# Orange-OpenSource/pyDcop

Measured on AMD Instinct MI355X. Metric: MaxSum iterations/sec on 100k-var random graph-coloring DCOP, higher is better.
Workload: dtype f64; 1 GPU; coloring_100k; n_vars=100000, n_factors=200000, n_edges=400000, domain=3, params=damping 0.5/both, stability 0.1, start leafs, parallelism=one GPU, 1 launch(es) per cycle, parity_checked=True, parity_test=tests/test_gpu_parity.py::test_north_star_100k_coloring

## Files before the change

include/maxsum_gpu.h:

```cpp
#ifndef MAXSUM_GPU_H
#define MAXSUM_GPU_H

#include <stdint.h>

#ifdef __cplusplus
extern "C" {
#endif

#define MXS_OK            0
#define MXS_E_INVALID    -1
#define MXS_E_NODEVICE   -2
#define MXS_E_HIP        -3
#define MXS_E_NOMEM      -4
#define MXS_E_STATE      -5
#define MXS_E_COMM       -6

#define MXS_MODE_MIN 0
#define MXS_MODE_MAX 1
#define MXS_DAMP_NONE    0
#define MXS_DAMP_VARS    1
#define MXS_DAMP_FACTORS 2
#define MXS_DAMP_BOTH    3
#define MXS_START_LEAFS      0
#define MXS_START_LEAFS_VARS 1
#define MXS_START_ALL        2
#define MXS_DTYPE_F64 0
#define MXS_DTYPE_F32 1

typedef struct mxs_graph {
    int32_t        n_vars;
    int32_t        n_factors;
    int32_t        n_edges;
    const int32_t *dom_size;
    const double  *var_cost;
    const int32_t *init_idx;
    const int32_t *factor_rowptr;
    const int32_t *edge_var;
    const int64_t *table_off;
    const double  *tables;
    const int32_t *var_rowptr;
    const int32_t *var_edges;
    const uint8_t *var_owned;
    const uint8_t *factor_owned;
    const double  *eval_var_cost;
} mxs_graph;

typedef struct mxs_params {
    int32_t mode;
    int32_t damping_nodes;
    int32_t start_messages;
    int32_t dtype;
    double  damping;
    double  stability;
    int32_t graph_chunk;
    int32_t layout_flags;
} mxs_params;

typedef struct mxs_engine mxs_engine;

int mxs_device_count(int32_t *count);

int mxs_create(const mxs_graph *g, const mxs_params *p, int32_t device,
               mxs_engine **out);

int mxs_reset(mxs_engine *e);

int mxs_run(mxs_engine *e, int32_t n_cycles);

int mxs_run_timed(mxs_engine *e, int32_t n_cycles, float *elapsed_ms);

int mxs_run_reps(mxs_engine *e, int32_t n_cycles, int32_t reps, float *elapsed_ms);

int mxs_run_async(mxs_engine *e, int32_t n_cycles);
int mxs_sync(mxs_engine *e);

int mxs_cycle_count(const mxs_engine *e, int64_t *cycles);

int mxs_get_assignment(mxs_engine *e, int32_t *idx, double *belief);

int mxs_get_messages(mxs_engine *e, double *v2f, double *f2v,
                     uint8_t *count_v2f, uint8_t *count_f2v);

int mxs_set_state(mxs_engine *e, const double *v2f, const double *f2v,
                  const uint8_t *count_v2f, const uint8_t *count_f2v,
                  const int32_t *idx, const double *belief, int64_t cycles);

int mxs_eval_cost(mxs_engine *e, const int32_t *idx, double infinity,
                  double *cost, int64_t *violations);

int mxs_cycle_bytes(const mxs_engine *e, int64_t *algorithmic_bytes,
                    int32_t *launches_per_cycle);

int mxs_table_storage(const mxs_engine *e, int64_t factors[4], int64_t *table_bytes_per_cycle);

int mxs_factor_order(const mxs_engine *e, int32_t *tiled);

int mxs_factor_kernels(const mxs_engine *e, int64_t counts[7]);

int mxs_variable_kernels(const mxs_engine *e, int64_t counts[6]);

int mxs_update_factor_table(mxs_engine *e, int32_t factor, const double *table, int64_t n_entries);

int mxs_set_parent_table(mxs_engine *e, int32_t factor, const double *parent, int32_t n_dims,
                         const int32_t *dims, const uint8_t *is_external);
int mxs_slice_factor(mxs_engine *e, int32_t factor, const int32_t *external_idx);

int mxs_debug_timeline(mxs_engine *e, int64_t *out, int32_t cap, int32_t *n_blocks);

int mxs_halo_setup(mxs_engine *e, const int32_t *send_edges, int64_t n_send,
                   const int32_t *recv_edges, int64_t n_recv);
int mxs_halo_buffers(mxs_engine *e, void **send_dev, int64_t *send_bytes,
                     void **recv_dev, int64_t *recv_bytes);
int mxs_halo_bind(mxs_engine *e, void *send_dev, void *recv_dev);
int mxs_step_compute(mxs_engine *e);
int mxs_step_pack(mxs_engine *e);
int mxs_step_unpack(mxs_engine *e);
int mxs_stream(mxs_engine *e, void **stream);

#define MXS_UNIQUE_ID_BYTES 128
int mxs_comm_unique_id(const char *rccl_path, uint8_t *id );
int mxs_comm_init(mxs_engine *e, const char *rccl_path, int32_t rank, int32_t world,
                  const uint8_t *id, const int64_t *send_counts, const int64_t *recv_counts);
int mxs_comm_exchange(mxs_engine *e);
int mxs_run_sharded(mxs_engine *e, int32_t n_cycles);
#define MXS_MAX_PEERS 8
#define MXS_MAX_ARITY 30
#define MXS_IPC_HANDLE_BYTES 64
typedef struct mxs_peer_info {
    int32_t qualifies;
    int32_t rank;
    int64_t ghost_len;
    int64_t recv_at[MXS_MAX_PEERS];
    int64_t recv_len[MXS_MAX_PEERS];
    uint8_t ghost_handle[MXS_IPC_HANDLE_BYTES];
    uint8_t flag_handle[MXS_IPC_HANDLE_BYTES];
    int64_t pid;
    uint64_t ghost_ptr, flag_ptr;
} mxs_peer_info;
int mxs_peer_export(mxs_engine *e, int32_t rank, int32_t world, const int64_t *send_counts,
                    const int64_t *recv_counts, mxs_peer_info *out);
int mxs_peer_connect(mxs_engine *e, const mxs_peer_info *all );

int mxs_shard_mode(const mxs_engine *e, int32_t *fused_launch, int32_t *direct_exchange);

int mxs_destroy(mxs_engine *e);

const char *mxs_last_error(void);

typedef struct mxs_amaxsum mxs_amaxsum;
int mxs_amaxsum_create(const mxs_graph *g, const mxs_params *p, int32_t device, mxs_amaxsum **out);
int mxs_amaxsum_reset(mxs_amaxsum *e);
int mxs_amaxsum_run(mxs_amaxsum *e, int32_t max_generations, int64_t *delivered);
int mxs_amaxsum_status(const mxs_amaxsum *e, int32_t *next_generation, int64_t *pending, int64_t *delivered);
int mxs_amaxsum_generation_sizes(const mxs_amaxsum *e, int64_t *out, int32_t cap, int32_t *n);
int mxs_amaxsum_get_assignment(mxs_amaxsum *e, int32_t *idx, double *belief);
int mxs_amaxsum_get_messages(mxs_amaxsum *e, double *f_cost, double *v_cost, double *f_prev, double *v_prev,
                             uint8_t *f_has, uint8_t *v_has, uint8_t *f_cnt, uint8_t *v_cnt);
int mxs_amaxsum_eval_cost(mxs_amaxsum *e, const int32_t *idx, double infinity, double *cost, int64_t *violations);
int mxs_amaxsum_update_factor_table(mxs_amaxsum *e, int32_t factor, const double *table, int64_t n_entries);
int mxs_amaxsum_destroy(mxs_amaxsum *e);

typedef struct mxs_mgm mxs_mgm;
int mxs_mgm_create(const mxs_graph *g, const mxs_params *p, const int32_t *name_rank, int32_t device,
                   mxs_mgm **out);
int mxs_mgm_reset(mxs_mgm *e);
int mxs_mgm_set_value_rank(mxs_mgm *e, const int32_t *value_rank);
int mxs_mgm_run(mxs_mgm *e, int32_t n_rounds);
int mxs_mgm_rounds(const mxs_mgm *e, int64_t *rounds);
int mxs_mgm_get_state(mxs_mgm *e, int32_t *idx, double *cost, uint8_t *has_cost, double *gain, int32_t *new_value);
int mxs_mgm_eval_cost(mxs_mgm *e, const int32_t *idx, double infinity, double *cost, int64_t *violations);
int mxs_mgm_destroy(mxs_mgm *e);

typedef struct mxs_dsa mxs_dsa;
int mxs_dsa_create(const mxs_graph *g, const mxs_params *p, int32_t variant, double probability,
                   int32_t arity_mode, uint64_t seed, int32_t device, mxs_dsa **out);
int mxs_dsa_reset(mxs_dsa *e);
int mxs_dsa_set_value_rank(mxs_dsa *e, const int32_t *value_rank);
int mxs_dsa_run(mxs_dsa *e, int32_t n_cycles);
int mxs_dsa_cycles(const mxs_dsa *e, int64_t *cycles);
int mxs_dsa_get_state(mxs_dsa *e, int32_t *idx, double *cost);
int mxs_dsa_eval_cost(mxs_dsa *e, const int32_t *idx, double infinity, double *cost, int64_t *violations);
int mxs_dsa_destroy(mxs_dsa *e);
// ... 68 lines not shown
```

pydcop_amd/csrc/engine.hip:

```cpp
#include <hip/hip_runtime.h>
#include <dlfcn.h>
#include <unistd.h>

#include <algorithm>
#include <climits>
#include <cstdio>
#include <cstdlib>
#include <cstring>
#include <map>
#include <memory>
#include <mutex>
#include <string>
#include <vector>

#include "../../include/maxsum_gpu.h"
#include "kernels.h"
#include "nary_box.h"
#include "bin_box.h"
#include "small_box.h"
#include "layout.h"

namespace mxs {

static thread_local std::string g_err;
// ... 70 lines not shown
    r->GroupEnd = (int (*)())sym("ncclGroupEnd");
    r->GetErrorString = (const char* (*)(int))sym("ncclGetErrorString");
    if (!ok) return nullptr;
    const Rccl* out = r.get();
    libs[key] = std::move(r);
    return out;
}

#define NCCL_TRY(expr)                                                                      \
    do {                                                                                    \
        int _r = (expr);                                                                    \
        if (_r != 0)                                                                        \
            return fail(MXS_E_COMM, std::string(#expr) + ": " + rccl->GetErrorString(_r));  \
    } while (0)

template <typename U>
struct DevBuf {
    U* p = nullptr;
    size_t n = 0;
    hipError_t alloc(size_t count) {
        if (p) (void)hipFree(p);
        p = nullptr;
        n = count;
        return hipMalloc((void**)&p, std::max<size_t>(count, 1) * sizeof(U));
    }
    hipError_t upload(const std::vector<U>& h, hipStream_t st) {
        hipError_t e = alloc(h.size());
        if (e != hipSuccess || h.empty()) return e;
        e = hipMemcpyAsync(p, h.data(), h.size() * sizeof(U), hipMemcpyHostToDevice, st);
        if (e != hipSuccess) return e;
        return hipStreamSynchronize(st);
    }
    ~DevBuf() {
        if (p) (void)hipFree(p);
    }
};

struct EngineBase {
    virtual ~EngineBase() {}
    virtual int init(const mxs_graph& g, const mxs_params& p, int device) = 0;
    virtual int reset() = 0;
    virtual int run_async(int n) = 0;
    virtual int sync() = 0;
    virtual int run_timed(int n, float* ms) = 0;
    virtual int run_reps(int n, int reps, float* ms) = 0;
    virtual int get_assignment(int32_t* idx, double* belief) = 0;
    virtual int get_messages(double* v2f, double* f2v, uint8_t* cv, uint8_t* cf) = 0;
    virtual int set_state(const double* v2f, const double* f2v, const uint8_t* cv, const uint8_t* cf,
                          const int32_t* idx, const double* belief, int64_t cyc) = 0;
    virtual int eval_cost(const int32_t* idx, double infinity, double* cost, int64_t* viol) = 0;
    virtual int halo_setup(const int32_t* se, int64_t ns, const int32_t* re, int64_t nr) = 0;
    virtual int halo_buffers(void** s, int64_t* sb, void** r, int64_t* rb) = 0;
    virtual int halo_bind(void* s, void* r) = 0;
    virtual int step_compute() = 0;
    virtual int step_pack() = 0;
    virtual int step_unpack() = 0;
    virtual int comm_init(const char* path, int rank, int world, const uint8_t* id,
                          const int64_t* sc, const int64_t* rc) = 0;
    virtual int comm_exchange() = 0;
    virtual int run_sharded(int n) = 0;
    virtual void shard_mode(int32_t* f, int32_t* d) const = 0;
    virtual int peer_export(int rank, int world, const int64_t* sc, const int64_t* rc, mxs_peer_info* out) = 0;
    virtual int peer_connect(const mxs_peer_info* all) = 0;
    virtual bool peer_mode() const = 0;
    virtual int debug_timeline(int64_t* out, int32_t cap, int32_t* n_blocks) = 0;
    virtual int update_table(int32_t factor, const double* table, int64_t n) = 0;
    virtual int set_parent(int32_t factor, const double* parent, int32_t nd, const int32_t* dims, const uint8_t* ext) = 0;
    virtual int slice_factor(int32_t factor, const int32_t* ext_idx) = 0;
    Layout L;
    mxs_params params{};
    int64_t cycles = 0;
    hipStream_t stream = nullptr;
    hipStream_t comm = nullptr;
    int launches_per_cycle = 1;
};

template <typename T>
struct Engine : EngineBase {
    int device = 0;
    int cur = 0;
    DevBuf<T> v2f[2], f2v[2], tables, var_cost, belief, halo_send, halo_recv;
    DevBuf<uint8_t> cF, cV, owned, fowned;
    DevBuf<int32_t> vrowptr, vdom, init_idx, edge_gen_factor, edge_dom, sel, vell;
    DevBuf<WaveMeta> vwave;
    DevBuf<int32_t> edge_v2f, f2v_off, vslot_f2v, vslot_v2f;
    DevBuf<int32_t> frowptr, edge_var_int, eval_idx;
    DevBuf<int64_t> vcost_off, eval_tab_off, halo_send_off, halo_recv_off, timeline;
    bool timeline_on = false;
    DevBuf<FactorGen> fgen;
    DevBuf<uint32_t> sched;
    DevBuf<uint8_t> ctables;
    size_t ctables_used = 0;
    DevBuf<ClassInfo> classes;
    DevBuf<ClassInfo> classes2;
    DevBuf<ClassInfo> classes_f;
    DevBuf<ClassInfo> classes8;
    DevBuf<uint32_t> halo_flags;
    bool fused = false;
    uint32_t unpacks = 0;
    DevBuf<NaryDesc> ndesc;
    DevBuf<WideBlock> wide_blocks;
    DevBuf<HubBlock> hub_blocks;
    bool has_hub = false;
#ifdef MXS_WIDE_PROFILE
    DevBuf<int64_t> wide_prof;
#endif
    DevBuf<double> eval_tables, eval_var_cost, part_cost;
    DevBuf<unsigned long long> part_viol;
    hipEvent_t ev0 = nullptr, ev1 = nullptr;
    hipStream_t side = nullptr;
    hipEvent_t ev_fork = nullptr, ev_join = nullptr;
    bool overlap = false, capturing = false;
    bool streaming = false;
    hipEvent_t ev_p1 = nullptr;
    hipEvent_t ev_halo = nullptr;
    bool halo_pending = false;
    hipGraphExec_t graph_exec = nullptr;
    int graph_cycles = 0;
    bool graph_tried = false;
    int64_t n_halo_send = 0, n_halo_recv = 0;
    T* send_buf = nullptr;
    T* recv_buf = nullptr;
    bool halo_ready = false;
    static constexpr int EVAL_BLOCKS = 1024;
    static constexpr int FUSED_MAX_CUT_BLOCKS = 1024;

    ~Engine() override {
        for (int q = 0; q < MXS_MAX_PEERS; ++q) {
            if (peer_local[q]) continue;
            if (peer_ghost[q]) (void)hipIpcCloseMemHandle(peer_ghost[q]);
            if (peer_flag[q]) (void)hipIpcCloseMemHandle(peer_flag[q]);
        }
        if (nccl_comm) {
            if (comm) (void)hipStreamSynchronize(comm);
            (void)rccl->CommDestroy(nccl_comm);
        }
#ifdef MXS_WIDE_PROFILE
        wide_profile_dump();
#endif
        if (graph_exec) (void)hipGraphExecDestroy(graph_exec);
        if (ev_fork) (void)hipEventDestroy(ev_fork);
        if (ev_join) (void)hipEventDestroy(ev_join);
        if (side) (void)hipStreamDestroy(side);
        if (ev0) (void)hipEventDestroy(ev0);
        if (ev1) (void)hipEventDestroy(ev1);
        if (ev_p1) (void)hipEventDestroy(ev_p1);
        if (ev_halo) (void)hipEventDestroy(ev_halo);
        if (comm) (void)hipStreamDestroy(comm);
        if (stream) (void)hipStreamDestroy(stream);
    }

    SweepArgs<T> make_args(int from, bool start, int phase = 1) const {
        SweepArgs<T> a{};
        a.v2f_old = v2f[from].p;
        a.v2f_new = v2f[from ^ 1].p;
        a.f2v_old = f2v[from].p;
        a.f2v_new = f2v[from ^ 1].p;
        a.tables = tables.p;
        a.ctables = ctables.p;
        a.tab_neg = L.is_max ? 1 : 0;
        a.var_cost = var_cost.p;
        a.cF = cF.p;
        a.cV = cV.p;
        a.edge_v2f = edge_v2f.p;
        a.f2v_off = f2v_off.p;
        a.vrowptr = vrowptr.p;
        a.vslot_f2v = vslot_f2v.p;
        a.vslot_v2f = vslot_v2f.p;
        a.vell = vell.p;
        a.vwave = vwave.p;
        a.hub_blocks = hub_blocks.p;
        a.vdom = vdom.p;
        a.vcost_off = vcost_off.p;
        a.init_idx = init_idx.p;
        a.fgen = fgen.p;
        a.edge_gen_factor = edge_gen_factor.p;
        a.edge_dom = edge_dom.p;
        a.sel = sel.p;
        a.belief = belief.p;
        a.damping = (T)params.damping;
        a.stability = (T)params.stability;
        a.damp_f = (params.damping_nodes & MXS_DAMP_FACTORS) ? 1 : 0;
        a.damp_v = (params.damping_nodes & MXS_DAMP_VARS) ? 1 : 0;
        a.start = start ? 1 : 0;
        a.start_mode = params.start_messages;
        a.null_f2v = (int32_t)L.null_f2v;
        a.timeline = timeline_on ? timeline.p : nullptr;
#ifdef MXS_WIDE_PROFILE
        if (!timeline_on) a.timeline = wide_prof.p;
#endif
        a.halo_flags = nullptr;
        a.need_epoch = 0;
        a.send_out = direct ? send2[from ^ 1].p : nullptr;
        a.send_slot = direct ? send_slot.p : nullptr;
        a.n_peers = 0;
        a.me = comm_rank;
        a.ghost_lo = INT32_MAX;
        a.ghost_old = nullptr;
        for (int q = 0; q < MXS_MAX_PEERS; ++q) {
            a.peer_first[q] = INT32_MAX;
            a.peer_dst[q] = nullptr;
        }
        if (p2p) {
            a.n_peers = comm_world;
            a.ghost_lo = (int32_t)L.v2f_elems;
            a.ghost_old = start ? ghost3.p + 3 * ghost_len : ghost3.p + (int64_t)(gen % 3) * ghost_len;
            a.send_slot = send_slot.p;
            a.send_out = nullptr;
            for (int q = 0; q < comm_world; ++q) {
                a.peer_first[q] = peer_first[q];
                a.peer_dst[q] = peer_ghost[q] ? peer_ghost[q] + (int64_t)((gen + 1) % 3) * peer_len[q] + peer_at[q] : nullptr;
            }
        }
        if (phase == 3) {
            a.n_classes = (int32_t)L.fused_block_base.size();
            for (int i = 0; i < MAX_CLASSES; ++i)
                a.block_base[i] = i < a.n_classes ? L.fused_block_base[i] : INT32_MAX;
            a.classes = classes_f.p;
            a.halo_flags = halo_flags.p;
            a.need_epoch = p2p ? gen : unpacks;
            return a;
        }
        const std::vector<int32_t>& order = phase == 1 ? L.sweep_order : L.sweep_order2;
        a.n_classes = (int32_t)order.size();
        for (int i = 0; i < MAX_CLASSES; ++i)
            a.block_base[i] = i < a.n_classes ? L.classes[order[i]].block_base : INT32_MAX;
        a.classes = phase == 1 ? classes.p : classes2.p;
        a.sched = (phase == 1 && !L.sched.empty()) ? sched.p : nullptr;
        return a;
    }

    int launch_sweep(const SweepArgs<T>& a, int nb) {
        if (nb <= 0) return MXS_OK;
        const dim3 grid(nb), block(BLOCK);
        if (p2p) {
            switch (L.dsel) {
                case 2: hipLaunchKernelGGL((k_sweep_p2p<T, 2>), grid, block, 0, stream, a); break;
                case 3: hipLaunchKernelGGL((k_sweep_p2p<T, 3>), grid, block, 0, stream, a); break;
                case 4: hipLaunchKernelGGL((k_sweep_p2p<T, 4>), grid, block, 0, stream, a); break;
                default: hipLaunchKernelGGL((k_sweep_p2p<T, 0>), grid, block, 0, stream, a); break;
            }
        } else if (timeline_on && has_hub) {
            if (L.dsel == 3) hipLaunchKernelGGL((k_sweep_timeline_hub<T, 3>), grid, block, 0, stream, a);
            else hipLaunchKernelGGL((k_sweep_timeline_hub<T, 0>), grid, block, 0, stream, a);
        } else if (timeline_on) {
            switch (L.dsel) {
                case 2: hipLaunchKernelGGL((k_sweep_timeline<T, 2>), grid, block, 0, stream, a); break;
                case 3: hipLaunchKernelGGL((k_sweep_timeline<T, 3>), grid, block, 0, stream, a); break;
                case 4: hipLaunchKernelGGL((k_sweep_timeline<T, 4>), grid, block, 0, stream, a); break;
                default: hipLaunchKernelGGL((k_sweep_timeline<T, 0>), grid, block, 0, stream, a); break;
            }
        } else if (has_hub) {
#define MXS_SWEEP_HUB(DS)                                                                                          \
    do {                                                                                                           \
        if (streaming) {                                                                                           \
            if (a.sched) hipLaunchKernelGGL((k_sweep_hub<T, DS, NT_STREAMING, true>), grid, block, 0, stream, a);  \
            else hipLaunchKernelGGL((k_sweep_hub<T, DS, NT_STREAMING, false>), grid, block, 0, stream, a);         \
        } else {                                                                                                   \
            if (a.sched) hipLaunchKernelGGL((k_sweep_hub<T, DS, MXS_NT, true>), grid, block, 0, stream, a);        \
            else hipLaunchKernelGGL((k_sweep_hub<T, DS, MXS_NT, false>), grid, block, 0, stream, a);               \
        }                                                                                                          \
    } while (0)
            if (L.dsel == 3) MXS_SWEEP_HUB(3);
            else MXS_SWEEP_HUB(0);
#undef MXS_SWEEP_HUB
        } else {
#define MXS_SWEEP(DS)                                                                                          \
    do {                                                                                                       \
        if (streaming) {                                                                                       \
            if (a.sched) hipLaunchKernelGGL((k_sweep<T, DS, NT_STREAMING, true>), grid, block, 0, stream, a);  \
            else hipLaunchKernelGGL((k_sweep<T, DS, NT_STREAMING, false>), grid, block, 0, stream, a);         \
        } else {                                                                                               \
            if (a.sched) hipLaunchKernelGGL((k_sweep<T, DS, MXS_NT, true>), grid, block, 0, stream, a);        \
            else hipLaunchKernelGGL((k_sweep<T, DS, MXS_NT, false>), grid, block, 0, stream, a);               \
        }                                                                                                      \
    } while (0)
            switch (L.dsel) {
                case 2:
                    if (streaming) {
                        if (a.sched) hipLaunchKernelGGL((k_sweep_d2<T, NT_STREAMING, true>), grid, block, 0, stream, a);
                        else hipLaunchKernelGGL((k_sweep_d2<T, NT_STREAMING, false>), grid, block, 0, stream, a);
                    } else {
                        if (a.sched) hipLaunchKernelGGL((k_sweep_d2<T, MXS_NT, true>), grid, block, 0, stream, a);
                        else hipLaunchKernelGGL((k_sweep_d2<T, MXS_NT, false>), grid, block, 0, stream, a);
                    }
                    break;
                case 3: MXS_SWEEP(3); break;
                case 4: MXS_SWEEP(4); break;
                default: MXS_SWEEP(0); break;
            }
#undef MXS_SWEEP
        }
        HIP_TRY(hipGetLastError());
        return MXS_OK;
    }

    std::vector<int8_t> nary_ls_cache;
    bool nary_last_same(const NaryLaunch& nl) {
        const size_t idx = (size_t)(&nl - L.nary_launches.data());
        if (nary_ls_cache.size() != L.nary_launches.size()) nary_ls_cache.assign(L.nary_launches.size(), -1);
        if (nary_ls_cache[idx] < 0) {
            int8_t ok = 1;
            for (int j = 0; j < nl.count && ok; ++j) {
                const NaryDesc& d = L.ndesc[nl.first + j];
                if (nl.threads % d.dom[(d.arity & 255) - 1] != 0) ok = 0;
            }
            nary_ls_cache[idx] = ok;
        }
        return nary_ls_cache[idx] == 1;
    }

    std::vector<int32_t> nary_cap_cache;
    int nary_group_cap(const NaryLaunch& nl) {
        const size_t idx = (size_t)(&nl - L.nary_launches.data());
        if (nary_cap_cache.size() != L.nary_launches.size()) nary_cap_cache.assign(L.nary_launches.size(), -1);
        if (nary_cap_cache[idx] < 0) {
            int cap = 2;
            for (int j = 0; j < nl.count; ++j) {
                const NaryDesc& d = L.ndesc[nl.first + j];
                int sumd = 0;
                for (int i = 0; i < (d.arity & 255); ++i) sumd += d.dom[i];
                cap = std::max(cap, sumd);
            }
            nary_cap_cache[idx] = (cap + 1) & ~1;
        }
        return nary_cap_cache[idx];
    }

    const NaryLaunch* launch_of(int fi) const {
        for (const NaryLaunch& x : L.nary_launches)
            if (L.f_ndesc[fi] >= x.first && L.f_ndesc[fi] < x.first + x.count) return &x;
        return nullptr;
    }

    int pack8_host_group() const {
        if (L.pack8_classes.empty() || !L.opt.pack8_fused) return -1;
        if (params.layout_flags & (32 | 64)) return -1;
        int best = -1;
        for (size_t i = 0; i < L.nary_launches.size(); ++i) {
            const NaryLaunch& nl = L.nary_launches[i];
            if (!is_bin2(nl.box) || nl.cut) continue;
            if (best < 0 || nl.count > L.nary_launches[best].count) best = (int)i;
        }
        return best;
    }

    int launch_nary(const SweepArgs<T>& a, int cut) {
        const int host8 = cut == 0 ? pack8_host_group() : -1;
// ... 53 lines not shown
        }                                                                                                                                      \
        break;
                switch (nl.arity) {
                    MXS_NARY_MULTI(3) MXS_NARY_MULTI(4) MXS_NARY_MULTI(5) MXS_NARY_MULTI(6)
                    default: return fail(MXS_E_STATE, "no multi-pass n-ary kernel for this arity");
                }
#undef MXS_NARY_MULTI
                HIP_TRY(hipGetLastError());
                continue;
            }
            switch (nl.arity * 16 + nl.nj) {
                MXS_NARY_CASE(2, 1) MXS_NARY_CASE(2, 2) MXS_NARY_CASE(2, 3) MXS_NARY_CASE(2, 4)
                MXS_NARY_CASE(3, 1) MXS_NARY_CASE(3, 2) MXS_NARY_CASE(3, 3) MXS_NARY_CASE(3, 4)
                MXS_NARY_CASE(4, 1) MXS_NARY_CASE(4, 2) MXS_NARY_CASE(4, 3) MXS_NARY_CASE(4, 4)
                MXS_NARY_CASE(5, 1) MXS_NARY_CASE(5, 2) MXS_NARY_CASE(5, 3) MXS_NARY_CASE(5, 4)
                default: return fail(MXS_E_STATE, "no n-ary kernel for this (arity, size) group");
            }
#undef MXS_NARY_CASE
#undef MXS_NARY_PACKED
            HIP_TRY(hipGetLastError());
        }
        return MXS_OK;
    }

    int launch_wide(const SweepArgs<T>& a, hipStream_t ws) {
        if (!L.pack8_classes.empty() && pack8_host_group() < 0) {
            const ClassInfo& ci = L.classes[L.pack8_classes[0]];
            hipLaunchKernelGGL((k_variable_pack8<T>), dim3((unsigned)((ci.count + BLOCK - 1) / BLOCK)), dim3(BLOCK), 0, ws, a,
                               (const ClassInfo*)classes8.p);
            HIP_TRY(hipGetLastError());
        }
        if (!L.wide_blocks.empty()) {
            hipLaunchKernelGGL((k_variable_wide<T>), dim3((unsigned)L.wide_blocks.size()), dim3(WIDE_TPB), 0, ws, a,
                               (const WideBlock*)wide_blocks.p);
            HIP_TRY(hipGetLastError());
        }
        return MXS_OK;
    }
    int n_wide_launches() const { return (L.wide_blocks.empty() ? 0 : 1) + ((L.pack8_classes.empty() || pack8_host_group() >= 0) ? 0 : 1); }

    int launch_phase(int from, bool start, int phase) {
        const SweepArgs<T> a = make_args(from, start, phase);
        if (phase == 3) {
            int rc = launch_sweep(a, L.n_blocks_fused);
            if (rc) return rc;
            { int rc2 = launch_wide(a, stream); if (rc2) return rc2; }
            return launch_nary(a, 0);
        }
        if (phase == 1) {
            int rc = launch_sweep(a, (start || L.sweep_regular) ? L.n_blocks_sweep : 0);
            if (rc) return rc;
            const bool vars_only = (params.layout_flags & 32) != 0, factors_only = (params.layout_flags & 64) != 0;
            if (vars_only || factors_only) {
                if (!factors_only) { rc = launch_wide(a, stream); if (rc) return rc; }
                return vars_only ? MXS_OK : launch_nary(a, 0);
            }
            const bool fork = overlap && !capturing && n_wide_launches() > 0 && !L.nary_launches.empty();
            hipStream_t ws = stream;
            if (fork) {
                HIP_TRY(hipEventRecord(ev_fork, stream));
                HIP_TRY(hipStreamWaitEvent(side, ev_fork, 0));
                ws = side;
            }
            rc = launch_wide(a, ws);
            if (rc) return rc;
            if (fork) HIP_TRY(hipEventRecord(ev_join, side));
            rc = launch_nary(a, 0);
            if (rc) return rc;
            if (fork) HIP_TRY(hipStreamWaitEvent(stream, ev_join, 0));
            return MXS_OK;
        }
        int rc = launch_sweep(a, L.n_blocks_sweep2);
        if (rc) return rc;
        return launch_nary(a, 1);
    }

    int launch_cycle(int from, bool start) {
        int rc = launch_phase(from, start, 1);
        if (rc) return rc;
        return launch_phase(from, start, 2);
    }

    int upload_class_arrays() {
        std::vector<ClassInfo> order;
        for (int c : L.sweep_order) order.push_back(L.classes[c]);
        HIP_TRY(classes.upload(order, stream));
        order.clear();
        for (int c : L.sweep_order2) order.push_back(L.classes[c]);
        HIP_TRY(classes2.upload(order, stream));
        order.clear();
        if (L.n_blocks_fused > 0) {
            for (int c : L.sweep_order) order.push_back(L.classes[c]);
            for (int c : L.sweep_order2) order.push_back(L.classes[c]);
            for (size_t i = 0; i < order.size(); ++i) order[i].block_base = L.fused_block_base[i];
        }
        HIP_TRY(classes_f.upload(order, stream));
        order.clear();
        for (int c : L.pack8_classes) order.push_back(L.classes[c]);
        HIP_TRY(classes8.upload(order, stream));
        return MXS_OK;
    }

    int promote_class(int cls) {
        if (L.classes[cls].tab_type == TAB_FULL) return MXS_OK;
        { int rc = sync(); if (rc) return rc; }
        L.classes[cls].tab_type = TAB_FULL;
        for (int fi = 0; fi < L.n_factors; ++fi)
            if (L.f_class[fi] == cls) L.f_tab_type[fi] = (uint8_t)TAB_FULL;
        if (graph_exec) {
            (void)hipGraphExecDestroy(graph_exec);
            graph_exec = nullptr;
            graph_tried = false;
        }
        return upload_class_arrays();
    }

    int widen_factor(int fi, const double* values = nullptr) {
        if (L.f_tab_type[fi] == TAB_FULL) return MXS_OK;
        if (L.f_class[fi] >= 0) return promote_class(L.f_class[fi]);
        { int rc = sync(); if (rc) return rc; }
        int64_t bin2_at = -1;
        if (const NaryLaunch* nl = launch_of(fi); nl && is_bin2(nl->box)) {
            int rc = append_bin2_full_image(fi, *nl, values, &bin2_at);
            if (rc) return rc;
        }
        struct Item { int cut, code, type, fi; NaryDesc d; };
        std::vector<int> fi_of(L.ndesc.size(), -1);
        for (int f2 = 0; f2 < L.n_factors; ++f2)
            if (L.f_ndesc[f2] >= 0) fi_of[L.f_ndesc[f2]] = f2;
        std::vector<Item> items;
        for (const NaryLaunch& nl : L.nary_launches)
            for (int j = 0; j < nl.count; ++j) {
                Item it{nl.cut, nary_group_code(nl.box, nl.arity, nl.nj, nl.threads / 64), nl.tab_type, fi_of[nl.first + j],
                        L.ndesc[nl.first + j]};
                if (it.fi == fi && bin2_at >= 0) {
                    it.type = TAB_FULL;
                    it.d.tab_off = bin2_at;
                } else if (it.fi == fi) {
                    it.type = TAB_FULL;
                    it.d.tab_off = L.f_tab_base[fi];
                    int64_t R = 1;
                    for (int i = 1; i < nl.arity; ++i) R *= it.d.dom[i];
                    if (!(nl.box == 0 && nl.nj == NARY_NJ_MULTI)) it.code = nary_group_code(0, nl.arity, nary_classic_nj(R), nary_classic_waves(R));
                }
                items.push_back(it);
            }
        std::stable_sort(items.begin(), items.end(), [](const Item& x, const Item& y) {
            return x.cut != y.cut ? x.cut < y.cut : x.code != y.code ? x.code < y.code : x.type < y.type;
        });
        L.ndesc.clear();
        L.nary_launches.clear();
        nary_ls_cache.clear();
        nary_cap_cache.clear();
        for (size_t i = 0; i < items.size(); ++i) {
            const Item& it = items[i];
            if (i == 0 || it.cut != items[i - 1].cut || it.code != items[i - 1].code || it.type != items[i - 1].type)
                L.nary_launches.push_back(NaryLaunch{(it.code / 256) % 16, (it.code / 16) % 16, (it.code % 16) * 64,
                                                     (int32_t)i, 0, it.cut, it.type, it.code / 4096});
            L.nary_launches.back().count += 1;
            L.f_ndesc[it.fi] = (int32_t)i;
            L.ndesc.push_back(it.d);
        }
        L.f_tab_type[fi] = (uint8_t)TAB_FULL;
        if (bin2_at >= 0) L.f_ctab_off[fi] = bin2_at;
        if (graph_exec) {
            (void)hipGraphExecDestroy(graph_exec);
            graph_exec = nullptr;
            graph_tried = false;
        }
        HIP_TRY(ndesc.upload(L.ndesc, stream));
        launches_per_cycle = ((L.n_blocks_sweep > 0 && L.sweep_regular) ? 1 : 0) + (L.n_blocks_sweep2 > 0 ? 1 : 0) +
                             (int)L.nary_launches.size() + n_wide_launches();
        return MXS_OK;
    }

    int init(const mxs_graph& g, const mxs_params& p, int dev) override {
        params = p;
        device = dev;
        std::string e = build_layout(g, p, L);
        if (!e.empty()) return fail(MXS_E_INVALID, e);
        if (params.graph_chunk < 0) params.graph_chunk = L.algorithmic_bytes < (4 << 20) ? 32 : 0;
        {
            streaming = L.algorithmic_bytes > ((int64_t)256 << 20);
            const char* env = getenv("MAXSUM_STREAMING");
            if (env && (env[0] == '0' || env[0] == '1')) streaming = env[0] == '1';
        }
        int count = 0;
        if (hipGetDeviceCount(&count) != hipSuccess || count <= 0)
            return fail(MXS_E_NODEVICE, "no HIP device visible: the Max-Sum engine has no CPU fallback");
        if (dev < 0 || dev >= count) return fail(MXS_E_INVALID, "device index out of range");
        hipDeviceProp_t prop;
        HIP_TRY(hipGetDeviceProperties(&prop, dev));
        if (std::string(prop.gcnArchName).find("gfx950") == std::string::npos)
            return fail(MXS_E_NODEVICE, std::string("device is ") + prop.gcnArchName +
                                            ", this library is built for gfx950 (MI355X) only");
        HIP_TRY(hipSetDevice(dev));
        HIP_TRY(hipStreamCreateWithFlags(&stream, hipStreamNonBlocking));
        HIP_TRY(hipEventCreate(&ev0));
        HIP_TRY(hipEventCreate(&ev1));
        HIP_TRY(hipStreamCreateWithFlags(&side, hipStreamNonBlocking));
        HIP_TRY(hipEventCreateWithFlags(&ev_fork, hipEventDisableTiming));
        HIP_TRY(hipEventCreateWithFlags(&ev_join, hipEventDisableTiming));
        {
            const char* env = getenv("MAXSUM_NARY_OVERLAP");
            overlap = L.algorithmic_bytes >= ((int64_t)400 << 20);
            if (env && (env[0] == '0' || env[0] == '1')) overlap = env[0] == '1';
        }
        {
            int lo = 0, hi = 0;
            HIP_TRY(hipDeviceGetStreamPriorityRange(&lo, &hi));
            HIP_TRY(hipStreamCreateWithPriority(&comm, hipStreamNonBlocking, hi));
        }
        HIP_TRY(hipEventCreateWithFlags(&ev_p1, hipEventDisableTiming));
        HIP_TRY(hipEventCreateWithFlags(&ev_halo, hipEventDisableTiming));

        auto conv = [](const std::vector<double>& src) {
            std::vector<T> out(src.size());
            for (size_t i = 0; i < src.size(); ++i) out[i] = (T)src[i];
            return out;
        };
        for (int b = 0; b < 2; ++b) {
            HIP_TRY(v2f[b].alloc((size_t)L.v2f_elems));
            HIP_TRY(f2v[b].alloc((size_t)L.f2v_elems));
        }
        HIP_TRY(edge_v2f.upload(L.v2f_off, stream));
        HIP_TRY(f2v_off.upload(L.f2v_off, stream));
        HIP_TRY(vslot_f2v.upload(L.vslot_f2v, stream));
        HIP_TRY(vslot_v2f.upload(L.vslot_v2f, stream));
        HIP_TRY(tables.upload(conv(L.tables), stream));
        HIP_TRY(ctables.upload(L.ctables, stream));
        HIP_TRY(var_cost.upload(conv(L.var_cost), stream));
        HIP_TRY(cF.alloc((size_t)L.n_edges));
        HIP_TRY(cV.alloc((size_t)L.n_cv));
        HIP_TRY(vell.upload(L.vell, stream));
        HIP_TRY(vwave.upload(L.vwave, stream));
        HIP_TRY(owned.upload(L.owned, stream));
        HIP_TRY(fowned.upload(L.fowned, stream));
        HIP_TRY(vrowptr.upload(L.vrowptr, stream));
        HIP_TRY(vdom.upload(L.vdom, stream));
        HIP_TRY(init_idx.upload(L.init_idx, stream));
        HIP_TRY(edge_gen_factor.upload(L.edge_gen_factor, stream));
        HIP_TRY(edge_dom.upload(L.edge_dom, stream));
        HIP_TRY(sel.alloc((size_t)L.n_vars));
        HIP_TRY(belief.alloc((size_t)L.n_vars));
        HIP_TRY(vcost_off.upload(L.vcost_off, stream));
        HIP_TRY(fgen.upload(L.fgen, stream));
        { int rc = upload_class_arrays(); if (rc) return rc; }
        HIP_TRY(sched.upload(L.sched, stream));
        HIP_TRY(halo_flags.alloc(64));
        HIP_TRY(ndesc.upload(L.ndesc, stream));
        HIP_TRY(wide_blocks.upload(L.wide_blocks, stream));
        HIP_TRY(hub_blocks.upload(L.hub_blocks, stream));
        has_hub = !L.hub_blocks.empty();
#ifdef MXS_WIDE_PROFILE
        if (!L.wide_blocks.empty()) {
            HIP_TRY(wide_prof.alloc(8 * L.wide_blocks.size()));
            HIP_TRY(hipMemset(wide_prof.p, 0, sizeof(int64_t) * 8 * L.wide_blocks.size()));
        }
#endif
        HIP_TRY(frowptr.upload(L.frowptr, stream));
        HIP_TRY(edge_var_int.upload(L.edge_var_int, stream));
        HIP_TRY(eval_tab_off.upload(L.eval_tab_off, stream));
        HIP_TRY(eval_tables.upload(L.eval_tables, stream));
        HIP_TRY(eval_var_cost.upload(L.eval_var_cost, stream));
        HIP_TRY(eval_idx.alloc((size_t)L.n_vars));
        HIP_TRY(part_cost.alloc(EVAL_BLOCKS));
        HIP_TRY(part_viol.alloc(EVAL_BLOCKS));
        launches_per_cycle = ((L.n_blocks_sweep > 0 && L.sweep_regular) ? 1 : 0) + (L.n_blocks_sweep2 > 0 ? 1 : 0) +
                             (int)L.nary_launches.size() + n_wide_launches();
        return reset();
    }

    int reset() override {
        HIP_TRY(hipSetDevice(device));
        if (comm) HIP_TRY(hipStreamSynchronize(comm));
        HIP_TRY(hipStreamSynchronize(stream));
        for (int b = 0; b < 2; ++b) {
            HIP_TRY(hipMemsetAsync(v2f[b].p, 0, std::max<size_t>(v2f[b].n, 1) * sizeof(T), stream));
            HIP_TRY(hipMemsetAsync(f2v[b].p, 0, std::max<size_t>(f2v[b].n, 1) * sizeof(T), stream));
        }
        HIP_TRY(hipMemsetAsync(cF.p, 0, std::max<size_t>(cF.n, 1), stream));
        HIP_TRY(hipMemsetAsync(cV.p, 0, std::max<size_t>(cV.n, 1), stream));
        HIP_TRY(hipMemsetAsync(sel.p, 0, std::max<size_t>(sel.n, 1) * sizeof(int32_t), stream));
        HIP_TRY(hipMemsetAsync(belief.p, 0, std::max<size_t>(belief.n, 1) * sizeof(T), stream));
        if (!p2p) HIP_TRY(hipMemsetAsync(halo_flags.p, 0, 64 * sizeof(uint32_t), stream));
        unpacks = 0;
        cur = 0;
        cycles = 0;
        int rc = p2p ? launch_phase(cur, true, 3) : launch_cycle(cur, true);
        if (rc) return rc;
        cur ^= 1;
        halo_pending = false;
        if (p2p) {
            rc = p2p_publish();
            if (rc) return rc;
            return sync();
        }
        HIP_TRY(hipEventRecord(ev_p1, stream));
        if (halo_ready) {
            rc = pack();
            if (rc) return rc;
        }
        return sync();
    }

    void try_build_graph() {
        graph_tried = true;
        int chunk = params.graph_chunk;
        if (chunk < 0) chunk = 32;
        if (chunk < 2) return;
        chunk &= ~1;
        if (cur != 0) return;
        hipGraph_t graph = nullptr;
        if (hipStreamBeginCapture(stream, hipStreamCaptureModeThreadLocal) != hipSuccess) {
            (void)hipGetLastError();
            return;
        }
// ... 63 lines not shown
#endif
    int sync() override {
        HIP_TRY(hipStreamSynchronize(stream));
        if (comm) HIP_TRY(hipStreamSynchronize(comm));
        if (fused || p2p) {
            uint32_t h[1] = {0};
            HIP_TRY(hipMemcpyAsync(h, halo_flags.p + HALO_ERR_WORD, sizeof(h), hipMemcpyDeviceToHost, stream));
            HIP_TRY(hipStreamSynchronize(stream));
            if (h[0] != 0)
                return fail(MXS_E_STATE, "sharded cycle: cut factors waited > 5 s for a halo exchange that "
                                         "never arrived (an exchange / mxs_step_unpack per mxs_step_compute?)");
        }
        return MXS_OK;
    }

    int run_timed(int n, float* ms) override {
        HIP_TRY(hipSetDevice(device));
        if (!graph_tried && cur == 0 && n >= 2 * std::max(2, params.graph_chunk < 0 ? 32 : params.graph_chunk))
            try_build_graph();
        HIP_TRY(hipEventRecord(ev0, stream));
        int rc = run_async(n);
        if (rc) return rc;
        HIP_TRY(hipEventRecord(ev1, stream));
        HIP_TRY(hipEventSynchronize(ev1));
        float t = 0.f;
        HIP_TRY(hipEventElapsedTime(&t, ev0, ev1));
        if (ms) *ms = t;
        return MXS_OK;
    }

    int run_reps(int n, int reps, float* ms) override {
        HIP_TRY(hipSetDevice(device));
        if (n < 1 || reps < 1 || reps > 100000) return fail(MXS_E_INVALID, "mxs_run_reps: n >= 1, 1 <= reps <= 100000");
        if (halo_ready || p2p) return fail(MXS_E_STATE, "mxs_run_reps: not on a sharded engine");
        if (!graph_tried && cur == 0 && n >= 2 * std::max(2, params.graph_chunk < 0 ? 32 : params.graph_chunk))
            try_build_graph();
        std::vector<hipEvent_t> evs((size_t)reps + 1, nullptr);
        int rc = MXS_OK;
        hipError_t he = hipSuccess;
        for (hipEvent_t& e : evs)
            if (he == hipSuccess) he = hipEventCreate(&e);
        for (int r = 0; r < reps && he == hipSuccess && rc == MXS_OK; ++r) {
            if (r == 0) he = hipEventRecord(evs[0], stream);
            if (he == hipSuccess) rc = run_async(n);
            if (rc == MXS_OK && he == hipSuccess) he = hipEventRecord(evs[r + 1], stream);
        }
        if (he == hipSuccess && rc == MXS_OK) he = hipEventSynchronize(evs[reps]);
        for (int r = 0; r < reps && he == hipSuccess && rc == MXS_OK; ++r) {
            float t = 0.f;
            he = hipEventElapsedTime(&t, evs[r], evs[r + 1]);
            if (ms) ms[r] = t;
        }
        for (hipEvent_t e : evs)
            if (e) (void)hipEventDestroy(e);
        if (rc) return rc;
        HIP_TRY(he);
        return sync();
    }

    int get_assignment(int32_t* idx, double* bel) override {
        HIP_TRY(hipSetDevice(device));
        { int rc = sync(); if (rc) return rc; }
        const int nV = L.n_vars;
        std::vector<int32_t> hs(nV);
        std::vector<T> hb(nV);
        if (nV) {
            HIP_TRY(copy_sync(hs.data(), sel.p, sizeof(int32_t) * nV, hipMemcpyDeviceToHost, stream));
            HIP_TRY(copy_sync(hb.data(), belief.p, sizeof(T) * nV, hipMemcpyDeviceToHost, stream));
        }
        const double sign = L.is_max ? -1.0 : 1.0;
        for (int vi = 0; vi < nV; ++vi) {
            const int v = L.var_i2e[vi];
            if (idx) idx[v] = hs[vi];
            if (bel) bel[v] = sign * (double)hb[vi];
        }
        return MXS_OK;
    }

    int get_messages(double* v2f_out, double* f2v_out, uint8_t* cv, uint8_t* cf) override {
        HIP_TRY(hipSetDevice(device));
        { int rc = sync(); if (rc) return rc; }
        const int nE = L.n_edges;
        std::vector<T> hv((size_t)(L.v2f_elems + (p2p ? ghost_len : 0))), hf((size_t)L.f2v_elems);
        std::vector<uint8_t> hcF(nE), hcV((size_t)L.n_cv);
        if (L.v2f_elems)
            HIP_TRY(copy_sync(hv.data(), v2f[cur].p, sizeof(T) * (size_t)L.v2f_elems, hipMemcpyDeviceToHost, stream));
        if (p2p && ghost_len)
            HIP_TRY(copy_sync(hv.data() + L.v2f_elems, ghost3.p + (int64_t)(gen % 3) * ghost_len,
                              sizeof(T) * (size_t)ghost_len, hipMemcpyDeviceToHost, stream));
        if (L.f2v_elems)
            HIP_TRY(copy_sync(hf.data(), f2v[cur].p, sizeof(T) * hf.size(), hipMemcpyDeviceToHost, stream));
        if (nE) {
            HIP_TRY(copy_sync(hcF.data(), cF.p, nE, hipMemcpyDeviceToHost, stream));
            HIP_TRY(copy_sync(hcV.data(), cV.p, (size_t)L.n_cv, hipMemcpyDeviceToHost, stream));
        }
        std::vector<int64_t> ext_off(nE + 1, 0);
        for (int e = 0; e < nE; ++e) ext_off[e + 1] = ext_off[e] + L.edge_dom[L.edge_e2i[e]];
        const double sign = L.is_max ? -1.0 : 1.0;
        for (int ei = 0; ei < nE; ++ei) {
            const int e = L.edge_i2e[ei];
            const int D = L.edge_dom[ei];
            for (int d = 0; d < D; ++d) {
                if (v2f_out) v2f_out[ext_off[e] + d] = sign * (double)hv[L.v2f_off[ei] + d];
                if (f2v_out) f2v_out[ext_off[e] + d] = sign * (double)hf[L.f2v_off[ei] + d];
            }
            if (cf) cf[e] = L.edge_fcim[ei] ? (uint8_t)(int)hf[L.f2v_off[ei] + D] : hcF[ei];
        }
        if (cv)
            for (int k = 0; k < nE; ++k) {
                const int ei = L.vslot_edge[k];
                cv[L.edge_i2e[ei]] = L.edge_vcim[ei] ? (uint8_t)(int)hv[L.v2f_off[ei] + L.edge_dom[ei]]
                                                     : hcV[L.vslot_cv[k]];
            }
        return MXS_OK;
    }

    int set_state(const double* v2f_in, const double* f2v_in, const uint8_t* cv, const uint8_t* cf,
                  const int32_t* idx, const double* bel, int64_t cyc) override {
        HIP_TRY(hipSetDevice(device));
        { int rc = sync(); if (rc) return rc; }
        if (halo_ready || p2p) return fail(MXS_E_STATE, "mxs_set_state on a shard with an exchange set up");
        if (cyc < 0) return fail(MXS_E_INVALID, "negative cycle count");
        const int nE = L.n_edges, nV = L.n_vars;
        std::vector<T> hv((size_t)L.v2f_elems), hf((size_t)L.f2v_elems);
        std::vector<uint8_t> hcF(nE), hcV((size_t)L.n_cv);
        if (L.v2f_elems) HIP_TRY(copy_sync(hv.data(), v2f[cur].p, sizeof(T) * hv.size(), hipMemcpyDeviceToHost, stream));
        if (L.f2v_elems) HIP_TRY(copy_sync(hf.data(), f2v[cur].p, sizeof(T) * hf.size(), hipMemcpyDeviceToHost, stream));
        if (nE) {
            HIP_TRY(copy_sync(hcF.data(), cF.p, nE, hipMemcpyDeviceToHost, stream));
            HIP_TRY(copy_sync(hcV.data(), cV.p, (size_t)L.n_cv, hipMemcpyDeviceToHost, stream));
        }
        std::vector<int64_t> ext_off(nE + 1, 0);
        for (int e = 0; e < nE; ++e) ext_off[e + 1] = ext_off[e] + L.edge_dom[L.edge_e2i[e]];
        const double sign = L.is_max ? -1.0 : 1.0;
        for (int ei = 0; ei < nE; ++ei) {
            const int e = L.edge_i2e[ei];
            const int D = L.edge_dom[ei];
            for (int d = 0; d < D; ++d) {
                if (v2f_in) hv[L.v2f_off[ei] + d] = (T)(sign * v2f_in[ext_off[e] + d]);
                if (f2v_in) hf[L.f2v_off[ei] + d] = (T)(sign * f2v_in[ext_off[e] + d]);
            }
            if (cf) {
                if (cf[e] > SAME_COUNT) return fail(MXS_E_INVALID, "send counter above SAME_COUNT");
                if (L.edge_fcim[ei]) hf[L.f2v_off[ei] + D] = (T)(int)cf[e];
                else hcF[ei] = cf[e];
            }
        }
        if (cv)
            for (int k = 0; k < nE; ++k) {
                const int ei = L.vslot_edge[k];
                const uint8_t c = cv[L.edge_i2e[ei]];
                if (c > SAME_COUNT) return fail(MXS_E_INVALID, "send counter above SAME_COUNT");
                if (L.edge_vcim[ei]) hv[L.v2f_off[ei] + L.edge_dom[ei]] = (T)(int)c;
                else hcV[L.vslot_cv[k]] = c;
            }
        if (L.v2f_elems) HIP_TRY(copy_sync(v2f[cur].p, hv.data(), sizeof(T) * hv.size(), hipMemcpyHostToDevice, stream));
        if (L.f2v_elems) HIP_TRY(copy_sync(f2v[cur].p, hf.data(), sizeof(T) * hf.size(), hipMemcpyHostToDevice, stream));
        if (nE) {
            HIP_TRY(copy_sync(cF.p, hcF.data(), nE, hipMemcpyHostToDevice, stream));
            HIP_TRY(copy_sync(cV.p, hcV.data(), (size_t)L.n_cv, hipMemcpyHostToDevice, stream));
        }
        if ((idx || bel) && nV) {
            std::vector<int32_t> hs(nV);
            std::vector<T> hb(nV);
            HIP_TRY(copy_sync(hs.data(), sel.p, sizeof(int32_t) * nV, hipMemcpyDeviceToHost, stream));
            HIP_TRY(copy_sync(hb.data(), belief.p, sizeof(T) * nV, hipMemcpyDeviceToHost, stream));
            for (int vi = 0; vi < nV; ++vi) {
                const int v = L.var_i2e[vi];
                if (idx) {
                    if (idx[v] < 0 || idx[v] >= L.vdom[vi]) return fail(MXS_E_INVALID, "selection index out of the domain");
                    hs[vi] = idx[v];
                }
                if (bel) hb[vi] = (T)(sign * bel[v]);
            }
            HIP_TRY(copy_sync(sel.p, hs.data(), sizeof(int32_t) * nV, hipMemcpyHostToDevice, stream));
            HIP_TRY(copy_sync(belief.p, hb.data(), sizeof(T) * nV, hipMemcpyHostToDevice, stream));
        }
        cycles = cyc;
        return MXS_OK;
    }

    int eval_cost(const int32_t* idx, double infinity, double* cost, int64_t* viol) override {
        HIP_TRY(hipSetDevice(device));
        { int rc = sync(); if (rc) return rc; }
        const int nV = L.n_vars;
        const int32_t* didx = sel.p;
        if (idx) {
            std::vector<int32_t> h(nV);
            for (int vi = 0; vi < nV; ++vi) {
                const int32_t x = idx[L.var_i2e[vi]];
                if (x < 0 || x >= L.vdom[vi]) return fail(MXS_E_INVALID, "assignment index out of the domain");
                h[vi] = x;
            }
            HIP_TRY(copy_sync(eval_idx.p, h.data(), sizeof(int32_t) * nV, hipMemcpyHostToDevice, stream));
            didx = eval_idx.p;
        }
        EvalArgs a{};
        a.frowptr = frowptr.p;
        a.edge_var_int = edge_var_int.p;
        a.edge_dom = edge_dom.p;
        a.tab_off = eval_tab_off.p;
        a.tables = eval_tables.p;
        a.vdom = vdom.p;
        a.vcost_off = vcost_off.p;
        a.var_cost = eval_var_cost.p;
        a.owned = owned.p;
        a.fowned = fowned.p;
        a.idx = didx;
        a.part_cost = part_cost.p;
        a.part_viol = part_viol.p;
        a.n_factors = L.n_factors;
        a.n_vars = nV;
        a.infinity = infinity;
        const int total = L.n_factors + nV;
        const int nb = std::max(1, std::min(EVAL_BLOCKS, (total + BLOCK - 1) / BLOCK));
        hipLaunchKernelGGL(k_eval, dim3(nb), dim3(BLOCK), 0, stream, a);
        HIP_TRY(hipGetLastError());
        std::vector<double> pc(nb);
        std::vector<unsigned long long> pv(nb);
        HIP_TRY(hipStreamSynchronize(stream));
        HIP_TRY(copy_sync(pc.data(), part_cost.p, sizeof(double) * nb, hipMemcpyDeviceToHost, stream));
        HIP_TRY(copy_sync(pv.data(), part_viol.p, sizeof(unsigned long long) * nb, hipMemcpyDeviceToHost, stream));
        double c = 0;
        int64_t v = 0;
        for (int i = 0; i < nb; ++i) {
            c += pc[i];
            v += (int64_t)pv[i];
        }
        if (cost) *cost = c;
        if (viol) *viol = v;
        return MXS_OK;
    }

    int debug_timeline(int64_t* out, int32_t cap, int32_t* n_blocks) override {
        HIP_TRY(hipSetDevice(device));
        if (halo_ready) return fail(MXS_E_STATE, "mxs_debug_timeline: not on a sharded engine");
        const int nb = L.n_blocks_sweep;
        if (n_blocks) *n_blocks = nb;
        if (!out) return MXS_OK;
        if (cap < nb) return fail(MXS_E_INVALID, "timeline buffer too small");
        if (timeline.n < (size_t)3 * nb) {
            if (timeline.p) (void)hipFree(timeline.p);
// ... 758 lines not shown
    return e->impl->get_messages(v2f, f2v, cv, cf);
}

int mxs_set_state(mxs_engine* e, const double* v2f, const double* f2v, const uint8_t* cv, const uint8_t* cf,
                  const int32_t* idx, const double* belief, int64_t cycles) {
    CHECK_HANDLE(e);
    return e->impl->set_state(v2f, f2v, cv, cf, idx, belief, cycles);
}

int mxs_table_storage(const mxs_engine* e, int64_t factors[4], int64_t* table_bytes) {
    CHECK_HANDLE(e);
    const mxs::Layout& L = e->impl->L;
    const int64_t w = L.opt.word;
    int64_t n[4] = {0, 0, 0, 0}, bytes = 0;
    for (int fi = 0; fi < L.n_factors; ++fi) {
        const int t = L.f_tab_type[fi];
        const int64_t entries = L.eval_tab_off[fi + 1] - L.eval_tab_off[fi];
        n[t] += 1;
        if (L.f_class[fi] >= 0) bytes += t == mxs::TAB_FULL ? entries * w : L.classes[L.f_class[fi]].ctab_rec;
        else if (L.f_ndesc[fi] < 0) bytes += entries * w;
        else {
            for (const mxs::NaryLaunch& x : L.nary_launches)
                if (L.f_ndesc[fi] >= x.first && L.f_ndesc[fi] < x.first + x.count) {
                    const mxs::NaryDesc& d = L.ndesc[L.f_ndesc[fi]];
                    if (t == mxs::TAB_FULL && !mxs::is_bin2(x.box)) bytes += entries * w;
                    else bytes += mxs::nary_place_bytes(mxs::nary_place(x, d, (int)w), d.dom[0]);
                }
        }
    }
    if (factors) std::memcpy(factors, n, sizeof(n));
    if (table_bytes) *table_bytes = bytes;
    return MXS_OK;
}

int mxs_set_parent_table(mxs_engine* e, int32_t factor, const double* parent, int32_t n_dims,
                         const int32_t* dims, const uint8_t* is_external) {
    CHECK_HANDLE(e);
    return e->impl->set_parent(factor, parent, n_dims, dims, is_external);
}

int mxs_slice_factor(mxs_engine* e, int32_t factor, const int32_t* external_idx) {
    CHECK_HANDLE(e);
    return e->impl->slice_factor(factor, external_idx);
}

int mxs_eval_cost(mxs_engine* e, const int32_t* idx, double infinity, double* cost, int64_t* viol) {
    CHECK_HANDLE(e);
    return e->impl->eval_cost(idx, infinity, cost, viol);
}

int mxs_cycle_bytes(const mxs_engine* e, int64_t* bytes, int32_t* launches) {
    CHECK_HANDLE(e);
    if (bytes) *bytes = e->impl->L.algorithmic_bytes;
    if (launches) *launches = e->impl->launches_per_cycle;
    return MXS_OK;
}

int mxs_factor_order(const mxs_engine* e, int32_t* tiled) {
    CHECK_HANDLE(e);
    if (tiled) *tiled = e->impl->L.tiled ? 1 : 0;
    return MXS_OK;
}

int mxs_factor_kernels(const mxs_engine* e, int64_t counts[7]) {
    CHECK_HANDLE(e);
    if (!counts) return MXS_OK;
    const mxs::Layout& L = e->impl->L;
    for (int i = 0; i < 7; ++i) counts[i] = 0;
    for (int fi = 0; fi < L.n_factors; ++fi) {
        if (L.f_class[fi] >= 0) {
            const int k = L.classes[L.f_class[fi]].kind;
            counts[k == mxs::K_F_UNARY ? 0 : k == mxs::K_F_BIN ? 1 : 2] += 1;
        } else if (L.f_ndesc[fi] >= 0) {
            for (const mxs::NaryLaunch& x : L.nary_launches)
                if (L.f_ndesc[fi] >= x.first && L.f_ndesc[fi] < x.first + x.count)
                    counts[mxs::is_small(x.box) ? 6 : mxs::is_bin2(x.box) ? 5 : x.box ? 4 : 3] += 1;
        } else {
            counts[2] += 1;
        }
    }
    return MXS_OK;
}

int mxs_variable_kernels(const mxs_engine* e, int64_t counts[6]) {
    CHECK_HANDLE(e);
    if (!counts) return MXS_OK;
    const mxs::Layout& L = e->impl->L;
    for (int i = 0; i < 6; ++i) counts[i] = 0;
    int64_t swept = 0;
    for (const mxs::ClassInfo& ci : L.classes) {
        int64_t n = 0;
        if (ci.kind == mxs::K_V_PACK || ci.kind == mxs::K_V_PACK8) {
            for (int64_t w = ci.ell_base >> 6; w < (ci.ell_base + ci.count) >> 6; ++w) n += ((uint32_t)L.vwave[w].deg_nv >> 8) & 255u;
            counts[ci.kind == mxs::K_V_PACK ? 0 : 1] += n;
        } else if (ci.kind == mxs::K_V_WIDE) {
            counts[2] += (n = ci.count);
        } else if (ci.kind == mxs::K_V_GEN && !ci.start_only) {
            counts[3] += (n = ci.count);
        } else if (ci.kind == mxs::K_V_HUB) {
            for (int32_t w = ci.first; w < ci.first + ci.count; ++w) n += L.hub_blocks[w].ko0 == 0;
            counts[5] += n;
        }
        swept += n;
    }
    counts[4] = L.n_vars - swept;
    return MXS_OK;
}

int mxs_halo_setup(mxs_engine* e, const int32_t* se, int64_t ns, const int32_t* re, int64_t nr) {
    CHECK_HANDLE(e);
    if ((ns && !se) || (nr && !re) || ns < 0 || nr < 0) return fail(MXS_E_INVALID, "bad halo lists");
    return e->impl->halo_setup(se, ns, re, nr);
}

int mxs_halo_buffers(mxs_engine* e, void** s, int64_t* sb, void** r, int64_t* rb) {
    CHECK_HANDLE(e);
    return e->impl->halo_buffers(s, sb, r, rb);
}

int mxs_halo_bind(mxs_engine* e, void* s, void* r) { CHECK_HANDLE(e); return e->impl->halo_bind(s, r); }

int mxs_step_compute(mxs_engine* e) { CHECK_HANDLE(e); return e->impl->step_compute(); }
int mxs_step_pack(mxs_engine* e) { CHECK_HANDLE(e); return e->impl->step_pack(); }
int mxs_step_unpack(mxs_engine* e) { CHECK_HANDLE(e); return e->impl->step_unpack(); }

int mxs_comm_unique_id(const char* rccl_path, uint8_t* id) {
    if (!id) return fail(MXS_E_INVALID, "null argument");
    std::string err;
    const mxs::Rccl* rccl = mxs::load_rccl(rccl_path, err);
    if (!rccl) return fail(MXS_E_COMM, err);
    mxs::NcclUniqueId uid;
    int r = rccl->GetUniqueId(&uid);
    if (r != 0) return fail(MXS_E_COMM, std::string("ncclGetUniqueId: ") + rccl->GetErrorString(r));
    std::memcpy(id, uid.internal, MXS_UNIQUE_ID_BYTES);
    return MXS_OK;
}

int mxs_comm_init(mxs_engine* e, const char* rccl_path, int32_t rank, int32_t world, const uint8_t* id,
                  const int64_t* send_counts, const int64_t* recv_counts) {
    CHECK_HANDLE(e);
    return e->impl->comm_init(rccl_path, rank, world, id, send_counts, recv_counts);
}

int mxs_comm_exchange(mxs_engine* e) { CHECK_HANDLE(e); return e->impl->comm_exchange(); }
int mxs_run_sharded(mxs_engine* e, int32_t n) { CHECK_HANDLE(e); return e->impl->run_sharded(n); }

int mxs_peer_export(mxs_engine* e, int32_t rank, int32_t world, const int64_t* send_counts,
                    const int64_t* recv_counts, mxs_peer_info* out) {
    CHECK_HANDLE(e);
    return e->impl->peer_export(rank, world, send_counts, recv_counts, out);
}

int mxs_peer_connect(mxs_engine* e, const mxs_peer_info* all) {
    CHECK_HANDLE(e);
    return e->impl->peer_connect(all);
}

int mxs_shard_mode(const mxs_engine* e, int32_t* fused_launch, int32_t* direct_exchange) {
    CHECK_HANDLE(e);
    e->impl->shard_mode(fused_launch, direct_exchange);
    return MXS_OK;
}

int mxs_stream(mxs_engine* e, void** stream) {
    CHECK_HANDLE(e);
    if (stream) *stream = (void*)e->impl->comm;
// ... 33 lines not shown
```

pydcop_amd/csrc/kernels.h:

```cpp
#pragma once
#include <hip/hip_runtime.h>

#include <cmath>
#include <cstdint>
#include <cstring>
#include <type_traits>
#include <utility>

#include "layout.h"

namespace mxs {

constexpr int SAME_COUNT = 4;
#ifndef MXS_ASM_MIN
#define MXS_ASM_MIN 1
#endif
#ifndef SWEEP_MIN_WAVES
#define SWEEP_MIN_WAVES 4
#endif

#ifndef MXS_NT
#define MXS_NT 0
#endif
constexpr int NT_STREAMING = 9;
// ... 34 lines not shown
#define MXS_NT_TIGHT 1
#endif

template <typename T, int ELEMS, int NT = MXS_NT>
__device__ __forceinline__ void wave_store_linear(T* arr, int64_t wave_base, const T (&vals)[ELEMS]) {
    constexpr bool NT_STORE = (NT & 8) != 0;
    static_assert(64 * ELEMS * sizeof(T) % 16 == 0 && 64 * ELEMS * sizeof(T) <= STAGE_BYTES_PER_WAVE, "");
    if constexpr (ELEMS * sizeof(T) % 16 != 0) {
        const int w = (int)threadIdx.x >> 6, l = (int)threadIdx.x & 63;
        char* so = (char*)g_stage[w];
        __builtin_amdgcn_wave_barrier();
#pragma unroll
        for (int d = 0; d < ELEMS; ++d) ((T*)so)[l * ELEMS + d] = vals[d];
        __builtin_amdgcn_wave_barrier();
        char* out = (char*)(arr + wave_base);
        constexpr int BYTES = 64 * ELEMS * (int)sizeof(T), FULL = BYTES / 1024, REST = (BYTES % 1024) / 16;
#pragma unroll
        for (int k = 0; k < FULL; ++k) store_piece16<NT_STORE && MXS_NT_TIGHT>(out + k * 1024 + l * 16, so + k * 1024 + l * 16);
        if (REST > 0 && l < REST) store_piece16<NT_STORE && MXS_NT_TIGHT>(out + FULL * 1024 + l * 16, so + FULL * 1024 + l * 16);
        return;
    }
    const int w = (int)threadIdx.x >> 6, l = (int)threadIdx.x & 63;
    char* so = (char*)g_stage[w];
    __builtin_amdgcn_wave_barrier();
#pragma unroll
    for (int d = 0; d < ELEMS; ++d) ((T*)so)[l * ELEMS + d] = vals[d];
    __builtin_amdgcn_wave_barrier();
    char* out = (char*)(arr + wave_base);
    constexpr int PIECES = ELEMS * (int)sizeof(T) / 16;
#pragma unroll
    for (int k = 0; k < PIECES; ++k) store_piece16<NT_STORE>(out + k * 1024 + l * 16, so + k * 1024 + l * 16);
}

template <typename T>
struct SweepArgs {
    const T* v2f_old;
    T* v2f_new;
    const T* f2v_old;
    T* f2v_new;
    const T* tables;
    const uint8_t* ctables;
    int32_t tab_neg;
    const T* var_cost;
    uint8_t* cF;
    uint8_t* cV;
    const int32_t* edge_v2f;
    const int32_t* f2v_off;
    const int32_t* vrowptr;
    const int32_t* vslot_f2v;
    const int32_t* vslot_v2f;
    const int32_t* vell;
    const WaveMeta* vwave;
    const HubBlock* hub_blocks;
    const int32_t* vdom;
    const int64_t* vcost_off;
    const int32_t* init_idx;
    const FactorGen* fgen;
    const int32_t* edge_gen_factor;
    const int32_t* edge_dom;
    int32_t* sel;
    T* belief;
    T damping;
    T stability;
    int32_t damp_f;
    int32_t damp_v;
    int32_t start;
    int32_t start_mode;
    int32_t null_f2v;
    int64_t* timeline;
    uint32_t* halo_flags;
    uint32_t need_epoch;
    T* send_out;
    const int32_t* send_slot;
    int32_t n_peers;
    int32_t me;
    int32_t ghost_lo;
    const T* ghost_old;
    int32_t peer_first[MXS_MAX_PEERS];
    T* peer_dst[MXS_MAX_PEERS];
    int32_t n_classes;
    int32_t block_base[MAX_CLASSES];
    const ClassInfo* classes;
    const uint32_t* sched;
};

template <typename T>
__device__ __forceinline__ T pos_inf() {
    return (T)INFINITY;
}
__device__ __forceinline__ double absT(double x) { return fabs(x); }
__device__ __forceinline__ float absT(float x) { return fabsf(x); }

template <typename T>
__device__ __forceinline__ bool comp_match(T c, T prev_c, T stability) {
    if (prev_c != c) {
        const T delta = absT(prev_c - c);
        if (prev_c + c != (T)0) {
            if (!(((T)2 * delta / absT(prev_c + c)) < stability)) return false;
        } else {
            return false;
        }
    }
    return true;
}

template <typename T, int D>
__device__ __forceinline__ uint8_t damp_and_filter(T (&m)[D], const T (&prev)[D], uint8_t cnt,
                                                   bool damp_on, T damping, T stability) {
    if (cnt > 0 && damp_on) {
#pragma unroll
        for (int d = 0; d < D; ++d) m[d] = damping * prev[d] + ((T)1 - damping) * m[d];
    }
    bool match = cnt > 0;
#pragma unroll
    for (int d = 0; d < D; ++d) match = match && comp_match(m[d], prev[d], stability);
    if (!match) return 1;
    if (cnt < SAME_COUNT) return (uint8_t)(cnt + 1);
#pragma unroll
    for (int d = 0; d < D; ++d) m[d] = prev[d];
    return cnt;
}

template <typename T, int D>
struct Msg {
    static constexpr int H = half_stride(D, (int)sizeof(T));
    static constexpr int ALIGN = (H * (int)sizeof(T)) % 16 == 0 ? 16 : ((H * (int)sizeof(T)) % 8 == 0 ? 8 : 4);
    template <bool NT = false>
    static __device__ __forceinline__ void load(const T* p, T (&m)[D]) {
        const T* q = (const T*)__builtin_assume_aligned(p, ALIGN);
#pragma unroll
        for (int d = 0; d < D; ++d) m[d] = ldp<NT>(q + d);
    }
    static __device__ __forceinline__ void store(T* p, const T (&m)[D]) {
        T* q = (T*)__builtin_assume_aligned(p, ALIGN);
#pragma unroll
        for (int d = 0; d < H; ++d) q[d] = d < D ? m[d < D ? d : 0] : (T)0;
    }
    static __device__ __forceinline__ void load_sys(const T* p, T (&m)[D]) {
#pragma unroll
        for (int d = 0; d < D; ++d) m[d] = __hip_atomic_load(p + d, __ATOMIC_RELAXED, __HIP_MEMORY_SCOPE_SYSTEM);
    }
    static constexpr bool CNT_IN_MSG = H > D;
    template <bool NT = false>
    static __device__ __forceinline__ uint8_t load_c(const T* p, T (&m)[D]) {
        const T* q = (const T*)__builtin_assume_aligned(p, ALIGN);
#pragma unroll
        for (int d = 0; d < D; ++d) m[d] = ldp<NT>(q + d);
        return (uint8_t)(int)ldp<NT>(q + (D < H ? D : 0));
    }
    static __device__ __forceinline__ T padded(const T (&m)[D], uint8_t cnt, int d) {
        return d < D ? m[d < D ? d : 0] : (d == D ? (T)(int)cnt : (T)0);
    }
    static __device__ __forceinline__ void store_c(T* p, const T (&m)[D], uint8_t cnt) {
        T* q = (T*)__builtin_assume_aligned(p, ALIGN);
#pragma unroll
        for (int d = 0; d < H; ++d) q[d] = padded(m, cnt, d);
    }
};

template <typename T, int N, int NT = MXS_NT>
__device__ __forceinline__ void load_table(const SweepArgs<T>& a, const ClassInfo& ci, int j, T (&tab)[N]) {
    MXS_NT_FLAGS(NT);
    if (ci.tab_type == TAB_FULL) {
#pragma unroll
        for (int k = 0; k < N; ++k) tab[k] = ldp<NT_IDX>(a.tables + ci.tab_base + (int64_t)k * ci.count + j);
        return;
    }
    if (ci.tab_type == TAB_I8) {
        constexpr int REC = tab_record_bytes(N, 1);
        uint32_t w[REC / 4];
        const uint32_t* p = (const uint32_t*)__builtin_assume_aligned(
            a.ctables + ci.ctab_base + (int64_t)j * REC, REC >= 16 ? 16 : REC);
#pragma unroll
        for (int i = 0; i < REC / 4; ++i) w[i] = ldp<NT_IDX>(p + i);
#pragma unroll
        for (int k = 0; k < N; ++k) tab[k] = (T)(int)(int8_t)(uint8_t)(w[k >> 2] >> (8 * (k & 3)));
    } else if (ci.tab_type == TAB_I16) {
        constexpr int REC = tab_record_bytes(N, 2);
        uint32_t w[REC / 4];
        const uint32_t* p = (const uint32_t*)__builtin_assume_aligned(
            a.ctables + ci.ctab_base + (int64_t)j * REC, REC >= 16 ? 16 : REC);
#pragma unroll
        for (int i = 0; i < REC / 4; ++i) w[i] = ldp<NT_IDX>(p + i);
#pragma unroll
        for (int k = 0; k < N; ++k) tab[k] = (T)(int)(int16_t)(uint16_t)(w[k >> 1] >> (16 * (k & 1)));
    } else {
        constexpr int REC = tab_record_bytes(N, 4);
        uint32_t w[REC / 4];
        const uint32_t* p = (const uint32_t*)__builtin_assume_aligned(
            a.ctables + ci.ctab_base + (int64_t)j * REC, REC >= 16 ? 16 : REC);
#pragma unroll
        for (int i = 0; i < REC / 4; ++i) w[i] = ldp<NT_IDX>(p + i);
#pragma unroll
        for (int k = 0; k < N; ++k) {
            float f;
            __builtin_memcpy(&f, &w[k], 4);
            tab[k] = (T)f;
        }
    }
    if (a.tab_neg) {
#pragma unroll
        for (int k = 0; k < N; ++k) tab[k] = -tab[k];
    }
}

template <typename T, int D, int NT = MXS_NT>
__device__ __forceinline__ void factor_unary(const SweepArgs<T>& a, const ClassInfo& ci, int j) {
    MXS_NT_FLAGS(NT);
    constexpr int H = Msg<T, D>::H;
    const int64_t fo = ci.f2v_base + (int64_t)j * H;
    const int e = ci.edge_base + j;
    constexpr bool CIM = Msg<T, D>::CNT_IN_MSG;
    T out[D], prev[D], tab[D];
    uint8_t cn;
    if constexpr (CIM) cn = Msg<T, D>::template load_c<NT_PREV>(a.f2v_old + fo, prev);
    else {
        Msg<T, D>::template load<NT_PREV>(a.f2v_old + fo, prev);
        cn = a.cF[e];
    }
    load_table<T, D, NT>(a, ci, j, tab);
#pragma unroll
    for (int d = 0; d < D; ++d)
        out[d] = tab[d] + (T)0;
    uint8_t c = 0;
    if (!a.start)
        c = damp_and_filter<T, D>(out, prev, cn, a.damp_f != 0, a.damping, a.stability);
    if constexpr (CIM) {
        Msg<T, D>::store_c(a.f2v_new + fo, out, c);
    } else {
        Msg<T, D>::store(a.f2v_new + fo, out);
        a.cF[e] = c;
    }
}

template <typename T, int D, bool P2P = false, int NT = MXS_NT, bool CUT_HALF = true>
__device__ __forceinline__ void factor_binary(const SweepArgs<T>& a, const ClassInfo& ci, int j) {
    MXS_NT_FLAGS(NT);
    constexpr int H = Msg<T, D>::H;
    const int e = ci.edge_base + 2 * j;
    const int64_t fo0 = ci.f2v_base + (int64_t)j * H, fo1 = ci.f2v_base1 + (int64_t)j * H;
    constexpr bool CIM = Msg<T, D>::CNT_IN_MSG;
    const bool do0 = !CUT_HALF || ci.own_pos != 2, do1 = !CUT_HALF || ci.own_pos != 1;
    const int v0 = do1 ? ldp<NT_IDX>(a.edge_v2f + e) : 0, v1 = do0 ? ldp<NT_IDX>(a.edge_v2f + e + 1) : 0;
    uint8_t cn0 = 0, cn1 = 0;
    T m0[D], p0[D], m1[D], p1[D], tab[D * D];
#pragma unroll
    for (int d = 0; d < D; ++d) m0[d] = p0[d] = m1[d] = p1[d] = (T)0;
    if constexpr (CIM) {
        if (do0) cn0 = Msg<T, D>::template load_c<NT_PREV>(a.f2v_old + fo0, p0);
        if (do1) cn1 = Msg<T, D>::template load_c<NT_PREV>(a.f2v_old + fo1, p1);
    } else {
        if (do0) {
            cn0 = a.cF[e];
            Msg<T, D>::template load<NT_PREV>(a.f2v_old + fo0, p0);
        }
        if (do1) {
            cn1 = a.cF[e + 1];
            Msg<T, D>::template load<NT_PREV>(a.f2v_old + fo1, p1);
        }
    }
    load_table<T, D * D, NT>(a, ci, j, tab);
    if constexpr (P2P) {
        if (do1) {
            if (v0 >= a.ghost_lo) Msg<T, D>::load_sys(a.ghost_old + (v0 - a.ghost_lo), m0);
            else Msg<T, D>::load(a.v2f_old + v0, m0);
        }
        if (do0) {
            if (v1 >= a.ghost_lo) Msg<T, D>::load_sys(a.ghost_old + (v1 - a.ghost_lo), m1);
            else Msg<T, D>::load(a.v2f_old + v1, m1);
        }
    } else {
        if (do1) Msg<T, D>::template load<NT_GATHER>(a.v2f_old + v0, m0);
        if (do0) Msg<T, D>::template load<NT_GATHER>(a.v2f_old + v1, m1);
    }
    T o0[D], o1[D];
#pragma unroll
    for (int x = 0; x < D; ++x) {
        T best0 = pos_inf<T>(), best1 = pos_inf<T>();
#pragma unroll
        for (int y = 0; y < D; ++y) {
            const T c0 = tab[x * D + y] + ((T)0 + m1[y]);
            if (best0 > c0) best0 = c0;
            const T c1 = tab[y * D + x] + ((T)0 + m0[y]);
            if (best1 > c1) best1 = c1;
        }
        o0[x] = best0;
        o1[x] = best1;
    }
    uint8_t c0 = 0, c1 = 0;
    if (a.start) {
        const bool sends = a.start_mode == MXS_START_ALL;
#pragma unroll
        for (int d = 0; d < D; ++d) {
            o0[d] = sends ? o0[d] : (T)0;
            o1[d] = sends ? o1[d] : (T)0;
        }
    } else {
        c0 = damp_and_filter<T, D>(o0, p0, cn0, a.damp_f != 0, a.damping, a.stability);
        c1 = damp_and_filter<T, D>(o1, p1, cn1, a.damp_f != 0, a.damping, a.stability);
    }
    const int lw = (int)threadIdx.x & 63;
    if constexpr ((64 * H * sizeof(T)) % 16 == 0) {
        if ((j - lw + 63) < ci.count) {
            T full[H];
            if (do0) {
#pragma unroll
                for (int d = 0; d < H; ++d) full[d] = Msg<T, D>::padded(o0, CIM ? c0 : 0, d);
                wave_store_linear<T, H, NT>(a.f2v_new, fo0 - (int64_t)lw * H, full);
            }
            if (do1) {
#pragma unroll
                for (int d = 0; d < H; ++d) full[d] = Msg<T, D>::padded(o1, CIM ? c1 : 0, d);
                wave_store_linear<T, H, NT>(a.f2v_new, fo1 - (int64_t)lw * H, full);
            }
        } else {
            if (do0) Msg<T, D>::store_c(a.f2v_new + fo0, o0, CIM ? c0 : 0);
            if (do1) Msg<T, D>::store_c(a.f2v_new + fo1, o1, CIM ? c1 : 0);
        }
    } else {
        if (do0) Msg<T, D>::store_c(a.f2v_new + fo0, o0, CIM ? c0 : 0);
        if (do1) Msg<T, D>::store_c(a.f2v_new + fo1, o1, CIM ? c1 : 0);
    }
    if constexpr (!CIM) {
        if (do0) a.cF[e] = c0;
        if (do1) a.cF[e + 1] = c1;
    }
}

template <typename T>
__device__ __forceinline__ T factor_gen_value(const SweepArgs<T>& a, const FactorGen& fg, int pos,
                                              int d, int64_t others) {
    T best = pos_inf<T>();
    for (int64_t lin = 0; lin < others; ++lin) {
        int64_t rem = others, l = lin, t = 0;
        T sum_cost = (T)0;
        for (int i = 0; i < fg.arity; ++i) {
            const int e = fg.edge_base + i;
            const int Di = a.edge_dom[e];
            int digit;
            if (i == pos) {
                digit = d;
            } else {
                rem /= Di;
                digit = (int)(l / rem);
                l -= (int64_t)digit * rem;
                sum_cost += a.v2f_old[a.edge_v2f[e] + digit];
            }
            t = t * Di + digit;
        }
        const T cur = a.tables[fg.tab_off + t] + sum_cost;
        if (best > cur) best = cur;
    }
    return best;
}

template <typename T>
__device__ __forceinline__ void factor_generic(const SweepArgs<T>& a, const ClassInfo& ci, int j) {
    const int e = ci.edge_base + j;
    const FactorGen fg = a.fgen[a.edge_gen_factor[e]];
    const int pos = e - fg.edge_base;
    const int D = a.edge_dom[e];
    const T* prev = a.f2v_old + a.f2v_off[e];
    T* w = a.f2v_new + a.f2v_off[e];
    int64_t others = 1;
    for (int i = 0; i < fg.arity; ++i)
        if (i != pos) others *= a.edge_dom[fg.edge_base + i];
    if (a.start) {
        const bool sends = (fg.arity == 1 && a.start_mode != MXS_START_ALL) ||
                           a.start_mode == MXS_START_ALL;
        for (int d = 0; d < D; ++d) w[d] = sends ? factor_gen_value(a, fg, pos, d, others) : (T)0;
        a.cF[e] = 0;
        return;
    }
    const uint8_t cnt = a.cF[e];
    const bool damp = cnt > 0 && a.damp_f;
    bool match = cnt > 0;
    for (int d = 0; d < D; ++d) {
        T m = factor_gen_value(a, fg, pos, d, others);
        const T p = prev[d];
        if (damp) m = a.damping * p + ((T)1 - a.damping) * m;
        if (match) match = comp_match(m, p, a.stability);
        w[d] = m;
    }
    uint8_t out = 1;
    if (match) {
        if (cnt < SAME_COUNT) {
            out = (uint8_t)(cnt + 1);
        } else {
            out = cnt;
            for (int d = 0; d < D; ++d) w[d] = prev[d];
        }
    }
    a.cF[e] = out;
}

template <typename T, int D, bool P2P = false, int NT = MXS_NT>
__device__ __forceinline__ void variable_pack(const SweepArgs<T>& a, const ClassInfo& ci, int item) {
    MXS_NT_FLAGS(NT);
    constexpr int H = Msg<T, D>::H;
    const int lane_id = item + (int)threadIdx.x;
    if (lane_id >= ci.count) return;
    const int64_t pos = ci.ell_base + lane_id;
    const WaveMeta wm = a.vwave[__builtin_amdgcn_readfirstlane((int)(pos >> 6))];
    const uint32_t dn = (uint32_t)wm.deg_nv;
    const int deg = (int)(dn & 255u), nv = (int)((dn >> 8) & 255u);
    const int l = (int)threadIdx.x & 63;
    const int var = (int)(((uint32_t)l * (dn >> 16)) >> 15);
    const int k = l - var * deg;
    const bool has = var < nv;
    const int v = wm.first_var + (has ? var : 0);
    const int32_t slot = ldp<NT_IDX>(a.vell + pos);
    const int32_t send_at = a.send_slot != nullptr ? a.send_slot[pos] : -1;
    constexpr bool CIM = Msg<T, D>::CNT_IN_MSG;
    T pv[D], in[D], c[D], b[D], m[D];
    const int64_t vo = ci.v2f_base + (int64_t)lane_id * H;
    uint8_t cnt;
    if constexpr (CIM) cnt = Msg<T, D>::template load_c<NT_PREV>(a.v2f_old + vo, pv);
    else {
        cnt = a.cV[ci.cv_base + lane_id];
        Msg<T, D>::template load<NT_PREV>(a.v2f_old + vo, pv);
    }
    Msg<T, D>::template load<NT_GATHER>(a.f2v_old + (has ? slot : a.null_f2v), in);
#pragma unroll
    for (int d = 0; d < D; ++d) c[d] = a.var_cost[ci.cost_base + (int64_t)(v - ci.first) * D + d];
    int init = -1;
    if (a.start) init = a.init_idx[v];
    const int seg = l - (has ? k : 0);
    T sum_cost = (T)0;
#pragma unroll
    for (int d = 0; d < D; ++d) {
        T bd = c[d], md = c[d];
        for (int kk = 0; kk < deg; ++kk) {
            const T x = __shfl(in[d], seg + kk, 64);
            bd += x;
            if (kk != k) {
                sum_cost += x;
                md += x;
            }
        }
        b[d] = bd;
        m[d] = md;
    }
    int best = 0;
    T best_c = b[0];
#pragma unroll
    for (int d = 1; d < D; ++d)
        if (b[d] < best_c) {
            best = d;
            best_c = b[d];
        }
    if (init >= 0) {
        best = init;
        best_c = (T)0;
    }
    if (has && k == 0) {
        a.sel[v] = best;
        a.belief[v] = best_c;
    }
    const T avg = sum_cost / (T)D;
#pragma unroll
    for (int d = 0; d < D; ++d) m[d] = m[d] - avg;
    uint8_t co = 0;
    if (a.start) {
        const bool sends = (deg == 1 && a.start_mode == MXS_START_LEAFS) ||
                           a.start_mode != MXS_START_LEAFS;
#pragma unroll
        for (int d = 0; d < D; ++d) m[d] = sends ? m[d] : (T)0;
    } else {
        co = damp_and_filter<T, D>(m, pv, cnt, a.damp_v != 0, a.damping, a.stability);
    }
    if (!has) {
        co = 0;
#pragma unroll
        for (int d = 0; d < D; ++d) m[d] = (T)0;
    }
    if (send_at >= 0) {
        T* dst = a.send_out + (int64_t)send_at * H;
        if constexpr (P2P) {
            T* base = a.peer_dst[0];
            int first = a.peer_first[0];
#pragma unroll
            for (int q = 1; q < MXS_MAX_PEERS; ++q) {
                const bool ge = send_at >= a.peer_first[q];
                base = ge ? a.peer_dst[q] : base;
                first = ge ? a.peer_first[q] : first;
            }
            dst = base + (int64_t)(send_at - first) * H;
        }
        Msg<T, D>::store_c(dst, m, CIM ? co : 0);
    }
    if constexpr ((64 * H * sizeof(T)) % 16 == 0) {
        T full[H];
#pragma unroll
        for (int d = 0; d < H; ++d) full[d] = Msg<T, D>::padded(m, CIM ? co : 0, d);
        wave_store_linear<T, H, NT>(a.v2f_new, vo - (int64_t)l * H, full);
    } else {
        Msg<T, D>::store(a.v2f_new + vo, m);
    }
    if constexpr (!CIM) a.cV[ci.cv_base + lane_id] = co;
}

constexpr int PACK8_D = 8;
template <typename T>
__device__ __forceinline__ void variable_pack8_block(const SweepArgs<T>& a, const ClassInfo& ci, int block) {
    constexpr int H = PACK8_D;
    static_assert(half_stride(5, (int)sizeof(T)) == H && half_stride(8, (int)sizeof(T)) == H, "records of 5..8 values are 8 elements long");
    const int lane_id = block * BLOCK + (int)threadIdx.x;
    if (lane_id >= ci.count) return;
    const int64_t pos = ci.ell_base + lane_id;
// ... 253 lines not shown
                    for (; kk + 24 <= k_hi; kk += 24) {
                        fetch(xc, kk + 16);
                        consume(xa, kk, sel);
                        fetch(xa, kk + 24);
                        consume(xb, kk + 8, sel);
                        fetch(xb, kk + 32);
                        consume(xc, kk + 16, sel);
                    }
                    if (kk < k_hi) consume(xa, kk, sel);
                    if (kk + 8 < k_hi) consume(xb, kk + 8, sel);
                };
                const int n8 = (n + 7) & ~7;
                const int w_lo = ko_w - kt < 0 ? 0 : (ko_w - kt > n8 ? n8 : ((ko_w - kt) & ~7));
                const int w_hi = ko_w + 64 - kt < 0 ? 0 : (ko_w + 64 - kt > n8 ? n8 : ((ko_w + 64 - kt + 7) & ~7));
                run(0, w_lo, std::false_type{});
                run(w_lo, w_hi, std::true_type{});
                run(w_hi, n8, std::false_type{});
                if (MSG && last_k) {
                    const int d = d0 + dd;
                    if (park) {
                        if (real) a.v2f_new[vo + d] = acc;
                    } else {
#pragma unroll
                        for (int q = 0; q < 4; ++q) mreg[q] = d == q ? acc : mreg[q];
                    }
                    if (d == 0 || acc < best_c) {
                        best = d;
                        best_c = acc;
                    }
                }
            }
        };
        if (wave_on) {
            if (msg_role) walk(std::true_type{});
            else walk(std::false_type{});
        }
        d0 = d0n;
        kt = ktn;
    }
    if (!msg_role && wave_on) s_sum[(grp << 6) + lane] = acc;
    lds_barrier();
    if (bel) {
        const int v = hb.var;
        if (a.start && a.init_idx[v] >= 0) {
            best = a.init_idx[v];
            best_c = (T)0;
        }
        a.sel[v] = best;
        a.belief[v] = best_c;
    }
    if (!real) return;
    const T avg = s_sum[(grp << 6) + lane] / (T)D;
    const T* prev = a.v2f_old + vo;
    T* w = a.v2f_new + vo;
    const bool start_sends = (deg == 1 && a.start_mode == MXS_START_LEAFS) || a.start_mode != MXS_START_LEAFS;
    const bool damp = cnt > 0 && a.damp_v;
    bool match = cnt > 0;
    for (int dd = 0; dd < D; ++dd) {
        T mm = park ? w[dd] : (dd == 0 ? mreg[0] : dd == 1 ? mreg[1] : dd == 2 ? mreg[2] : mreg[3]);
        mm = mm - avg;
        if (a.start) {
            w[dd] = start_sends ? mm : (T)0;
            continue;
        }
        const T p = prev[dd];
        if (damp) mm = a.damping * p + ((T)1 - a.damping) * mm;
        if (match) match = comp_match(mm, p, a.stability);
        w[dd] = mm;
    }
    uint8_t out = 1;
    if (a.start) {
        out = 0;
    } else if (match) {
        if (cnt < SAME_COUNT) {
            out = (uint8_t)(cnt + 1);
        } else {
            out = cnt;
            for (int dd = 0; dd < D; ++dd) w[dd] = prev[dd];
        }
    }
    a.cV[k0 + ko] = out;
}

template <typename T, int D, bool P2P = false, int NT = MXS_NT, bool CUT_HALF = true>
__device__ __forceinline__ void sweep_d(const SweepArgs<T>& a, const ClassInfo& ci, int item) {
    if (ci.kind == K_V_PACK) {
        variable_pack<T, D, P2P, NT>(a, ci, item);
        return;
    }
    const int j = item + (int)threadIdx.x;
    if (j >= ci.count) return;
    if (ci.kind == K_F_BIN) factor_binary<T, D, P2P, NT, CUT_HALF>(a, ci, j);
    else if (ci.kind == K_F_UNARY) factor_unary<T, D, NT>(a, ci, j);
}

constexpr unsigned long long HALO_WAIT_TICKS = 500000000ull;
constexpr int HALO_ERR_WORD = 32;
__device__ __forceinline__ void wait_for_halo(uint32_t* flags, uint32_t need, int n_peers, int me) {
    if (threadIdx.x == 0) {
        const unsigned long long t0 = wall_clock64();
        const int n = n_peers > 0 ? n_peers : 1;
        for (int q = 0; q < n; ++q) {
            if (n_peers > 0 && q == me) continue;
            while (__hip_atomic_load(flags + q, __ATOMIC_RELAXED, __HIP_MEMORY_SCOPE_SYSTEM) < need &&
                   __hip_atomic_load(flags + HALO_ERR_WORD, __ATOMIC_RELAXED, __HIP_MEMORY_SCOPE_AGENT) == 0) {
                __builtin_amdgcn_s_sleep(64);
                if (wall_clock64() - t0 > HALO_WAIT_TICKS) {
                    atomicOr(flags + HALO_ERR_WORD, 1u);
                    break;
                }
            }
        }
        if (n_peers > 0) __builtin_amdgcn_fence(__ATOMIC_ACQUIRE, "");
    }
    __syncthreads();
    if (n_peers > 0) {
        __builtin_amdgcn_fence(__ATOMIC_ACQUIRE, "workgroup");
    } else {
        __builtin_amdgcn_fence(__ATOMIC_ACQUIRE, "agent");
    }
}

template <typename T, int DSEL, bool P2P = false, int NT = MXS_NT, bool SCHED = false, bool HUB = false>
__device__ __forceinline__ int sweep_block(const SweepArgs<T>& a) {
    int c = 0, blk = -1;
    if (SCHED || a.sched != nullptr) {
        const uint32_t s = a.sched[blockIdx.x];
        c = (int)(s >> 24);
        blk = (int)(s & 0xffffffu);
    } else {
#pragma unroll
        for (int i = 1; i < MAX_CLASSES; ++i) c += ((int)blockIdx.x >= a.block_base[i]) ? 1 : 0;
    }
    const ClassInfo ci = a.classes[c];
    const int item = (blk >= 0 ? blk : (int)blockIdx.x - ci.block_base) * ci.per_block;
    if (!SCHED && ci.wait_halo && a.halo_flags != nullptr) wait_for_halo(a.halo_flags, a.need_epoch, a.n_peers, a.me);
    if (HUB && ci.kind == K_V_HUB) {
        variable_hub<T>(a, ci, item);
        return ci.kind;
    }
    if (ci.kind == K_F_GEN || ci.kind == K_V_GEN) {
        const int j = item + (int)threadIdx.x;
        if (j >= ci.count) return ci.kind;
        if (ci.kind == K_F_GEN) factor_generic<T>(a, ci, j);
        else variable_generic<T>(a, ci, j);
        return ci.kind;
    }
    if (DSEL != 0) {
        sweep_d<T, (DSEL != 0 ? DSEL : 2), P2P, NT, !SCHED>(a, ci, item);
    } else {
        switch (ci.D) {
            case 2: sweep_d<T, 2, P2P, NT, !SCHED>(a, ci, item); break;
            case 3: sweep_d<T, 3, P2P, NT, !SCHED>(a, ci, item); break;
            case 4: sweep_d<T, 4, P2P, NT, !SCHED>(a, ci, item); break;
            default: break;
        }
    }
    return ci.kind;
}

#ifndef SWEEP_SGPRS
#define SWEEP_SGPRS 104
#endif
template <typename T, int DSEL, int NT = MXS_NT, bool SCHED = false>
__global__ void __launch_bounds__(BLOCK, SWEEP_MIN_WAVES) __attribute__((amdgpu_num_sgpr(SWEEP_SGPRS)))
k_sweep(SweepArgs<T> a) {
    sweep_block<T, DSEL, false, NT, SCHED>(a);
}
template <typename T, int NT = MXS_NT, bool SCHED = false>
__global__ void __launch_bounds__(BLOCK, SWEEP_MIN_WAVES) __attribute__((amdgpu_num_sgpr(80)))
k_sweep_d2(SweepArgs<T> a) {
    sweep_block<T, 2, false, NT, SCHED>(a);
}

template <typename T, int DSEL, int NT = MXS_NT, bool SCHED = false>
__global__ void __launch_bounds__(BLOCK, SWEEP_MIN_WAVES) k_sweep_hub(SweepArgs<T> a) {
    sweep_block<T, DSEL, false, NT, SCHED, true>(a);
}

template <typename T, int DSEL>
__global__ void __launch_bounds__(BLOCK, SWEEP_MIN_WAVES) k_sweep_p2p(SweepArgs<T> a) {
    sweep_block<T, DSEL, true, MXS_NT, false, true>(a);
}

template <typename T, int DSEL, bool HUB>
__device__ __forceinline__ void sweep_timeline(const SweepArgs<T>& a) {
    const int64_t t0 = (int64_t)wall_clock64();
    const int kind = sweep_block<T, DSEL, false, MXS_NT, false, HUB>(a);
    __builtin_amdgcn_s_waitcnt(0);
    const int64_t t1 = (int64_t)wall_clock64();
    if (threadIdx.x == 0) {
        a.timeline[3 * (int64_t)blockIdx.x + 0] = t0;
        a.timeline[3 * (int64_t)blockIdx.x + 1] = t1;
        a.timeline[3 * (int64_t)blockIdx.x + 2] = kind;
    }
}
template <typename T, int DSEL>
__global__ void __launch_bounds__(BLOCK, SWEEP_MIN_WAVES) k_sweep_timeline(SweepArgs<T> a) {
    sweep_timeline<T, DSEL, false>(a);
}
template <typename T, int DSEL>
__global__ void __launch_bounds__(BLOCK) k_sweep_timeline_hub(SweepArgs<T> a) {
    sweep_timeline<T, DSEL, true>(a);
}

constexpr int NARY_MAX_SUMD = 1024;
constexpr int NARY_MAX_R = 1024;
constexpr int NARY_MAX_NJ = NARY_MAX_R / BLOCK;
constexpr int NARY_MAX_ARITY = 6;

template <typename T>
struct OrdKey;
template <>
struct OrdKey<double> {
    typedef unsigned long long U;
    static __device__ __forceinline__ U enc(double x) {
        U b;
        memcpy(&b, &x, 8);
        return (b >> 63) ? ~b : (b | 0x8000000000000000ull);
    }
    static __device__ __forceinline__ double dec(U k) {
        const U b = (k >> 63) ? (k & 0x7fffffffffffffffull) : ~k;
        double x;
        memcpy(&x, &b, 8);
        return x;
    }
};
template <>
struct OrdKey<float> {
    typedef unsigned int U;
    static __device__ __forceinline__ U enc(float x) {
        U b;
        memcpy(&b, &x, 4);
        return (b >> 31) ? ~b : (b | 0x80000000u);
    }
    static __device__ __forceinline__ float dec(U k) {
        const U b = (k >> 31) ? (k & 0x7fffffffu) : ~k;
        float x;
        memcpy(&x, &b, 4);
        return x;
    }
};

template <typename T>
__device__ __forceinline__ T wave_min(T x) {
#pragma unroll
    for (int s = 32; s > 0; s >>= 1) {
        const T y = __shfl(x, (int)((threadIdx.x & 63) ^ s), 64);
        x = y < x ? y : x;
    }
    return x;
}

__device__ __forceinline__ double min2(double x, double y) {
#if defined(__HIP_DEVICE_COMPILE__) && MXS_ASM_MIN
    double r;
    asm("v_min_f64 %0, %1, %2" : "=v"(r) : "v"(x), "v"(y));
    return r;
#else
    return __builtin_fmin(x, y);
#endif
}
__device__ __forceinline__ float min2(float x, float y) { return __builtin_fminf(x, y); }

template <int CTRL, int ROW_MASK>
__device__ __forceinline__ double dpp_mov(double x) {
    int lo = __double2loint(x), hi = __double2hiint(x);
    lo = __builtin_amdgcn_update_dpp(lo, lo, CTRL, ROW_MASK, 0xf, false);
    hi = __builtin_amdgcn_update_dpp(hi, hi, CTRL, ROW_MASK, 0xf, false);
    return __hiloint2double(hi, lo);
}
template <int CTRL, int ROW_MASK>
__device__ __forceinline__ float dpp_mov(float x) {
    int b = __float_as_int(x);
    b = __builtin_amdgcn_update_dpp(b, b, CTRL, ROW_MASK, 0xf, false);
    return __int_as_float(b);
}
typedef unsigned int swap2u __attribute__((ext_vector_type(2)));
template <bool W32, bool SECOND>
__device__ __forceinline__ unsigned int swap_word(unsigned int w) {
    const swap2u r = W32 ? __builtin_amdgcn_permlane32_swap(w, w, false, false)
                         : __builtin_amdgcn_permlane16_swap(w, w, false, false);
// ... 946 lines not shown
```

pydcop_amd/csrc/layout.cpp:

```cpp
#include "layout.h"

#include <algorithm>
#include <cstdlib>
#include <cmath>
#include <cstring>
#include <numeric>
#include <map>
#include <sstream>
#include <tuple>

namespace mxs {

LayoutOptions options_from_params(const mxs_params& p) {
    LayoutOptions o;
    o.word = (p.dtype == MXS_DTYPE_F32) ? 4 : 8;
    const int f = p.layout_flags;
    o.no_specialise = (f & 4) != 0;
    o.sort_by_degree = !(f & 8);
    o.nary = !(f & 16);
    o.sort_factors = MXS_SORT_FACTORS_DEFAULT != 0;
    if (f & 128) o.sort_factors = true;
    if (f & 256) o.sort_factors = false;
    o.factors_second = MXS_FACTORS_SECOND_DEFAULT != 0;
    if (f & 512) o.factors_second = true;
    if (f & 1024) o.factors_second = false;
    o.schedule = MXS_SCHEDULE_DEFAULT != 0;
    if (f & 4096) o.schedule = true;
    if (f & 2048) o.schedule = false;
    o.compact_tables = MXS_COMPACT_TABLES_DEFAULT != 0;
    if (f & 16384) o.compact_tables = true;
    if (f & 8192) o.compact_tables = false;
    o.box = !(f & 32768);
    o.half_cut = !(f & 65536);
    o.pack8_fused = !(f & 2097152);
    o.pack8 = !(f & 1048576);
    o.bin2 = !(f & 524288);
    o.merge_types = !(f & 16777216);
    o.nary_multi = !(f & 33554432);
    o.small = !(f & 8388608);
    o.hub = !(f & 4194304);
    o.tile_bytes = -1;
    if (f & 131072) o.tile_bytes = MXS_TILE_BYTES;
    if (f & 262144) o.tile_bytes = 0;
    if (!(f & (131072 | 262144)))
        if (const char* tb = std::getenv("MAXSUM_TILE_KB")) {
            char* end = nullptr;
            const long long kb = std::strtoll(tb, &end, 10);
            if (end != tb && *end == '\0' && kb >= 0) o.tile_bytes = (int64_t)kb * 1024;
        }
    return o;
}

namespace {

struct FKey {
    int kind, D;
    int cut = 0;
    int own = 0;
    bool operator<(const FKey& o) const {
        return cut != o.cut ? cut < o.cut : kind != o.kind ? kind < o.kind : D != o.D ? D < o.D : own < o.own;
    }
    bool operator==(const FKey& o) const { return kind == o.kind && D == o.D && cut == o.cut && own == o.own; }
};

std::string validate(const mxs_graph& g) {
    std::ostringstream err;
    if (g.n_vars < 0 || g.n_factors < 0 || g.n_edges < 0) return "negative size";
    if (g.n_vars && (!g.dom_size || !g.var_cost || !g.var_rowptr)) return "null variable arrays";
    if (g.n_factors && (!g.factor_rowptr || !g.table_off || !g.tables)) return "null factor arrays";
    if (g.n_edges && (!g.edge_var || !g.var_edges)) return "null edge arrays";
    for (int32_t v = 0; v < g.n_vars; ++v)
        if (g.dom_size[v] < 1 || g.dom_size[v] > 4096) {
            err << "variable " << v << ": domain size " << g.dom_size[v] << " not in 1..4096";
            return err.str();
        }
    if (g.n_factors) {
        if (g.factor_rowptr[0] != 0 || g.factor_rowptr[g.n_factors] != g.n_edges)
            return "factor_rowptr does not span the edges";
        if (g.table_off[0] != 0) return "table_off[0] must be 0";
    } else if (g.n_edges) {
        return "edges without factors";
    }
    for (int32_t f = 0; f < g.n_factors; ++f) {
        const int32_t e0 = g.factor_rowptr[f], e1 = g.factor_rowptr[f + 1];
        if (e1 <= e0) { err << "factor " << f << " has no variable"; return err.str(); }
        if (e1 - e0 > MAX_ARITY) { err << "factor " << f << ": arity > " << MAX_ARITY << " not supported"; return err.str(); }
        int64_t size = 1;
        for (int32_t e = e0; e < e1; ++e) {
            const int32_t v = g.edge_var[e];
            if (v < 0 || v >= g.n_vars) { err << "edge " << e << ": variable out of range"; return err.str(); }
            for (int32_t e2 = e0; e2 < e; ++e2)
                if (g.edge_var[e2] == v) { err << "factor " << f << " lists variable " << v << " twice"; return err.str(); }
            size *= g.dom_size[v];
            if (size > ((int64_t)1 << 40)) { err << "factor " << f << ": table too large"; return err.str(); }
        }
        if (g.table_off[f + 1] - g.table_off[f] != size) {
            err << "factor " << f << ": table_off inconsistent with scope (" << size << " entries expected)";
            return err.str();
        }
    }
    if (g.n_vars) {
        if (g.var_rowptr[0] != 0 || g.var_rowptr[g.n_vars] != g.n_edges)
            return "var_rowptr does not span the edges";
        std::vector<uint8_t> seen(g.n_edges, 0);
        for (int32_t v = 0; v < g.n_vars; ++v) {
            if (g.var_rowptr[v + 1] < g.var_rowptr[v]) return "var_rowptr not monotone";
            for (int32_t k = g.var_rowptr[v]; k < g.var_rowptr[v + 1]; ++k) {
                const int32_t e = g.var_edges[k];
                if (e < 0 || e >= g.n_edges || seen[e] || g.edge_var[e] != v) {
                    err << "var_edges[" << k << "] inconsistent";
                    return err.str();
                }
                seen[e] = 1;
            }
            if (g.init_idx && g.init_idx[v] >= g.dom_size[v]) return "init_idx out of the domain";
        }
    }
    return "";
}

}

int narrowest_tab_type(const double* v, int64_t n, int word) {
    bool i8 = true, i16 = true, f32 = true;
    for (int64_t k = 0; k < n; ++k) {
        const double x = v[k];
        const bool integral = std::isfinite(x) && x == std::floor(x) && !(x == 0.0 && std::signbit(x));
        if (!integral || std::fabs(x) > 127.0) i8 = false;
        if (!integral || std::fabs(x) > 32767.0) i16 = false;
        if (!((double)(float)x == x || (x != x))) f32 = false;
        if (x != x) i8 = i16 = false;
        if (!i16 && !f32) break;
    }
    if (i8) return TAB_I8;
    if (i16) return TAB_I16;
    if (f32 && word == 8) return TAB_F32;
    return TAB_FULL;
}

void encode_tab_record(const double* v, int entries, int t, uint8_t* dst) {
    for (int k = 0; k < entries; ++k) {
        if (t == TAB_I8) {
            const int8_t x = (int8_t)v[k];
            std::memcpy(dst + k, &x, 1);
        } else if (t == TAB_I16) {
            const int16_t x = (int16_t)v[k];
            std::memcpy(dst + 2 * k, &x, 2);
        } else {
            const float x = (float)v[k];
            std::memcpy(dst + 4 * k, &x, 4);
        }
    }
}

void encode_tab_entry(double v, int t, int word, uint8_t* dst) {
    if (t != TAB_FULL) {
        encode_tab_record(&v, 1, t, dst);
    } else if (word == 8) {
        std::memcpy(dst, &v, 8);
    } else {
        const float x = (float)v;
        std::memcpy(dst, &x, 4);
    }
}

std::string build_layout(const mxs_graph& g, const mxs_params& p, Layout& L) {
    {
        std::string e = validate(g);
        if (!e.empty()) return e;
    }
    if (p.mode != MXS_MODE_MIN && p.mode != MXS_MODE_MAX) return "invalid mode";
    if (p.damping_nodes < 0 || p.damping_nodes > 3) return "invalid damping_nodes";
    if (p.start_messages < 0 || p.start_messages > 2) return "invalid start_messages";
    if (p.dtype != MXS_DTYPE_F64 && p.dtype != MXS_DTYPE_F32) return "invalid dtype";

    L = Layout();
    L.opt = options_from_params(p);
    L.n_vars = g.n_vars;
    L.n_factors = g.n_factors;
    L.n_edges = g.n_edges;
    L.is_max = (p.mode == MXS_MODE_MAX);
    const double sign = L.is_max ? -1.0 : 1.0;
    const int nV = g.n_vars, nF = g.n_factors, nE = g.n_edges;

    std::vector<int> vsort(nV);
    for (int v = 0; v < nV; ++v) {
        const int deg = g.var_rowptr[v + 1] - g.var_rowptr[v];
        const int D = g.dom_size[v];
        const bool own = !g.var_owned || g.var_owned[v];
        int kind, sub;
        if (!own) { kind = 90; sub = 0; }
        else if (deg == 0) { kind = 80; sub = 0; }
        else if (!L.opt.no_specialise && D >= 2 && D <= MAX_REG_D && deg <= MAX_PACK_DEG) {
            kind = K_V_PACK; sub = D;
        } else if (!L.opt.no_specialise && L.opt.pack8 && D > MAX_REG_D && D <= MAX_PACK8_D && deg <= MAX_PACK_DEG) {
            kind = K_V_PACK8;
            sub = 0;
        } else if (!L.opt.no_specialise && D <= 256 && (int64_t)deg * D <= 1024 && deg <= 256 &&
                   !(L.opt.hub && D <= MAX_PACK8_D && deg > MAX_PACK_DEG)) {
            kind = K_V_WIDE;
            sub = 0;
        } else if (!L.opt.no_specialise && L.opt.hub) {
            kind = K_V_HUB;
// ... 88 lines not shown
            const bool o0 = g.var_owned[g.edge_var[e0]] != 0, o1 = g.var_owned[g.edge_var[e0 + 1]] != 0;
            k.own = (o0 && !o1) ? 1 : ((!o0 && o1) ? 2 : 0);
        }
        fkey[f] = k;
    }
    if (L.opt.bin2 && L.opt.compact_tables && L.opt.merge_types) {
        struct Stat { int64_t entries[4] = {0, 0, 0, 0}; int to[4] = {0, 1, 2, 3}; };
        std::map<std::tuple<int, int, int>, Stat> stat;
        auto bin2_key = [&](int f, std::tuple<int, int, int>& key, int& t) {
            const FKey& k = fkey[f];
            if (k.kind != K_F_NARY || !is_bin2(nary_code_box(k.D >> 2))) return false;
            key = std::make_tuple(k.D >> 2, k.cut, k.own);
            t = k.D & 3;
            return true;
        };
        std::tuple<int, int, int> key;
        int t = 0;
        for (int f = 0; f < nF; ++f)
            if (bin2_key(f, key, t)) stat[key].entries[t] += g.table_off[f + 1] - g.table_off[f];
        auto bytes_of = [&](int tt) { return tt == TAB_FULL ? (int64_t)L.opt.word : (int64_t)tab_elem_bytes(tt); };
        bool any = false;
        for (auto& kv : stat) {
            Stat& st = kv.second;
            for (int n = TAB_I8; n > TAB_FULL; --n) {
                if (!st.entries[n]) continue;
                int w = n - 1;
                while (w >= TAB_FULL && !st.entries[w]) --w;
                if (w < TAB_FULL) continue;
                if (st.entries[n] * (bytes_of(w) - bytes_of(n)) > BIN2_MERGE_BYTES) continue;
                st.entries[w] += st.entries[n];
                st.entries[n] = 0;
                for (int q = TAB_FULL; q <= TAB_I8; ++q)
                    if (st.to[q] == n) st.to[q] = w;
                any = true;
            }
        }
        if (any)
            for (int f = 0; f < nF; ++f)
                if (bin2_key(f, key, t)) fkey[f].D = (fkey[f].D & ~3) | stat[key].to[t];
    }
    L.factor_i2e.resize(nF);
    std::iota(L.factor_i2e.begin(), L.factor_i2e.end(), 0);
    std::vector<int64_t> floc(nF, 0);
    if (L.opt.sort_factors)
        for (int f = 0; f < nF; ++f)
            if (g.factor_rowptr[f + 1] > g.factor_rowptr[f]) floc[f] = L.var_e2i[g.edge_var[g.factor_rowptr[f]]];
    if (L.opt.sort_factors && L.opt.tile_bytes != 0 && nV > 0) {
        const int64_t tile = L.opt.tile_bytes > 0 ? L.opt.tile_bytes : MXS_TILE_BYTES;
        const int64_t per_var = std::max<int64_t>(1, (int64_t)nE * 3 * L.opt.word / std::max(1, nV));
        const int64_t W = std::max<int64_t>(256, tile / per_var);
        const int64_t NB = (nV + W - 1) / W;
        bool on = NB > 1;
        if (on && L.opt.tile_bytes < 0) {
            int64_t n_bin = 0, n_near = 0, bytes = 0;
            for (int f = 0; f < nF; ++f) {
                const int e0 = g.factor_rowptr[f];
                int64_t cells = 1;
                for (int e = e0; e < g.factor_rowptr[f + 1]; ++e) cells *= g.dom_size[g.edge_var[e]];
                bytes += cells * L.opt.word;
                if (fkey[f].kind != K_F_BIN) continue;
                const int64_t b0 = L.var_e2i[g.edge_var[e0]] / W, b1 = L.var_e2i[g.edge_var[e0 + 1]] / W;
                ++n_bin;
                n_near += b0 == b1;
            }
            for (int e = 0; e < nE; ++e) bytes += 6 * (int64_t)g.dom_size[g.edge_var[e]] * L.opt.word + 8;
            for (int v = 0; v < nV; ++v) bytes += (int64_t)g.dom_size[v] * L.opt.word + 8 + L.opt.word;
            on = n_bin > 0 && 2 * n_near < n_bin && (L.opt.word == 4 || bytes <= MXS_TILE_RESIDENT_BYTES);
        }
        if (on)
            for (int f = 0; f < nF; ++f) {
                const int e0 = g.factor_rowptr[f];
                if (fkey[f].kind != K_F_BIN) continue;
                const int64_t v0 = L.var_e2i[g.edge_var[e0]], v1 = L.var_e2i[g.edge_var[e0 + 1]];
                floc[f] = ((v0 / W) * NB + v1 / W) * (int64_t)nV + v0;
            }
        L.tiled = on;
    }
    std::stable_sort(L.factor_i2e.begin(), L.factor_i2e.end(), [&](int a, int b) {
        return fkey[a] < fkey[b] || (fkey[a] == fkey[b] && floc[a] < floc[b]);
    });

    L.factor_e2i.resize(nF);
    for (int fi = 0; fi < nF; ++fi) L.factor_e2i[L.factor_i2e[fi]] = fi;
    L.f_tab_base.assign(nF, 0);
    L.f_tab_stride.assign(nF, 1);
    L.f_ctab_off.assign(nF, -1);
    L.f_class.assign(nF, -1);
    L.f_ndesc.assign(nF, -1);
    L.f_tab_type.assign(nF, (uint8_t)TAB_FULL);

    L.edge_i2e.resize(nE);
    L.edge_e2i.resize(nE);
    L.frowptr.assign(nF + 1, 0);
    L.f2v_off.resize(nE);
    L.v2f_off.assign(nE, 0);
    L.edge_dom.resize(nE);
    L.edge_half.resize(nE);
    L.edge_gen_factor.assign(nE, -1);
    L.edge_fcim.assign(nE, 0);
    L.edge_vcim.assign(nE, 0);
    {
        int ei = 0;
        int64_t off = 0;
        const int align = 32 / L.opt.word;
        for (int fi = 0; fi < nF;) {
            const FKey key = fkey[L.factor_i2e[fi]];
            int fj = fi;
            while (fj < nF && fkey[L.factor_i2e[fj]] == key) ++fj;
            off = (off + align - 1) / align * align;
            const bool split = key.kind == K_F_BIN;
            const int Hc = split ? L.half(key.D) : 0;
            const int64_t half_len = split ? ((int64_t)(fj - fi) * Hc + align - 1) / align * align : 0;
            for (int f2 = fi; f2 < fj; ++f2) {
                const int f = L.factor_i2e[f2];
                L.frowptr[f2] = ei;
                for (int e = g.factor_rowptr[f]; e < g.factor_rowptr[f + 1]; ++e, ++ei) {
                    L.edge_i2e[ei] = e;
                    L.edge_e2i[e] = ei;
                    const int D = g.dom_size[g.edge_var[e]];
                    const int H = L.half(D);
                    L.edge_dom[ei] = D;
                    L.edge_half[ei] = H;
                    int64_t at = off;
                    if (split) {
                        at = off + (int64_t)(e - g.factor_rowptr[f]) * half_len + (int64_t)(f2 - fi) * Hc;
                    } else {
                        const int bytes = H * L.opt.word;
                        const int al = (bytes % 16 == 0 ? 16 : bytes % 8 == 0 ? 8 : L.opt.word) / L.opt.word;
                        off = (off + al - 1) / al * al;
                        at = off;
                        off += H;
                    }
                    if (at > ((int64_t)1 << 31) - 8192) return "message buffer exceeds 2^31 elements";
                    L.f2v_off[ei] = (int32_t)at;
                }
            }
            if (split) off += 2 * half_len;
            if (off > ((int64_t)1 << 31) - 8192) return "message buffer exceeds 2^31 elements";
            fi = fj;
        }
        L.frowptr[nF] = ei;
        off = (off + align - 1) / align * align;
        L.null_f2v = off;
        off += std::max(L.half(MAX_REG_D), L.half(MAX_PACK8_D));
        L.f2v_elems = off;
    }

    L.vrowptr.assign(nV + 1, 0);
    L.vslot_edge.resize(nE);
    L.vslot_f2v.resize(nE);
    L.vslot_v2f.assign(nE, 0);
    L.vslot_cv.resize(nE);
    L.vdom.resize(nV);
    L.vhalf.resize(nV);
    L.vcost_off.resize(nV);
    L.init_idx.assign(nV, -1);
    L.owned.assign(nV, 1);
    L.edge_var_int.resize(nE);
    {
        std::vector<int64_t> ext_cost_off(nV + 1, 0);
        for (int v = 0; v < nV; ++v) ext_cost_off[v + 1] = ext_cost_off[v] + g.dom_size[v];
        L.var_cost.resize(ext_cost_off[nV]);
        L.eval_var_cost.resize(ext_cost_off[nV]);
        int k = 0;
        int64_t coff = 0;
        for (int vi = 0; vi < nV; ++vi) {
            const int v = L.var_i2e[vi];
            L.vrowptr[vi] = k;
            for (int kk = g.var_rowptr[v]; kk < g.var_rowptr[v + 1]; ++kk, ++k) {
                const int ei = L.edge_e2i[g.var_edges[kk]];
                L.vslot_edge[k] = ei;
                L.vslot_f2v[k] = L.f2v_off[ei];
                L.edge_var_int[ei] = vi;
            }
            L.vdom[vi] = g.dom_size[v];
            L.vhalf[vi] = L.half(g.dom_size[v]);
            L.vcost_off[vi] = coff;
            for (int d = 0; d < g.dom_size[v]; ++d) {
                L.var_cost[coff + d] = sign * g.var_cost[ext_cost_off[v] + d];
                L.eval_var_cost[coff + d] = (g.eval_var_cost ? g.eval_var_cost : g.var_cost)[ext_cost_off[v] + d];
            }
            coff += g.dom_size[v];
            if (g.init_idx) L.init_idx[vi] = g.init_idx[v];
            if (g.var_owned) L.owned[vi] = g.var_owned[v] ? 1 : 0;
        }
        L.vrowptr[nV] = k;
    }

    L.eval_tab_off.assign(nF + 1, 0);
    for (int fi = 0; fi < nF; ++fi) {
        const int f = L.factor_i2e[fi];
        L.eval_tab_off[fi + 1] = L.eval_tab_off[fi] + (g.table_off[f + 1] - g.table_off[f]);
    }
    L.fowned.assign(nF, 1);
    if (g.factor_owned)
        for (int fi = 0; fi < nF; ++fi) L.fowned[fi] = g.factor_owned[L.factor_i2e[fi]] ? 1 : 0;
    L.eval_tables.resize(L.eval_tab_off[nF]);
    L.tables.resize(L.eval_tab_off[nF]);
    for (int fi = 0; fi < nF; ++fi) {
        const int f = L.factor_i2e[fi];
        std::copy(g.tables + g.table_off[f], g.tables + g.table_off[f + 1],
                  L.eval_tables.begin() + L.eval_tab_off[fi]);
    }
    const bool second = g.var_owned != nullptr && L.opt.factors_second;
    auto sweep_class = [&](int cls, int per_block, int cut = 0) {
        L.classes[cls].per_block = per_block;
        (cut ? L.sweep_order2 : L.sweep_order).push_back(cls);
    };
    for (int fi = 0; fi < nF;) {
        const FKey key = fkey[L.factor_i2e[fi]];
        int fj = fi;
        while (fj < nF && fkey[L.factor_i2e[fj]] == key) ++fj;
        const int n = fj - fi;
        ClassInfo ci{};
        ci.kind = key.kind;
        ci.D = key.kind == K_F_NARY ? 0 : key.D;
        ci.H = ci.D ? L.half(ci.D) : 0;
        ci.first = fi;
        ci.count = n;
        ci.edge_base = L.frowptr[fi];
        ci.f2v_base = nE ? L.f2v_off[L.frowptr[fi]] : 0;
        ci.f2v_base1 = key.kind == K_F_BIN ? L.f2v_off[L.frowptr[fi] + 1] : 0;
        ci.own_pos = key.own;
        ci.tab_base = L.eval_tab_off[fi];
        const int cls = (int)L.classes.size();
        if (key.kind == K_F_UNARY || key.kind == K_F_BIN) {
            const int entries = (key.kind == K_F_UNARY) ? key.D : key.D * key.D;
            for (int j = 0; j < n; ++j) {
                const double* src = L.eval_tables.data() + L.eval_tab_off[fi + j];
                for (int k = 0; k < entries; ++k)
                    L.tables[ci.tab_base + (int64_t)k * n + j] = sign * src[k];
                L.f_tab_base[fi + j] = ci.tab_base + j;
                L.f_tab_stride[fi + j] = n;
            }
            if (ci.H > ci.D)
                for (int e = L.frowptr[fi]; e < L.frowptr[fj]; ++e) L.edge_fcim[e] = 1;
            if (L.opt.compact_tables) {
                const int64_t lo = L.eval_tab_off[fi], hi = L.eval_tab_off[fj];
                const int t = narrowest_tab_type(L.eval_tables.data() + lo, hi - lo, L.opt.word);
                if (t != TAB_FULL) {
                    ci.tab_type = t;
                    ci.ctab_rec = tab_record_bytes(entries, tab_elem_bytes(t));
                    ci.ctab_base = (int64_t)((L.ctables.size() + 255) / 256 * 256);
                    L.ctables.resize((size_t)(ci.ctab_base + (int64_t)n * ci.ctab_rec), 0);
                    for (int j = 0; j < n; ++j) {
                        L.f_tab_type[fi + j] = (uint8_t)t;
                        L.f_ctab_off[fi + j] = ci.ctab_base + (int64_t)j * ci.ctab_rec;
                        encode_tab_record(L.eval_tables.data() + L.eval_tab_off[fi + j], entries, t,
                                          L.ctables.data() + L.f_ctab_off[fi + j]);
                    }
                }
            }
            for (int j = 0; j < n; ++j) L.f_class[fi + j] = cls;
            L.classes.push_back(ci);
            sweep_class(cls, BLOCK, key.cut || second);
        } else {
            const int gen_base = (int)L.fgen.size();
            for (int j = 0; j < n; ++j) {
                const int f2 = fi + j;
                FactorGen fg{L.frowptr[f2], L.frowptr[f2 + 1] - L.frowptr[f2], L.eval_tab_off[f2]};
                for (int e = L.frowptr[f2]; e < L.frowptr[f2 + 1]; ++e)
                    L.edge_gen_factor[e] = gen_base + j;
                L.fgen.push_back(fg);
                L.f_tab_base[f2] = L.eval_tab_off[f2];
                L.f_tab_stride[f2] = 1;
                for (int64_t k = L.eval_tab_off[f2]; k < L.eval_tab_off[f2 + 1]; ++k)
                    L.tables[k] = sign * L.eval_tables[k];
            }
            if (key.kind == K_F_GEN) {
                ci.count = L.frowptr[fj] - L.frowptr[fi];
                L.classes.push_back(ci);
                sweep_class(cls, BLOCK, key.cut || second);
            } else {
                const int code = key.D / 4, t = key.D % 4;
                NaryLaunch nl{(code / 256) % 16, (code / 16) % 16, (code % 16) * 64, (int32_t)L.ndesc.size(), n, key.cut, t,
                              code / 4096};
                for (int j = 0; j < n; ++j) {
                    const int f2 = fi + j;
                    NaryDesc d{};
                    d.tab_off = L.eval_tab_off[f2];
                    d.edge_base = L.frowptr[f2];
                    d.arity = L.frowptr[f2 + 1] - L.frowptr[f2];
                    for (int i = 0; i < NARY_DESC_ARITY; ++i) {
                        const bool in = i < d.arity;
                        d.dom[i] = in ? L.edge_dom[d.edge_base + i] : 1;
                        d.f2v_off[i] = in ? L.f2v_off[d.edge_base + i] : 0;
                        d.v2f_off[i] = 0;
                        d.magic[i] = d.dom[i] > 1 ? (uint32_t)((((uint64_t)1 << 32) + d.dom[i] - 1) / d.dom[i]) : 0u;
                    }
                    if (t != TAB_FULL || is_bin2(nl.box) || is_small(nl.box)) {
                        const NaryPlace pl = nary_place(nl, d, L.opt.word);
                        const int64_t ne = L.eval_tab_off[f2 + 1] - L.eval_tab_off[f2];
                        const int64_t al = is_bin2(nl.box) ? 16 : 256;
                        const int64_t at = (int64_t)((L.ctables.size() + al - 1) / al * al);
                        L.ctables.resize((size_t)(at + nary_place_bytes(pl, d.dom[0])), 0);
                        const double* src = L.eval_tables.data() + L.eval_tab_off[f2];
                        for (int64_t k = 0; k < ne; ++k)
                            encode_tab_entry(src[k], t, L.opt.word, L.ctables.data() + at + nary_place_pos(pl, k));
                        L.f_tab_type[f2] = (uint8_t)t;
                        L.f_ctab_off[f2] = at;
                        d.tab_off = at;
                    }
                    L.f_ndesc[f2] = (int32_t)L.ndesc.size();
                    L.ndesc.push_back(d);
                }
                L.nary_launches.push_back(nl);
            }
        }
        fi = fj;
    }

    L.n_cv = nE;
    for (int k = 0; k < nE; ++k) L.vslot_cv[k] = k;
    int64_t voff = 0;
    for (int vi = 0; vi < nV;) {
        const int v0 = L.var_i2e[vi];
        const int key = vsort[v0] / 4096;
        int vj = vi;
        while (vj < nV && vsort[L.var_i2e[vj]] / 4096 == key) ++vj;
        const int kind = key / 1024, sub = key % 1024;
        ClassInfo ci{};
        ci.first = vi;
        ci.count = vj - vi;
        ci.cost_base = L.vcost_off[vi];
        bool swept = true;
        {
            const int64_t align = 32 / L.opt.word;
            voff = (voff + align - 1) / align * align;
        }
        if (kind == K_V_PACK) {
            ci.kind = K_V_PACK;
            ci.D = sub;
            ci.H = L.half(ci.D);
        } else if (kind == K_V_PACK8) {
            ci.kind = K_V_PACK8;
            ci.D = MAX_PACK8_D;
            ci.H = L.half(ci.D);
            ci.uni_D = L.vdom[vi];
            for (int w = vi; w < vj; ++w)
                if (L.vdom[w] != ci.uni_D) ci.uni_D = 0;
        } else if (kind == K_V_GEN) {
            ci.kind = K_V_GEN;
        } else if (kind == K_V_HUB) {
            ci.kind = K_V_HUB;
            std::vector<int> order(vj - vi);
            std::iota(order.begin(), order.end(), vi);
            std::stable_sort(order.begin(), order.end(), [&](int x, int y) {
                return (int64_t)(L.vrowptr[x + 1] - L.vrowptr[x]) * L.vdom[x] > (int64_t)(L.vrowptr[y + 1] - L.vrowptr[y]) * L.vdom[y];
            });
            ci.first = (int32_t)L.hub_blocks.size();
            for (int w : order) {
                const int deg = L.vrowptr[w + 1] - L.vrowptr[w];
                const uint32_t row = 8u + (uint32_t)(deg < HUB_TILE ? ((deg + 7) & ~7) : HUB_TILE);
                for (int ko0 = 0; ko0 <= deg; ko0 += HUB_EDGES)
                    L.hub_blocks.push_back(HubBlock{w, ko0, L.vdom[w], deg, L.vrowptr[w],
                                                    (uint32_t)((((uint64_t)1 << 32) + row - 1) / row), L.vcost_off[w]});
            }
            ci.count = (int32_t)L.hub_blocks.size() - ci.first;
        } else if (kind == K_V_WIDE) {
            ci.kind = K_V_WIDE;
            for (int w = vi; w < vj;) {
                const int D = L.vdom[w];
                WideBlock wb{w, 0, D, L.vrowptr[w], 0, (uint32_t)((((uint64_t)1 << 32) + D - 1) / D), L.vcost_off[w]};
                while (w < vj && L.vdom[w] == D) {
                    const int deg = L.vrowptr[w + 1] - L.vrowptr[w];
                    if (wb.n_vars > 0 && ((int64_t)(wb.n_slots + deg) * D > WIDE_CAPB || wb.n_slots + deg > WIDE_MAX_SLOTS ||
                                          wb.n_vars + 1 > WIDE_MAX_VARS || (int64_t)(wb.n_vars + 1) * D > WIDE_MAX_COSTS))
                        break;
                    wb.n_vars += 1;
                    wb.n_slots += deg;
                    ++w;
                }
                L.wide_blocks.push_back(wb);
            }
        } else if (kind == 80) {
            ci.kind = K_V_GEN;
            ci.start_only = 1;
        } else {
            swept = false;
        }
        if (ci.kind == K_V_PACK || ci.kind == K_V_PACK8) {
            ci.ell_base = (int64_t)L.vell.size();
            ci.cv_base = L.n_cv;
            ci.v2f_base = voff;
            int64_t lanes = 0;
            for (int w = vi; w < vj;) {
                const int deg = L.vrowptr[w + 1] - L.vrowptr[w];
                int w2 = w;
                while (w2 < vj && L.vrowptr[w2 + 1] - L.vrowptr[w2] == deg) ++w2;
                const int per_wave = 64 / deg;
                for (int x = w; x < w2; x += per_wave) {
                    const int nv = std::min(per_wave, w2 - x);
                    L.vwave.push_back(WaveMeta{x, (int32_t)((uint32_t)deg | ((uint32_t)nv << 8) |
                                                          ((uint32_t)((32768 + deg - 1) / deg) << 16))});
                    for (int lane = 0; lane < 64; ++lane) {
                        const int var = lane / deg, k = lane % deg;
                        if (var < nv) {
                            const int ks = L.vrowptr[x + var] + k;
                            L.vell.push_back(L.vslot_f2v[ks]);
                            L.vslot_cv[ks] = ci.cv_base + lanes;
                            L.vslot_v2f[ks] = (int32_t)(ci.v2f_base + lanes * ci.H);
                            if (ci.H > ci.D) L.edge_vcim[L.vslot_edge[ks]] = 1;
                        } else {
                            L.vell.push_back(-1);
                        }
                        ++lanes;
                    }
                }
                w = w2;
            }
            ci.count = (int32_t)lanes;
            L.n_cv += lanes;
            voff += lanes * ci.H;
        } else {
            for (int w = vi; w < vj; ++w)
                for (int k = L.vrowptr[w]; k < L.vrowptr[w + 1]; ++k) {
                    L.vslot_v2f[k] = (int32_t)voff;
                    voff += L.vhalf[w];
                }
        }
        if (voff > ((int64_t)1 << 31) - 8192) return "message buffer exceeds 2^31 elements";
        if (swept) {
            const int cls = (int)L.classes.size();
            L.classes.push_back(ci);
            if (ci.kind == K_V_WIDE) {
                L.classes[cls].per_block = 1;
                L.wide_classes.push_back(cls);
            } else if (ci.kind == K_V_PACK8) {
                L.classes[cls].per_block = BLOCK;
                L.pack8_classes.push_back(cls);
            } else {
                sweep_class(cls, ci.kind == K_V_HUB ? 1 : BLOCK);
            }
        }
        vi = vj;
    }
    L.v2f_elems = voff;
    for (int k = 0; k < nE; ++k) L.v2f_off[L.vslot_edge[k]] = L.vslot_v2f[k];
    for (NaryDesc& d : L.ndesc)
        for (int i = 0; i < (d.arity & 255); ++i) d.v2f_off[i] = L.v2f_off[d.edge_base + i];

    {
        auto prio = [&](int c) {
            switch (L.classes[c].kind) {
                case K_V_HUB: return -1;
                case K_V_GEN: return 0;
                case K_F_GEN: return 1;
                case K_V_PACK: return 2;
                default: return 4;
            }
        };
        std::stable_sort(L.sweep_order.begin(), L.sweep_order.end(),
                         [&](int x, int y) { return prio(x) < prio(y); });
        if (p.layout_flags & (32 | 64)) {
            std::vector<int32_t> keep;
            for (int c : L.sweep_order) {
                const int k = L.classes[c].kind;
                const bool is_var = k == K_V_GEN || k == K_V_PACK || k == K_V_HUB;
                if (((p.layout_flags & 32) && !is_var) || ((p.layout_flags & 64) && is_var)) keep.push_back(c);
            }
            L.sweep_order = keep;
            if (p.layout_flags & 64) L.sweep_order2.clear();
        }
        if ((int)L.sweep_order.size() > MAX_CLASSES || (int)L.sweep_order2.size() > MAX_CLASSES)
            return "too many kernel classes";
        int nb = 0;
        for (int c : L.sweep_order) {
            ClassInfo& ci = L.classes[c];
            ci.block_base = nb;
            nb += (ci.count + ci.per_block - 1) / ci.per_block;
        }
        L.n_blocks_sweep = nb;
        nb = 0;
        for (int c : L.sweep_order2) {
            ClassInfo& ci = L.classes[c];
            ci.block_base = nb;
            nb += (ci.count + ci.per_block - 1) / ci.per_block;
        }
        L.n_blocks_sweep2 = nb;
        for (int c : L.sweep_order2) L.classes[c].wait_halo = 1;
        if (!L.sweep_order2.empty() && L.sweep_order.size() + L.sweep_order2.size() <= (size_t)MAX_CLASSES) {
            for (int c : L.sweep_order) L.fused_block_base.push_back(L.classes[c].block_base);
            for (int c : L.sweep_order2) L.fused_block_base.push_back(L.n_blocks_sweep + L.classes[c].block_base);
            L.n_blocks_fused = L.n_blocks_sweep + L.n_blocks_sweep2;
        }
        for (int c : L.sweep_order)
            if (!L.classes[c].start_only) L.sweep_regular = true;
        if (L.opt.schedule && L.n_blocks_sweep >= 2 && !(p.layout_flags & (32 | 64))) {
            struct Blk { double key; int prio; uint32_t code; };
            std::vector<Blk> blks;
            std::vector<uint32_t> hub_blks;
            std::vector<Blk> long_blks;
            constexpr int LONG_PACK_DEG = 24;
            blks.reserve(L.n_blocks_sweep);
            auto first_var_of_factor = [&](int fi) { return (double)L.edge_var_int[L.frowptr[fi]]; };
            for (size_t slot = 0; slot < L.sweep_order.size(); ++slot) {
                const ClassInfo& ci = L.classes[L.sweep_order[slot]];
                const int nbc = (ci.count + ci.per_block - 1) / ci.per_block;
                if (nbc >= (1 << 24)) { blks.clear(); break; }
                for (int j = 0; j < nbc; ++j) {
                    const int64_t i0 = (int64_t)j * ci.per_block;
                    const int64_t i1 = std::min<int64_t>(ci.count, i0 + ci.per_block) - 1;
                    double k0 = 0, k1 = 0;
                    int prio = 1;
                    if (ci.kind == K_V_HUB) {
                        hub_blks.push_back((uint32_t)(slot << 24) | (uint32_t)j);
                        continue;
                    }
                    switch (ci.kind) {
                        case K_V_PACK: {
                            const WaveMeta& w0 = L.vwave[(ci.ell_base + i0) >> 6];
                            const WaveMeta& w1 = L.vwave[(ci.ell_base + i1) >> 6];
                            if ((int)((uint32_t)w1.deg_nv & 255u) >= LONG_PACK_DEG) {
                                long_blks.push_back(Blk{-(double)((uint32_t)w1.deg_nv & 255u), 0, (uint32_t)(slot << 24) | (uint32_t)j});
                                continue;
                            }
                            k0 = w0.first_var;
                            k1 = w1.first_var + (int)(((uint32_t)w1.deg_nv >> 8) & 255u) - 1;
                            prio = 0;
                            break;
                        }
// ... 58 lines not shown
```

pydcop_amd/csrc/layout.h:

```cpp
#pragma once
#include <cstdint>
#include <string>
#include <vector>

#include "../../include/maxsum_gpu.h"

namespace mxs {

enum Kind : int32_t {
    K_F_UNARY = 1,
    K_F_BIN = 2,
    K_F_GEN = 3,
    K_F_NARY = 4,
    K_V_PACK = 5,
    K_V_GEN = 6,
    K_V_WIDE = 7,
    K_V_PACK8 = 8,
    K_V_HUB = 9,
};

#ifndef MXS_BLOCK
#define MXS_BLOCK 256
#endif
constexpr int BLOCK = MXS_BLOCK;

#ifndef MXS_FACTORS_SECOND_DEFAULT
#define MXS_FACTORS_SECOND_DEFAULT 0
#endif
#ifndef MXS_SORT_FACTORS_DEFAULT
#define MXS_SORT_FACTORS_DEFAULT 1
#endif
#ifndef MXS_SCHEDULE_DEFAULT
#define MXS_SCHEDULE_DEFAULT 1
#endif
#ifndef MXS_TILE_BYTES
#define MXS_TILE_BYTES (512 << 10)
#endif
#ifndef MXS_TILE_RESIDENT_BYTES
#define MXS_TILE_RESIDENT_BYTES (256ll << 20)
#endif
#ifndef MXS_COMPACT_TABLES_DEFAULT
#define MXS_COMPACT_TABLES_DEFAULT 1
#endif
enum TabType : int32_t { TAB_FULL = 0, TAB_F32 = 1, TAB_I16 = 2, TAB_I8 = 3 };
constexpr int tab_elem_bytes(int t) { return t == TAB_I8 ? 1 : t == TAB_I16 ? 2 : t == TAB_F32 ? 4 : 0; }
constexpr int tab_record_bytes(int entries, int elem) {
    const int b = entries * elem;
    return b <= 4 ? 4 : b <= 8 ? 8 : (b + 15) / 16 * 16;
}
constexpr int nary_slot_bytes(int nj, int elem) {
    const int b = nj * elem;
    return b <= 4 ? 4 : b <= 8 ? 8 : 16;
}
constexpr int64_t nary_packed_pos(int64_t d0, int64_t q, int nt, int slot, int elem) {
    return (d0 * nt + q % nt) * slot + (q / nt) * elem;
}
constexpr int BOX_SHAPES[][3] = {{2, 2, 2}, {3, 3, 3}, {4, 4, 4}, {6, 6, 6}};
constexpr int BOX_N_SHAPES = 4;
constexpr int BOX_WAVES = 4;
constexpr int BOX_MAX_SUMD = 128;
constexpr int BOX_MAX_WORDS = 64;
constexpr bool box_record_fits(int b0, int b1, int b2, int elem) {
    const int words = (b0 * b1 * b2 * elem + 3) / 4;
    return words <= BOX_MAX_WORDS || (words <= 2 * BOX_MAX_WORDS - 8 && words % 4 == 0 && b0 % 2 == 0);
}
constexpr int box_rec_words(int entries, int elem) { return (entries * elem + 3) / 4; }
constexpr bool box_pow2(int x) { return x > 0 && (x & (x - 1)) == 0; }
constexpr int box_lanes(int d, int b) {
    int l = 1;
    while (l * b < d) l *= 2;
    return l;
}
#ifndef MXS_BOX_MAX_PAD_PCT
#define MXS_BOX_MAX_PAD_PCT 240
#endif
constexpr int nary_box_shape(int d0, int d1, int d2, int elem) {
    int best = 0;
    long best_cells = 0;
    for (int s = 0; s < BOX_N_SHAPES; ++s) {
        const int b0 = BOX_SHAPES[s][0], b1 = BOX_SHAPES[s][1], b2 = BOX_SHAPES[s][2];
        const int l0 = box_lanes(d0, b0), l1 = box_lanes(d1, b1), l2 = box_lanes(d2, b2);
        if (l0 * l1 * l2 != 64) continue;
        if (l0 > 16 || l1 > 16 || l2 > 16) continue;
        if (l0 * b0 + l1 * b1 + l2 * b2 > BOX_MAX_SUMD) continue;
        if (!box_record_fits(b0, b1, b2, elem)) continue;
        const long cells = 64L * b0 * b1 * b2;
        if (cells * 100 > (long)MXS_BOX_MAX_PAD_PCT * d0 * d1 * d2) continue;
        if (!best || cells < best_cells) {
            best = s + 1;
            best_cells = cells;
        }
    }
    return best;
}
struct Bin2Shape {
    int L0, L1, B0, B1;
};
constexpr Bin2Shape BIN2_SHAPES[] = {
    {2, 2, 2, 2},  {2, 2, 3, 3},  {2, 2, 4, 4},
    {4, 4, 3, 3},  {4, 4, 4, 4},  {4, 4, 5, 5},  {4, 4, 6, 6},  {4, 4, 8, 8},
    {8, 8, 5, 5},  {8, 8, 6, 6},  {8, 8, 8, 8},
    {16, 1, 1, 1}, {16, 1, 2, 1}, {16, 1, 4, 1},
};
constexpr int BIN2_N_SHAPES = (int)(sizeof(BIN2_SHAPES) / sizeof(BIN2_SHAPES[0]));
constexpr int BIN2_BASE = 32;
constexpr int BIN2_WAVES = 4;
constexpr int BIN2_MAX_D = 64;
constexpr int SMALL_BASE = 64;
constexpr int SMALL_P = 5;
constexpr int SMALL_WAVES = 4;
constexpr bool is_small(int box) { return box >= SMALL_BASE; }
constexpr int small_lead(int arity) { return arity == 3 ? 1 : 2; }
constexpr int small_group(int arity) { return arity == 3 ? 8 : 32; }
constexpr int small_pow(int e) {
    int r = 1;
    for (int i = 0; i < e; ++i) r *= SMALL_P;
// ... 30 lines not shown
    int32_t dom[6];
    int32_t multi;
};
constexpr int64_t nary_place_pos(const NaryPlace& p, int64_t k) {
    if (p.box == 0) return p.multi ? k * p.elem : nary_packed_pos(k / p.R, k % p.R, p.nt, p.slot, p.elem);
    if (is_small(p.box)) {
        int x[6] = {0, 0, 0, 0, 0, 0};
        int64_t rem = k;
        for (int i = p.arity - 1; i >= 0; --i) {
            x[i] = (int)(rem % p.dom[i]);
            rem /= p.dom[i];
        }
        const int L = small_lead(p.arity);
        int64_t lane = 0, e = 0;
        for (int i = 0; i < L; ++i) lane = lane * SMALL_P + x[i];
        for (int i = L; i < p.arity; ++i) e = e * SMALL_P + x[i];
        return lane * small_rec_bytes(p.arity, p.elem) + e * p.elem;
    }
    if (is_bin2(p.box)) {
        const Bin2Shape sh = BIN2_SHAPES[p.box - BIN2_BASE];
        const int64_t piece = bin2_piece_bytes(sh.B1, p.elem), x1 = k % p.d1, x0 = k / p.d1;
        return x0 * (sh.L1 * piece) + (x1 / sh.B1) * piece + (x1 % sh.B1) * p.elem;
    }
    const int b0 = BOX_SHAPES[p.box - 1][0], b1 = BOX_SHAPES[p.box - 1][1], b2 = BOX_SHAPES[p.box - 1][2];
    const int64_t x2 = k % p.d2, x1 = (k / p.d2) % p.d1, x0 = k / ((int64_t)p.d1 * p.d2);
    const int l1n = box_lanes(p.d1, b1), l2n = box_lanes(p.d2, b2);
    const int64_t lane = ((x0 / b0) * l1n + x1 / b1) * l2n + x2 / b2;
    const int64_t byte = (((x0 % b0) * b1 + x1 % b1) * b2 + x2 % b2) * p.elem;
    const int words = box_rec_words(b0 * b1 * b2, p.elem), full = words / 4, rest = words % 4;
    const int64_t piece = byte / 16;
    return piece < full ? (piece * 64 + lane) * 16 + byte % 16
                        : (int64_t)full * 1024 + lane * rest * 4 + byte % 16;
}
constexpr int64_t nary_place_bytes(const NaryPlace& p, int D0) {
    if (p.box == 0) return p.multi ? ((int64_t)D0 * p.R * p.elem + 15) / 16 * 16 + 16 : (int64_t)D0 * p.nt * p.slot;
    if (is_small(p.box)) return ((int64_t)small_pow(small_lead(p.arity)) * small_rec_bytes(p.arity, p.elem) + 15) / 16 * 16;
    if (is_bin2(p.box)) {
        const Bin2Shape sh = BIN2_SHAPES[p.box - BIN2_BASE];
        return ((int64_t)D0 * sh.L1 * bin2_piece_bytes(sh.B1, p.elem) + 15) / 16 * 16;
    }
    const int* b = BOX_SHAPES[p.box - 1];
    return (int64_t)64 * 4 * box_rec_words(b[0] * b[1] * b[2], p.elem);
}
constexpr int NUM_XCD = 8;
constexpr int MAX_REG_D = 4;
constexpr int MAX_ARITY = MXS_MAX_ARITY;
constexpr int MAX_PACK_DEG = 64;
constexpr int MAX_PACK8_D = 8;
constexpr int MAX_CLASSES = 24;

#ifndef MXS_TIGHT
#define MXS_TIGHT 1
#endif
constexpr int half_stride(int D, int word) {
    const int bytes = D * word;
    if (MXS_TIGHT && bytes <= 32 && D <= 4) return D;
    const int padded = bytes <= 8 ? 8 : bytes <= 16 ? 16 : (bytes + 31) / 32 * 32;
    return padded / word;
}

struct ClassInfo {
    int32_t kind;
    int32_t D;
    int32_t H;
    int32_t wait_halo;
    int32_t first;
    int32_t count;
    int32_t edge_base;
    int32_t start_only;
    int64_t f2v_base;
    int64_t tab_base;
    int64_t cost_base;
    int32_t block_base;
    int32_t per_block;
    int64_t ell_base;
    int64_t cv_base;
    int64_t v2f_base;
    int64_t f2v_base1;
    int32_t tab_type;
    int32_t ctab_rec;
    int64_t ctab_base;
    int32_t own_pos;
    int32_t uni_D;
};

constexpr int NARY_DESC_ARITY = 6;
struct NaryDesc {
    int64_t tab_off;
    int32_t edge_base;
    int32_t arity;
    int32_t dom[NARY_DESC_ARITY];
    int32_t v2f_off[NARY_DESC_ARITY];
    int32_t f2v_off[NARY_DESC_ARITY];
    uint32_t magic[NARY_DESC_ARITY];
};

#ifndef MXS_WIDE_TPB
#define MXS_WIDE_TPB 256
#endif
constexpr int WIDE_TPB = MXS_WIDE_TPB;
constexpr int WIDE_CAPB = 4 * WIDE_TPB;
constexpr int WIDE_MAX_SLOTS = WIDE_TPB;
constexpr int WIDE_MAX_VARS = 128;
constexpr int WIDE_MAX_COSTS = WIDE_TPB * 3 / 2;
constexpr int WIDE_MAX_D = 256;
struct WideBlock {
    int32_t first_var;
    int32_t n_vars;
    int32_t D;
    int32_t slot0;
    int32_t n_slots;
    uint32_t magic;
    int64_t cost_off;
};

struct HubBlock {
    int32_t var;
    int32_t ko0;
    int32_t D, deg;
    int32_t slot0;
    uint32_t magic;
    int64_t cost_off;
};
constexpr int HUB_CW = MXS_BLOCK / 128;
constexpr int HUB_EDGES = 64 * HUB_CW;
constexpr int HUB_TILE = 2048;
constexpr int HUB_LDS = 2560;

struct NaryLaunch {
    int32_t arity, nj;
    int32_t threads;
    int32_t first;
    int32_t count;
    int32_t cut;
    int32_t tab_type;
    int32_t box;
};
inline NaryPlace nary_place(const NaryLaunch& nl, const NaryDesc& d, int word = 0) {
    NaryPlace p{};
    p.box = nl.box;
    p.elem = nl.tab_type == TAB_FULL ? word : tab_elem_bytes(nl.tab_type);
    p.nt = nl.threads;
    p.slot = nary_slot_bytes(nl.nj > 0 ? nl.nj : 1, p.elem);
    p.multi = nl.box == 0 && nl.nj == NARY_NJ_MULTI;
    int64_t R = 1;
    for (int i = 1; i < (d.arity & 255); ++i) R *= d.dom[i];
    p.R = (int32_t)R;
    p.d1 = d.dom[1];
    p.d2 = d.dom[2];
    p.arity = d.arity & 255;
    for (int i = 0; i < 6; ++i) p.dom[i] = d.dom[i];
    return p;
}
constexpr int nary_group_code(int box, int arity, int nj, int waves) { return ((box * 16 + arity) * 16 + nj) * 16 + waves; }
constexpr int nary_code_box(int code) { return code >> 12; }
constexpr int64_t BIN2_MERGE_BYTES = (int64_t)8 << 20;
constexpr int nary_classic_nj(int64_t R) { return (int)((R + BLOCK - 1) / BLOCK); }
constexpr int nary_classic_waves(int64_t R) { return (int)(((R + nary_classic_nj(R) - 1) / nary_classic_nj(R) + 63) / 64); }

struct WaveMeta {
    int32_t first_var;
    int32_t deg_nv;
};

struct FactorGen {
    int32_t edge_base;
    int32_t arity;
    int64_t tab_off;
};

struct LayoutOptions {
    int word = 8;
    bool no_specialise = false;
    bool sort_by_degree = true;
    bool nary = true;
    bool sort_factors = false;
    bool factors_second = false;
    bool schedule = false;
    bool compact_tables = false;
    bool box = true;
    bool pack8_fused = true;
    bool pack8 = true;
    bool small = true;
    bool nary_multi = true;
    bool merge_types = true;
    bool bin2 = true;
    bool hub = true;
    bool half_cut = true;
    int64_t tile_bytes = -1;
};

struct Layout {
    LayoutOptions opt;
    int32_t n_vars = 0, n_factors = 0, n_edges = 0;
    bool is_max = false;

    std::vector<int32_t> factor_i2e, var_i2e, edge_i2e;
    std::vector<int32_t> factor_e2i;
    std::vector<int64_t> f_tab_base;
    std::vector<int32_t> f_tab_stride;
    std::vector<int32_t> var_e2i, edge_e2i;

    std::vector<ClassInfo> classes;
    std::vector<int32_t> sweep_order;
    std::vector<int32_t> sweep_order2;
    std::vector<int32_t> fused_block_base;
    int32_t n_blocks_fused = 0;
    int32_t n_blocks_sweep2 = 0;
    int32_t n_blocks_sweep = 0;
    std::vector<uint32_t> sched;
    bool sweep_regular = false;
    std::vector<NaryDesc> ndesc;
    std::vector<NaryLaunch> nary_launches;
    std::vector<int32_t> pack8_classes;
    std::vector<int32_t> wide_classes;
    std::vector<WideBlock> wide_blocks;
    std::vector<HubBlock> hub_blocks;

    std::vector<int32_t> f2v_off;
    std::vector<int32_t> v2f_off;
    std::vector<int32_t> edge_dom;
    std::vector<int32_t> edge_half;
    std::vector<int32_t> edge_gen_factor;
    std::vector<int32_t> edge_var_int;
    std::vector<uint8_t> edge_fcim, edge_vcim;
    int64_t f2v_elems = 0, v2f_elems = 0;
    int64_t null_f2v = 0;

    std::vector<FactorGen> fgen;
    std::vector<double> tables;
    std::vector<uint8_t> ctables;
    std::vector<int64_t> f_ctab_off;
    std::vector<int32_t> f_class;
    std::vector<int32_t> f_ndesc;
    std::vector<uint8_t> f_tab_type;
    std::vector<int32_t> vrowptr;
    std::vector<int32_t> vslot_edge;
    std::vector<int32_t> vslot_f2v;
    std::vector<int32_t> vslot_v2f;
    std::vector<int64_t> vslot_cv;
    std::vector<int32_t> vell;
    std::vector<WaveMeta> vwave;
    int64_t n_cv = 0;
    int dsel = 0;
    std::vector<int32_t> vdom;
    std::vector<int32_t> vhalf;
    std::vector<int64_t> vcost_off;
    std::vector<double> var_cost;
    std::vector<int32_t> init_idx;
    std::vector<uint8_t> owned;
    std::vector<uint8_t> fowned;

    std::vector<int64_t> eval_tab_off;
    std::vector<double> eval_tables;
    std::vector<double> eval_var_cost;
    std::vector<int32_t> frowptr;

    int64_t algorithmic_bytes = 0;
    bool tiled = false;

    int half(int D) const { return half_stride(D, opt.word); }
};

std::string build_layout(const mxs_graph& g, const mxs_params& p, Layout& out);
int narrowest_tab_type(const double* v, int64_t n, int word);
void encode_tab_record(const double* v, int entries, int t, uint8_t* dst);
void encode_tab_entry(double v, int t, int word, uint8_t* dst);
LayoutOptions options_from_params(const mxs_params& p);

}
```

pydcop_amd/engine.py:

```python
import ctypes as C
import os
import sys
from typing import Optional, Tuple

import numpy as np

from .graph import CGraph, CParams, FlatGraph, Params

_HERE = os.path.dirname(os.path.abspath(__file__))
DEFAULT_LIB = os.environ.get("MAXSUM_HIP_LIB") or os.path.join(_HERE, "csrc", "libmaxsum_hip.so")
_TEST_ENGINES = set()


def register_test_engine(path: str, make_default: bool = False):
    global DEFAULT_LIB
    _TEST_ENGINES.add(os.path.realpath(path))
    if make_default:
        DEFAULT_LIB = os.path.realpath(path)

ABI_SYMBOLS = (
    "mxs_device_count", "mxs_create", "mxs_reset", "mxs_run", "mxs_run_timed", "mxs_run_reps",
    "mxs_run_async", "mxs_sync", "mxs_cycle_count", "mxs_get_assignment",
    "mxs_get_messages", "mxs_eval_cost", "mxs_cycle_bytes", "mxs_halo_setup",
    "mxs_halo_buffers", "mxs_halo_bind", "mxs_step_compute", "mxs_step_pack", "mxs_step_unpack", "mxs_stream",
    "mxs_comm_unique_id", "mxs_comm_init", "mxs_comm_exchange", "mxs_run_sharded", "mxs_shard_mode",
    "mxs_peer_export", "mxs_peer_connect",
    "mxs_debug_timeline", "mxs_update_factor_table", "mxs_destroy", "mxs_last_error", "mxs_version",
    "mxs_build_kind", "mxs_set_state", "mxs_set_parent_table", "mxs_slice_factor",
    "mxs_table_storage", "mxs_factor_order", "mxs_factor_kernels", "mxs_variable_kernels",
    "mxs_amaxsum_create", "mxs_amaxsum_reset", "mxs_amaxsum_run", "mxs_amaxsum_status",
    "mxs_amaxsum_generation_sizes", "mxs_amaxsum_get_assignment", "mxs_amaxsum_get_messages",
    "mxs_amaxsum_eval_cost", "mxs_amaxsum_update_factor_table", "mxs_amaxsum_destroy",
    "mxs_mgm_create", "mxs_mgm_reset", "mxs_mgm_set_value_rank", "mxs_mgm_run", "mxs_mgm_rounds", "mxs_mgm_get_state",
    "mxs_mgm_eval_cost", "mxs_mgm_destroy",
    "mxs_dsa_create", "mxs_dsa_reset", "mxs_dsa_set_value_rank", "mxs_dsa_run", "mxs_dsa_cycles", "mxs_dsa_get_state",
    "mxs_dsa_eval_cost", "mxs_dsa_destroy",
    "mxs_dsa_create_replicas", "mxs_dsa_replicas", "mxs_dsa_get_state_replica", "mxs_dsa_replica_costs",
    "mxs_dsa_track_best", "mxs_dsa_get_best",
    "mxs_dpop_create", "mxs_dpop_solve", "mxs_dpop_get_state", "mxs_dpop_eval_cost", "mxs_dpop_stats",
    "mxs_dpop_util_dims", "mxs_dpop_get_util", "mxs_dpop_destroy",
    "mxs_gdba_create", "mxs_gdba_reset", "mxs_gdba_run", "mxs_gdba_rounds", "mxs_gdba_get_state",
    "mxs_gdba_get_modifiers", "mxs_gdba_eval_cost", "mxs_gdba_destroy",
    "mxs_dba_create", "mxs_dba_reset", "mxs_dba_run", "mxs_dba_rounds", "mxs_dba_finished", "mxs_dba_get_state",
    "mxs_dba_get_weights", "mxs_dba_mask_bytes", "mxs_dba_eval_cost", "mxs_dba_destroy",
)

MGM2_SYMBOLS = (
    "mxs_mgm2_create", "mxs_mgm2_reset", "mxs_mgm2_run", "mxs_mgm2_rounds", "mxs_mgm2_get_state", "mxs_mgm2_eval_cost",
    "mxs_mgm2_destroy",
)


MAX_PEERS = 8


class PeerInfo(C.Structure):
    _fields_ = [("qualifies", C.c_int32), ("rank", C.c_int32), ("ghost_len", C.c_int64),
                ("recv_at", C.c_int64 * MAX_PEERS), ("recv_len", C.c_int64 * MAX_PEERS),
                ("ghost_handle", C.c_uint8 * 64), ("flag_handle", C.c_uint8 * 64),
                ("pid", C.c_int64), ("ghost_ptr", C.c_uint64), ("flag_ptr", C.c_uint64)]


class MaxSumGpuError(RuntimeError):
    """A C-ABI call failed (the message comes from mxs_last_error)."""


_libs = {}
_hip_runtime = None


def hip_runtime_path() -> str:
    env = os.environ.get("MAXSUM_HIP_RUNTIME")
    if env:
        return env
    torch = sys.modules.get("torch")
    if torch is not None:
        cand = os.path.join(os.path.dirname(torch.__file__), "lib", "libamdhip64.so")
        if os.path.exists(cand):
            return cand
    rocm = os.environ.get("ROCM_PATH", "/opt/rocm")
    for name in ("libamdhip64.so", "libamdhip64.so.7", "libamdhip64.so.6"):
        cand = os.path.join(rocm, "lib", name)
        if os.path.exists(cand):
            return cand
    return "libamdhip64.so"


def _load_hip_runtime():
    global _hip_runtime
    if _hip_runtime is None:
        path = hip_runtime_path()
        try:
            _hip_runtime = (path, C.CDLL(path, mode=C.RTLD_GLOBAL))
        except OSError as e:
            raise MaxSumGpuError(f"cannot load the HIP runtime {path}: {e}. "
                                 "maxsum_gpu has no CPU fallback.") from e
    return _hip_runtime[0]


def load_library(path: Optional[str] = None) -> C.CDLL:
    path = os.path.realpath(path or DEFAULT_LIB)
    if path in _libs:
        return _libs[path]
    if not os.path.exists(path):
        raise MaxSumGpuError(
            f"{path} not found: build it with `python -c 'import __graft_entry__ as g; g.build()'` "
            "(hipcc --offload-arch=gfx950). maxsum_gpu has no CPU fallback.")
    registered_test = path in _TEST_ENGINES
    if not registered_test:
        if not os.path.basename(path).startswith("libmaxsum_hip"):
            raise MaxSumGpuError(
                f"{path} is not a build of libmaxsum_hip: maxsum_gpu has no CPU fallback and loads "
# ... 16 lines not shown
        "mxs_sync": ([vp], C.c_int),
        "mxs_cycle_count": ([vp, C.POINTER(i64)], C.c_int),
        "mxs_get_assignment": ([vp, vp, vp], C.c_int),
        "mxs_get_messages": ([vp, vp, vp, vp, vp], C.c_int),
        "mxs_eval_cost": ([vp, vp, C.c_double, C.POINTER(C.c_double), C.POINTER(i64)], C.c_int),
        "mxs_set_state": ([vp, vp, vp, vp, vp, vp, vp, i64], C.c_int),
        "mxs_set_parent_table": ([vp, i32, vp, i32, vp, vp], C.c_int),
        "mxs_slice_factor": ([vp, i32, vp], C.c_int),
        "mxs_table_storage": ([vp, vp, C.POINTER(i64)], C.c_int),
        "mxs_amaxsum_create": ([C.POINTER(CGraph), C.POINTER(CParams), i32, C.POINTER(vp)], C.c_int),
        "mxs_amaxsum_reset": ([vp], C.c_int),
        "mxs_amaxsum_update_factor_table": ([vp, i32, vp, i64], C.c_int),
        "mxs_amaxsum_run": ([vp, i32, C.POINTER(i64)], C.c_int),
        "mxs_amaxsum_status": ([vp, C.POINTER(i32), C.POINTER(i64), C.POINTER(i64)], C.c_int),
        "mxs_amaxsum_generation_sizes": ([vp, vp, i32, C.POINTER(i32)], C.c_int),
        "mxs_amaxsum_get_assignment": ([vp, vp, vp], C.c_int),
        "mxs_amaxsum_get_messages": ([vp] + [vp] * 8, C.c_int),
        "mxs_amaxsum_eval_cost": ([vp, vp, C.c_double, C.POINTER(C.c_double), C.POINTER(i64)], C.c_int),
        "mxs_amaxsum_destroy": ([vp], C.c_int),
        "mxs_mgm_create": ([C.POINTER(CGraph), C.POINTER(CParams), vp, i32, C.POINTER(vp)], C.c_int),
        "mxs_mgm_reset": ([vp], C.c_int),
        "mxs_mgm_set_value_rank": ([vp, vp], C.c_int),
        "mxs_mgm_run": ([vp, i32], C.c_int),
        "mxs_mgm_rounds": ([vp, C.POINTER(i64)], C.c_int),
        "mxs_mgm_get_state": ([vp, vp, vp, vp, vp, vp], C.c_int),
        "mxs_mgm_eval_cost": ([vp, vp, C.c_double, C.POINTER(C.c_double), C.POINTER(i64)], C.c_int),
        "mxs_mgm_destroy": ([vp], C.c_int),
        "mxs_mgm2_create": ([C.POINTER(CGraph), C.POINTER(CParams), vp, C.c_double, i32, C.c_uint64, i32,
                             C.POINTER(vp)], C.c_int),
        "mxs_mgm2_reset": ([vp], C.c_int),
        "mxs_mgm2_run": ([vp, i32], C.c_int),
        "mxs_mgm2_rounds": ([vp, C.POINTER(i64)], C.c_int),
        "mxs_mgm2_get_state": ([vp, vp, vp, vp], C.c_int),
        "mxs_mgm2_eval_cost": ([vp, vp, C.c_double, C.POINTER(C.c_double), C.POINTER(i64)], C.c_int),
        "mxs_mgm2_destroy": ([vp], C.c_int),
        "mxs_dsa_create": ([C.POINTER(CGraph), C.POINTER(CParams), i32, C.c_double, i32, C.c_uint64, i32,
                            C.POINTER(vp)], C.c_int),
        "mxs_dsa_reset": ([vp], C.c_int),
        "mxs_dsa_set_value_rank": ([vp, vp], C.c_int),
        "mxs_dsa_run": ([vp, i32], C.c_int),
        "mxs_dsa_cycles": ([vp, C.POINTER(i64)], C.c_int),
        "mxs_dsa_get_state": ([vp, vp, vp], C.c_int),
        "mxs_dsa_eval_cost": ([vp, vp, C.c_double, C.POINTER(C.c_double), C.POINTER(i64)], C.c_int),
        "mxs_dsa_destroy": ([vp], C.c_int),
        "mxs_dsa_create_replicas": ([C.POINTER(CGraph), C.POINTER(CParams), i32, C.c_double, i32, vp, i32, i32,
                                     C.POINTER(vp)], C.c_int),
        "mxs_dsa_replicas": ([vp, C.POINTER(i32)], C.c_int),
        "mxs_dsa_get_state_replica": ([vp, i32, vp, vp], C.c_int),
        "mxs_dsa_replica_costs": ([vp, C.c_double, vp, vp], C.c_int),
        "mxs_dsa_track_best": ([vp, i32, C.c_double], C.c_int),
        "mxs_dsa_get_best": ([vp, i32, C.POINTER(i32), C.POINTER(i64), C.POINTER(C.c_double), C.POINTER(i64), vp], C.c_int),
        "mxs_dpop_create": ([C.POINTER(CGraph), C.POINTER(CParams), vp, vp, vp, i64, i32, i32, C.POINTER(vp)], C.c_int),
        "mxs_dpop_solve": ([vp], C.c_int),
        "mxs_dpop_get_state": ([vp, vp, vp], C.c_int),
        "mxs_dpop_eval_cost": ([vp, vp, C.c_double, C.POINTER(C.c_double), C.POINTER(i64)], C.c_int),
        "mxs_dpop_stats": ([vp, vp, i32], C.c_int),
        "mxs_dpop_util_dims": ([vp, i32, vp, C.POINTER(i32)], C.c_int),
        "mxs_dpop_get_util": ([vp, i32, vp, i64], C.c_int),
        "mxs_dpop_destroy": ([vp], C.c_int),
        "mxs_gdba_create": ([C.POINTER(CGraph), C.POINTER(CParams), vp, vp, i32, i32, i32, C.c_uint64, i64, i32,
                             C.POINTER(vp)], C.c_int),
        "mxs_gdba_reset": ([vp], C.c_int),
        "mxs_gdba_run": ([vp, i32], C.c_int),
        "mxs_gdba_rounds": ([vp, C.POINTER(i64)], C.c_int),
        "mxs_gdba_get_state": ([vp, vp, vp, vp, vp, vp], C.c_int),
        "mxs_gdba_get_modifiers": ([vp, i32, vp, i64, C.POINTER(i64)], C.c_int),
        "mxs_gdba_eval_cost": ([vp, vp, C.c_double, C.POINTER(C.c_double), C.POINTER(i64)], C.c_int),
        "mxs_gdba_destroy": ([vp], C.c_int),
        "mxs_dba_create": ([C.POINTER(CGraph), C.POINTER(CParams), vp, C.c_double, i32, C.c_uint64, i64, i32,
                            C.POINTER(vp)], C.c_int),
        "mxs_dba_reset": ([vp], C.c_int),
        "mxs_dba_run": ([vp, i32], C.c_int),
        "mxs_dba_rounds": ([vp, C.POINTER(i64)], C.c_int),
        "mxs_dba_finished": ([vp, C.POINTER(i32), C.POINTER(i64)], C.c_int),
        "mxs_dba_get_state": ([vp, vp, vp, vp, vp, vp, vp, vp, vp], C.c_int),
        "mxs_dba_get_weights": ([vp, vp], C.c_int),
        "mxs_dba_mask_bytes": ([vp, C.POINTER(i64)], C.c_int),
        "mxs_dba_eval_cost": ([vp, vp, C.c_double, C.POINTER(C.c_double), C.POINTER(i64)], C.c_int),
        "mxs_dba_destroy": ([vp], C.c_int),
        "mxs_cycle_bytes": ([vp, C.POINTER(i64), C.POINTER(i32)], C.c_int),
        "mxs_factor_order": ([vp, C.POINTER(i32)], C.c_int),
        "mxs_factor_kernels": ([vp, vp], C.c_int),
        "mxs_variable_kernels": ([vp, vp], C.c_int),
        "mxs_halo_setup": ([vp, vp, i64, vp, i64], C.c_int),
        "mxs_halo_buffers": ([vp, C.POINTER(vp), C.POINTER(i64), C.POINTER(vp), C.POINTER(i64)], C.c_int),
        "mxs_halo_bind": ([vp, vp, vp], C.c_int),
        "mxs_step_compute": ([vp], C.c_int),
        "mxs_step_pack": ([vp], C.c_int),
        "mxs_step_unpack": ([vp], C.c_int),
        "mxs_stream": ([vp, C.POINTER(vp)], C.c_int),
        "mxs_comm_unique_id": ([C.c_char_p, vp], C.c_int),
        "mxs_comm_init": ([vp, C.c_char_p, i32, i32, vp, vp, vp], C.c_int),
        "mxs_comm_exchange": ([vp], C.c_int),
        "mxs_run_sharded": ([vp, i32], C.c_int),
        "mxs_shard_mode": ([vp, C.POINTER(i32), C.POINTER(i32)], C.c_int),
        "mxs_peer_export": ([vp, i32, i32, vp, vp, C.POINTER(PeerInfo)], C.c_int),
        "mxs_peer_connect": ([vp, C.POINTER(PeerInfo)], C.c_int),
        "mxs_debug_timeline": ([vp, vp, i32, C.POINTER(i32)], C.c_int),
        "mxs_update_factor_table": ([vp, i32, vp, i64], C.c_int),
        "mxs_destroy": ([vp], C.c_int),
        "mxs_last_error": ([], C.c_char_p),
        "mxs_version": ([], i32),
        "mxs_build_kind": ([], i32),
    }
    for name, (argtypes, restype) in protos.items():
        fn = getattr(lib, name)
        fn.argtypes = argtypes
        fn.restype = restype
    _libs[path] = lib
    return lib


def rccl_path() -> str:
    env = os.environ.get("MAXSUM_RCCL_LIB")
    if env:
        return env
    torch = sys.modules.get("torch")
    if torch is not None:
        cand = os.path.join(os.path.dirname(torch.__file__), "lib", "librccl.so")
        if os.path.exists(cand):
            return cand
    rocm = os.environ.get("ROCM_PATH", "/opt/rocm")
    for name in ("librccl.so", "librccl.so.1"):
        cand = os.path.join(rocm, "lib", name)
        if os.path.exists(cand):
            return cand
    return "librccl.so"


UNIQUE_ID_BYTES = 128


def comm_unique_id(lib_path: Optional[str] = None, rccl: Optional[str] = None) -> bytes:
    lib = load_library(lib_path)
    buf = C.create_string_buffer(UNIQUE_ID_BYTES)
    rc = lib.mxs_comm_unique_id((rccl or rccl_path()).encode(), C.cast(buf, C.c_void_p))
    if rc != 0:
        raise MaxSumGpuError(f"maxsum_gpu error {rc}: {lib.mxs_last_error().decode()}")
    return buf.raw


def peer_qualifies(info: bytes) -> bool:
    return bool(PeerInfo.from_buffer_copy(info).qualifies)


def device_count(lib_path: Optional[str] = None) -> int:
    n = C.c_int32(0)
    load_library(lib_path).mxs_device_count(C.byref(n))
    return int(n.value)


class MaxSumEngine:

    def __init__(self, graph: FlatGraph, params: Optional[Params] = None, device: int = 0,
                 lib_path: Optional[str] = None):
        self._h = None
        self._lib = load_library(lib_path)
        self.graph = graph
        self.params = params or Params()
        cg, cp = graph.to_c(), self.params.to_c()
        h = C.c_void_p()
        self._check(self._lib.mxs_create(C.byref(cg), C.byref(cp), int(device), C.byref(h)))
        self._h = h

    def _check(self, rc: int):
        if rc != 0:
# ... 21 lines not shown
    def sync(self):
        self._check(self._lib.mxs_sync(self._h))

    @property
    def cycle_count(self) -> int:
        n = C.c_int64(0)
        self._check(self._lib.mxs_cycle_count(self._h, C.byref(n)))
        return int(n.value)

    def assignment(self) -> Tuple[np.ndarray, np.ndarray]:
        idx = np.empty(self.graph.n_vars, dtype=np.int32)
        belief = np.empty(self.graph.n_vars, dtype=np.float64)
        self._check(self._lib.mxs_get_assignment(self._h, idx.ctypes.data, belief.ctypes.data))
        return idx, belief

    def messages(self):
        nm, ne = int(self.graph.msg_off[-1]), self.graph.n_edges
        v2f, f2v = np.empty(nm), np.empty(nm)
        cv, cf = np.empty(ne, dtype=np.uint8), np.empty(ne, dtype=np.uint8)
        self._check(self._lib.mxs_get_messages(self._h, v2f.ctypes.data, f2v.ctypes.data,
                                               cv.ctypes.data, cf.ctypes.data))
        return v2f, f2v, cv, cf

    def state(self) -> dict:
        v2f, f2v, cv, cf = self.messages()
        idx, belief = self.assignment()
        return {"v2f": v2f, "f2v": f2v, "count_v2f": cv, "count_f2v": cf, "idx": idx, "belief": belief,
                "cycles": self.cycle_count}

    def set_state(self, v2f=None, f2v=None, count_v2f=None, count_f2v=None, idx=None, belief=None,
                  cycles: Optional[int] = None):
        nm, ne, nv = int(self.graph.msg_off[-1]), self.graph.n_edges, self.graph.n_vars

        def arr(a, dtype, n, what):
            if a is None:
                return None, None
            a = np.ascontiguousarray(a, dtype=dtype)
            if a.shape != (n,):
                raise ValueError(f"{what} must have {n} entries")
            return a, a.ctypes.data
        keep = []
        ptrs = []
        for a, dt, n, what in ((v2f, np.float64, nm, "v2f"), (f2v, np.float64, nm, "f2v"),
                               (count_v2f, np.uint8, ne, "count_v2f"), (count_f2v, np.uint8, ne, "count_f2v"),
                               (idx, np.int32, nv, "idx"), (belief, np.float64, nv, "belief")):
            a, p = arr(a, dt, n, what)
            keep.append(a)
            ptrs.append(p)
        cyc = self.cycle_count if cycles is None else int(cycles)
        self._check(self._lib.mxs_set_state(self._h, *ptrs, cyc))

    def eval_cost(self, idx=None, infinity: float = float("inf")) -> Tuple[float, int]:
        cost, viol = C.c_double(0), C.c_int64(0)
        p = None
        if idx is not None:
            idx = np.ascontiguousarray(idx, dtype=np.int32)
            if idx.shape[0] != self.graph.n_vars:
                raise ValueError("assignment must have one index per variable")
            p = idx.ctypes.data
        self._check(self._lib.mxs_eval_cost(self._h, p, float(infinity), C.byref(cost), C.byref(viol)))
        return float(cost.value), int(viol.value)

    def cycle_bytes(self) -> Tuple[int, int]:
        b, n = C.c_int64(0), C.c_int32(0)
        self._check(self._lib.mxs_cycle_bytes(self._h, C.byref(b), C.byref(n)))
        return int(b.value), int(n.value)

    def factor_order(self) -> str:
        t = C.c_int32(0)
        self._check(self._lib.mxs_factor_order(self._h, C.byref(t)))
        return "tiled" if t.value else "by_first_variable"

    def factor_kernels(self) -> dict:
        n = (C.c_int64 * 7)()
        self._check(self._lib.mxs_factor_kernels(self._h, n))
        return dict(zip(("reg_unary", "reg_binary", "generic", "workgroup", "wave_box", "lane_grid", "lane_group_small"),
                        (int(x) for x in n)))

    def variable_kernels(self) -> dict:
        n = (C.c_int64 * 6)()
        self._check(self._lib.mxs_variable_kernels(self._h, n))
        return dict(zip(("packed", "packed8", "wide", "generic", "not_swept", "hub"), (int(x) for x in n)))

    def table_storage(self) -> dict:
        n = (C.c_int64 * 4)()
        b = C.c_int64(0)
        self._check(self._lib.mxs_table_storage(self._h, n, C.byref(b)))
        return {"full": int(n[0]), "f32": int(n[1]), "i16": int(n[2]), "i8": int(n[3]),
                "bytes_per_cycle": int(b.value)}

    def update_factor_table(self, factor: int, table):
        t = np.ascontiguousarray(table, dtype=np.float64).reshape(-1)
        self._check(self._lib.mxs_update_factor_table(self._h, int(factor), t.ctypes.data, t.shape[0]))
        lo, hi = int(self.graph.table_off[factor]), int(self.graph.table_off[factor + 1])
        self.graph.tables[lo:hi] = t

    def set_parent_table(self, factor: int, parent, is_external):
        parent = np.ascontiguousarray(parent, dtype=np.float64)
        dims = np.ascontiguousarray(parent.shape, dtype=np.int32)
        ext = np.ascontiguousarray(is_external, dtype=np.uint8)
        if ext.shape != (parent.ndim,):
            raise ValueError("one is_external flag per dimension of the parent relation")
        self._check(self._lib.mxs_set_parent_table(self._h, int(factor), parent.ctypes.data, parent.ndim,
                                                   dims.ctypes.data, ext.ctypes.data))
        self._parents = getattr(self, "_parents", {})
        self._parents[int(factor)] = (parent, ext.astype(bool))

    def slice_factor(self, factor: int, external_idx):
        idx = np.ascontiguousarray(external_idx, dtype=np.int32)
        self._check(self._lib.mxs_slice_factor(self._h, int(factor), idx.ctypes.data))
        parent, ext = self._parents[int(factor)]
        sel, j = [], 0
        for i in range(parent.ndim):
            if ext[i]:
                sel.append(int(idx[j]))
                j += 1
            else:
                sel.append(slice(None))
        lo, hi = int(self.graph.table_off[factor]), int(self.graph.table_off[factor + 1])
        self.graph.tables[lo:hi] = parent[tuple(sel)].reshape(-1)

    def debug_timeline(self) -> np.ndarray:
        n = C.c_int32(0)
        self._check(self._lib.mxs_debug_timeline(self._h, None, 0, C.byref(n)))
        out = np.zeros((int(n.value), 3), dtype=np.int64)
        self._check(self._lib.mxs_debug_timeline(self._h, out.ctypes.data, int(n.value), C.byref(n)))
        return out

    def halo_setup(self, send_edges, recv_edges):
        s = np.ascontiguousarray(send_edges, dtype=np.int32)
        r = np.ascontiguousarray(recv_edges, dtype=np.int32)
        self._check(self._lib.mxs_halo_setup(self._h, s.ctypes.data, s.shape[0],
                                             r.ctypes.data, r.shape[0]))

    def halo_buffers(self):
        s, r = C.c_void_p(), C.c_void_p()
        sb, rb = C.c_int64(0), C.c_int64(0)
        self._check(self._lib.mxs_halo_buffers(self._h, C.byref(s), C.byref(sb), C.byref(r), C.byref(rb)))
        return (s.value, int(sb.value)), (r.value, int(rb.value))

    def halo_bind(self, send_ptr: int, recv_ptr: int):
        self._check(self._lib.mxs_halo_bind(self._h, C.c_void_p(send_ptr), C.c_void_p(recv_ptr)))

    def step_compute(self):
        self._check(self._lib.mxs_step_compute(self._h))

    def step_pack(self):
        self._check(self._lib.mxs_step_pack(self._h))

    def step_unpack(self):
        self._check(self._lib.mxs_step_unpack(self._h))

    def comm_init(self, rank: int, world: int, unique_id: bytes, send_counts, recv_counts,
                  rccl: Optional[str] = None):
        if len(unique_id) != UNIQUE_ID_BYTES:
            raise ValueError("unique_id must be the 128 bytes of comm_unique_id()")
        sc = np.ascontiguousarray(send_counts, dtype=np.int64)
        rc = np.ascontiguousarray(recv_counts, dtype=np.int64)
        if sc.shape != (world,) or rc.shape != (world,):
            raise ValueError("one count per rank")
        uid = C.create_string_buffer(bytes(unique_id), UNIQUE_ID_BYTES)
        self._check(self._lib.mxs_comm_init(self._h, (rccl or rccl_path()).encode(), int(rank), int(world),
                                            C.cast(uid, C.c_void_p), sc.ctypes.data, rc.ctypes.data))

    def comm_exchange(self):
        self._check(self._lib.mxs_comm_exchange(self._h))
# ... 47 lines not shown
```

Baseline: 57090 iterations/s.

## Fuse binary factor messages into packed variable sweep lanes

Adds a variable-factor (VF) fused path. Binary factors with narrow tables are no longer swept as their own class. Instead, each packed variable lane loads its partner's variable-to-factor message and the factor table, computes the incoming factor-to-variable message with damping and filtering, and writes it into a lane-aligned f2v region with its own send counters. This is meant to cut the separate factor pass and its scattered f2v traffic, at the cost of loading each table twice, extra per-lane index arrays, and a send-counter remapping (edge_cf) in the state get/set code. A compile macro MXS_VF_DEFAULT defaults to 0, so whether the path runs by default depends on how the options are read.

```diff
diff --git a/include/maxsum_gpu.h b/include/maxsum_gpu.h
--- a/include/maxsum_gpu.h
+++ b/include/maxsum_gpu.h
@@ -98,6 +98,8 @@
 int mxs_factor_kernels(const mxs_engine *e, int64_t counts[7]);
 
 int mxs_variable_kernels(const mxs_engine *e, int64_t counts[6]);
+
+int mxs_vf_factors(const mxs_engine *e, int64_t *n);
 
 int mxs_update_factor_table(mxs_engine *e, int32_t factor, const double *table, int64_t n_entries);
 
diff --git a/pydcop_amd/csrc/engine.hip b/pydcop_amd/csrc/engine.hip
--- a/pydcop_amd/csrc/engine.hip
+++ b/pydcop_amd/csrc/engine.hip
@@ -176,6 +176,7 @@
     DevBuf<T> v2f[2], f2v[2], tables, var_cost, belief, halo_send, halo_recv;
     DevBuf<uint8_t> cF, cV, owned, fowned;
     DevBuf<int32_t> vrowptr, vdom, init_idx, edge_gen_factor, edge_dom, sel, vell;
+    DevBuf<int32_t> vf_partner, vf_jp;
     DevBuf<WaveMeta> vwave;
     DevBuf<int32_t> edge_v2f, f2v_off, vslot_f2v, vslot_v2f;
     DevBuf<int32_t> frowptr, edge_var_int, eval_idx;
@@ -195,6 +196,7 @@
     DevBuf<NaryDesc> ndesc;
     DevBuf<WideBlock> wide_blocks;
     DevBuf<HubBlock> hub_blocks;
+    bool vf_widened = false;
     bool has_hub = false;
 #ifdef MXS_WIDE_PROFILE
     DevBuf<int64_t> wide_prof;
@@ -262,6 +264,8 @@
         a.vslot_f2v = vslot_f2v.p;
         a.vslot_v2f = vslot_v2f.p;
         a.vell = vell.p;
+        a.vf_partner = vf_partner.p;
+        a.vf_jp = vf_jp.p;
         a.vwave = vwave.p;
         a.hub_blocks = hub_blocks.p;
         a.vdom = vdom.p;
@@ -334,6 +338,19 @@
                 case 4: hipLaunchKernelGGL((k_sweep_p2p<T, 4>), grid, block, 0, stream, a); break;
                 default: hipLaunchKernelGGL((k_sweep_p2p<T, 0>), grid, block, 0, stream, a); break;
             }
+        } else if (timeline_on && L.n_vf_factors > 0 && !has_hub) {
+#define MXS_TIMELINE_VF(DS)                                                                                              \
+    do {                                                                                                                 \
+        if (vf_widened) hipLaunchKernelGGL((k_sweep_timeline_vf<T, DS, VF_ANY_TABLE>), grid, block, 0, stream, a);       \
+        else hipLaunchKernelGGL((k_sweep_timeline_vf<T, DS, VF_NARROW_TABLES>), grid, block, 0, stream, a);              \
+    } while (0)
+            switch (L.dsel) {
+                case 2: MXS_TIMELINE_VF(2); break;
+                case 3: MXS_TIMELINE_VF(3); break;
+                case 4: MXS_TIMELINE_VF(4); break;
+                default: MXS_TIMELINE_VF(0); break;
+            }
+#undef MXS_TIMELINE_VF
         } else if (timeline_on && has_hub) {
             if (L.dsel == 3) hipLaunchKernelGGL((k_sweep_timeline_hub<T, 3>), grid, block, 0, stream, a);
             else hipLaunchKernelGGL((k_sweep_timeline_hub<T, 0>), grid, block, 0, stream, a);
@@ -358,6 +375,31 @@
             if (L.dsel == 3) MXS_SWEEP_HUB(3);
             else MXS_SWEEP_HUB(0);
 #undef MXS_SWEEP_HUB
+        } else if (L.n_vf_factors > 0 && vf_widened) {
+            switch (L.dsel) {
+                case 2: hipLaunchKernelGGL((k_sweep_vf_widened<T, 2>), grid, block, 0, stream, a); break;
+                case 3: hipLaunchKernelGGL((k_sweep_vf_widened<T, 3>), grid, block, 0, stream, a); break;
+                case 4: hipLaunchKernelGGL((k_sweep_vf_widened<T, 4>), grid, block, 0, stream, a); break;
+                default: hipLaunchKernelGGL((k_sweep_vf_widened<T, 0>), grid, block, 0, stream, a); break;
+            }
+        } else if (L.n_vf_factors > 0) {
+#define MXS_SWEEP_VF(KERNEL, ...)                                                                                        \
+    do {                                                                                                                 \
+        if (streaming) {                                                                                                 \
+            if (a.sched) hipLaunchKernelGGL((KERNEL<T, ##__VA_ARGS__, NT_STREAMING, true>), grid, block, 0, stream, a);  \
+            else hipLaunchKernelGGL((KERNEL<T, ##__VA_ARGS__, NT_STREAMING, false>), grid, block, 0, stream, a);         \
+        } else {                                                                                                         \
+            if (a.sched) hipLaunchKernelGGL((KERNEL<T, ##__VA_ARGS__, MXS_NT, true>), grid, block, 0, stream, a);        \
+            else hipLaunchKernelGGL((KERNEL<T, ##__VA_ARGS__, MXS_NT, false>), grid, block, 0, stream, a);               \
+        }                                                                                                                \
+    } while (0)
+            switch (L.dsel) {
+                case 2: MXS_SWEEP_VF(k_sweep_vf_d2); break;
+                case 3: MXS_SWEEP_VF(k_sweep_vf, 3); break;
+                case 4: MXS_SWEEP_VF(k_sweep_vf, 4); break;
+                default: MXS_SWEEP_VF(k_sweep_vf, 0); break;
+            }
+#undef MXS_SWEEP_VF
         } else {
 #define MXS_SWEEP(DS)                                                                                          \
     do {                                                                                                       \
@@ -577,6 +619,10 @@
     }
 
     int upload_class_arrays() {
+        refresh_vf_classes(L);
+        vf_widened = false;
+        for (const ClassInfo& ci : L.classes)
+            if (ci.kind == K_V_PACK && ci.vf && ci.vf_tab_type == TAB_FULL) vf_widened = true;
         std::vector<ClassInfo> order;
         for (int c : L.sweep_order) order.push_back(L.classes[c]);
         HIP_TRY(classes.upload(order, stream));
@@ -725,9 +771,11 @@
         HIP_TRY(tables.upload(conv(L.tables), stream));
         HIP_TRY(ctables.upload(L.ctables, stream));
         HIP_TRY(var_cost.upload(conv(L.var_cost), stream));
-        HIP_TRY(cF.alloc((size_t)L.n_edges));
+        HIP_TRY(cF.alloc((size_t)L.n_cf));
         HIP_TRY(cV.alloc((size_t)L.n_cv));
         HIP_TRY(vell.upload(L.vell, stream));
+        HIP_TRY(vf_partner.upload(L.vf_partner, stream));
+        HIP_TRY(vf_jp.upload(L.vf_jp, stream));
         HIP_TRY(vwave.upload(L.vwave, stream));
         HIP_TRY(owned.upload(L.owned, stream));
         HIP_TRY(fowned.upload(L.fowned, stream));
@@ -957,7 +1005,7 @@
         { int rc = sync(); if (rc) return rc; }
         const int nE = L.n_edges;
         std::vector<T> hv((size_t)(L.v2f_elems + (p2p ? ghost_len : 0))), hf((size_t)L.f2v_elems);
-        std::vector<uint8_t> hcF(nE), hcV((size_t)L.n_cv);
+        std::vector<uint8_t> hcF((size_t)L.n_cf), hcV((size_t)L.n_cv);
         if (L.v2f_elems)
             HIP_TRY(copy_sync(hv.data(), v2f[cur].p, sizeof(T) * (size_t)L.v2f_elems, hipMemcpyDeviceToHost, stream));
         if (p2p && ghost_len)
@@ -966,7 +1014,7 @@
         if (L.f2v_elems)
             HIP_TRY(copy_sync(hf.data(), f2v[cur].p, sizeof(T) * hf.size(), hipMemcpyDeviceToHost, stream));
         if (nE) {
-            HIP_TRY(copy_sync(hcF.data(), cF.p, nE, hipMemcpyDeviceToHost, stream));
+            HIP_TRY(copy_sync(hcF.data(), cF.p, (size_t)L.n_cf, hipMemcpyDeviceToHost, stream));
             HIP_TRY(copy_sync(hcV.data(), cV.p, (size_t)L.n_cv, hipMemcpyDeviceToHost, stream));
         }
         std::vector<int64_t> ext_off(nE + 1, 0);
@@ -979,7 +1027,7 @@
                 if (v2f_out) v2f_out[ext_off[e] + d] = sign * (double)hv[L.v2f_off[ei] + d];
                 if (f2v_out) f2v_out[ext_off[e] + d] = sign * (double)hf[L.f2v_off[ei] + d];
             }
-            if (cf) cf[e] = L.edge_fcim[ei] ? (uint8_t)(int)hf[L.f2v_off[ei] + D] : hcF[ei];
+            if (cf) cf[e] = L.edge_fcim[ei] ? (uint8_t)(int)hf[L.f2v_off[ei] + D] : hcF[L.edge_cf[ei]];
         }
         if (cv)
             for (int k = 0; k < nE; ++k) {
@@ -998,11 +1046,11 @@
         if (cyc < 0) return fail(MXS_E_INVALID, "negative cycle count");
         const int nE = L.n_edges, nV = L.n_vars;
         std::vector<T> hv((size_t)L.v2f_elems), hf((size_t)L.f2v_elems);
-        std::vector<uint8_t> hcF(nE), hcV((size_t)L.n_cv);
+        std::vector<uint8_t> hcF((size_t)L.n_cf), hcV((size_t)L.n_cv);
         if (L.v2f_elems) HIP_TRY(copy_sync(hv.data(), v2f[cur].p, sizeof(T) * hv.size(), hipMemcpyDeviceToHost, stream));
         if (L.f2v_elems) HIP_TRY(copy_sync(hf.data(), f2v[cur].p, sizeof(T) * hf.size(), hipMemcpyDeviceToHost, stream));
         if (nE) {
-            HIP_TRY(copy_sync(hcF.data(), cF.p, nE, hipMemcpyDeviceToHost, stream));
+            HIP_TRY(copy_sync(hcF.data(), cF.p, (size_t)L.n_cf, hipMemcpyDeviceToHost, stream));
             HIP_TRY(copy_sync(hcV.data(), cV.p, (size_t)L.n_cv, hipMemcpyDeviceToHost, stream));
         }
         std::vector<int64_t> ext_off(nE + 1, 0);
@@ -1018,7 +1066,7 @@
             if (cf) {
                 if (cf[e] > SAME_COUNT) return fail(MXS_E_INVALID, "send counter above SAME_COUNT");
                 if (L.edge_fcim[ei]) hf[L.f2v_off[ei] + D] = (T)(int)cf[e];
-                else hcF[ei] = cf[e];
+                else hcF[L.edge_cf[ei]] = cf[e];
             }
         }
         if (cv)
@@ -1032,7 +1080,7 @@
         if (L.v2f_elems) HIP_TRY(copy_sync(v2f[cur].p, hv.data(), sizeof(T) * hv.size(), hipMemcpyHostToDevice, stream));
         if (L.f2v_elems) HIP_TRY(copy_sync(f2v[cur].p, hf.data(), sizeof(T) * hf.size(), hipMemcpyHostToDevice, stream));
         if (nE) {
-            HIP_TRY(copy_sync(cF.p, hcF.data(), nE, hipMemcpyHostToDevice, stream));
+            HIP_TRY(copy_sync(cF.p, hcF.data(), (size_t)L.n_cf, hipMemcpyHostToDevice, stream));
             HIP_TRY(copy_sync(cV.p, hcV.data(), (size_t)L.n_cv, hipMemcpyHostToDevice, stream));
         }
         if ((idx || bel) && nV) {
@@ -1957,6 +2005,12 @@
     return MXS_OK;
 }
 
+int mxs_vf_factors(const mxs_engine* e, int64_t* n) {
+    CHECK_HANDLE(e);
+    if (n) *n = e->impl->L.n_vf_factors;
+    return MXS_OK;
+}
+
 int mxs_variable_kernels(const mxs_engine* e, int64_t counts[6]) {
     CHECK_HANDLE(e);
     if (!counts) return MXS_OK;
diff --git a/pydcop_amd/csrc/kernels.h b/pydcop_amd/csrc/kernels.h
--- a/pydcop_amd/csrc/kernels.h
+++ b/pydcop_amd/csrc/kernels.h
@@ -140,6 +140,8 @@
     int32_t block_base[MAX_CLASSES];
     const ClassInfo* classes;
     const uint32_t* sched;
+    const int32_t* vf_partner;
+    const int32_t* vf_jp;
 };
 
 template <typename T>
@@ -291,6 +293,26 @@
     }
 }
 
+template <typename T, int D>
+__device__ __forceinline__ void binary_message(const T (&tab)[D * D], const T (&m)[D], bool to1, T (&o)[D]) {
+#pragma unroll
+    for (int x = 0; x < D; ++x) {
+        T best = pos_inf<T>();
+#pragma unroll
+        for (int y = 0; y < D; ++y) {
+            const T c = (to1 ? tab[y * D + x] : tab[x * D + y]) + ((T)0 + m[y]);
+            if (best > c) best = c;
+        }
+        o[x] = best;
+    }
+}
+template <typename T, int D>
+__device__ __forceinline__ void binary_start(const SweepArgs<T>& a, T (&o)[D]) {
+    const bool sends = a.start_mode == MXS_START_ALL;
+#pragma unroll
+    for (int d = 0; d < D; ++d) o[d] = sends ? o[d] : (T)0;
+}
+
 template <typename T, int D, bool P2P = false, int NT = MXS_NT, bool CUT_HALF = true>
 __device__ __forceinline__ void factor_binary(const SweepArgs<T>& a, const ClassInfo& ci, int j) {
     MXS_NT_FLAGS(NT);
@@ -332,27 +354,12 @@
         if (do0) Msg<T, D>::template load<NT_GATHER>(a.v2f_old + v1, m1);
     }
     T o0[D], o1[D];
-#pragma unroll
-    for (int x = 0; x < D; ++x) {
-        T best0 = pos_inf<T>(), best1 = pos_inf<T>();
-#pragma unroll
-        for (int y = 0; y < D; ++y) {
-            const T c0 = tab[x * D + y] + ((T)0 + m1[y]);
-            if (best0 > c0) best0 = c0;
-            const T c1 = tab[y * D + x] + ((T)0 + m0[y]);
-            if (best1 > c1) best1 = c1;
-        }
-        o0[x] = best0;
-        o1[x] = best1;
-    }
+    binary_message<T, D>(tab, m1, false, o0);
+    binary_message<T, D>(tab, m0, true, o1);
     uint8_t c0 = 0, c1 = 0;
     if (a.start) {
-        const bool sends = a.start_mode == MXS_START_ALL;
-#pragma unroll
-        for (int d = 0; d < D; ++d) {
-            o0[d] = sends ? o0[d] : (T)0;
-            o1[d] = sends ? o1[d] : (T)0;
-        }
+        binary_start<T, D>(a, o0);
+        binary_start<T, D>(a, o1);
     } else {
         c0 = damp_and_filter<T, D>(o0, p0, cn0, a.damp_f != 0, a.damping, a.stability);
         c1 = damp_and_filter<T, D>(o1, p1, cn1, a.damp_f != 0, a.damping, a.stability);
@@ -452,7 +459,8 @@
     a.cF[e] = out;
 }
 
-template <typename T, int D, bool P2P = false, int NT = MXS_NT>
+constexpr int VF_NARROW_TABLES = 1, VF_ANY_TABLE = 2;
+template <typename T, int D, bool P2P = false, int NT = MXS_NT, int VF = 0>
 __device__ __forceinline__ void variable_pack(const SweepArgs<T>& a, const ClassInfo& ci, int item) {
     MXS_NT_FLAGS(NT);
     constexpr int H = Msg<T, D>::H;
@@ -467,8 +475,16 @@
     const int k = l - var * deg;
     const bool has = var < nv;
     const int v = wm.first_var + (has ? var : 0);
-    const int32_t slot = ldp<NT_IDX>(a.vell + pos);
-    const int32_t send_at = a.send_slot != nullptr ? a.send_slot[pos] : -1;
+    const int vf = VF ? ci.vf : 0;
+    const int64_t fo = VF ? ci.vf_f2v_base + (int64_t)lane_id * H : 0;
+    int32_t slot, partner = -1, jp = 0;
+    if (VF && vf == 2) slot = (int32_t)fo;
+    else slot = ldp<NT_IDX>(a.vell + pos);
+    if (VF && vf) {
+        partner = ldp<NT_IDX>(a.vf_partner + pos);
+        jp = ldp<NT_IDX>(a.vf_jp + pos);
+    }
+    const int32_t send_at = (!VF && a.send_slot != nullptr) ? a.send_slot[pos] : -1;
     constexpr bool CIM = Msg<T, D>::CNT_IN_MSG;
     T pv[D], in[D], c[D], b[D], m[D];
     const int64_t vo = ci.v2f_base + (int64_t)lane_id * H;
@@ -483,6 +499,46 @@
     for (int d = 0; d < D; ++d) c[d] = a.var_cost[ci.cost_base + (int64_t)(v - ci.first) * D + d];
     int init = -1;
     if (a.start) init = a.init_idx[v];
+    if constexpr (VF) {
+        if (vf) {
+            T g[D], tab[D * D], o[D];
+            const uint8_t cnf = a.cF[ci.vf_cf_base + lane_id];
+            Msg<T, D>::template load<NT_GATHER>(a.v2f_old + (partner >= 0 ? (int64_t)partner : vo), g);
+            uint8_t cfo = 0;
+#pragma unroll
+            for (int d = 0; d < D; ++d) o[d] = (T)0;
+            auto message = [&](auto tt) {
+                ClassInfo fc{};
+                fc.tab_type = decltype(tt)::value;
+                fc.count = ci.vf_count;
+                fc.tab_base = ci.vf_tab_base;
+                fc.ctab_base = ci.vf_ctab_base;
+                load_table<T, D * D, NT>(a, fc, jp >> 1, tab);
+                if (partner >= 0) binary_message<T, D>(tab, g, (jp & 1) != 0, o);
+            };
+            switch (ci.vf_tab_type) {
+                case TAB_I8: message(std::integral_constant<int, TAB_I8>{}); break;
+                case TAB_I16: message(std::integral_constant<int, TAB_I16>{}); break;
+                case TAB_F32: message(std::integral_constant<int, TAB_F32>{}); break;
+                default:
+                    if constexpr (VF == VF_ANY_TABLE) message(std::integral_constant<int, TAB_FULL>{});
+                    break;
+            }
+            if (partner >= 0) {
+                if (a.start) binary_start<T, D>(a, o);
+                else cfo = damp_and_filter<T, D>(o, in, cnf, a.damp_f != 0, a.damping, a.stability);
+            }
+            if constexpr ((64 * H * sizeof(T)) % 16 == 0) {
+                T full[H];
+#pragma unroll
+                for (int d = 0; d < H; ++d) full[d] = Msg<T, D>::padded(o, 0, d);
+                wave_store_linear<T, H, NT>(a.f2v_new, fo - (int64_t)l * H, full);
+            } else {
+                Msg<T, D>::store(a.f2v_new + fo, o);
+            }
+            a.cF[ci.vf_cf_base + lane_id] = cfo;
+        }
+    }
     const int seg = l - (has ? k : 0);
     T sum_cost = (T)0;
 #pragma unroll
@@ -902,10 +958,10 @@
     a.cV[k0 + ko] = out;
 }
 
-template <typename T, int D, bool P2P = false, int NT = MXS_NT, bool CUT_HALF = true>
+template <typename T, int D, bool P2P = false, int NT = MXS_NT, bool CUT_HALF = true, int VF = 0>
 __device__ __forceinline__ void sweep_d(const SweepArgs<T>& a, const ClassInfo& ci, int item) {
     if (ci.kind == K_V_PACK) {
-        variable_pack<T, D, P2P, NT>(a, ci, item);
+        variable_pack<T, D, P2P, NT, VF>(a, ci, item);
         return;
     }
     const int j = item + (int)threadIdx.x;
@@ -941,7 +997,7 @@
     }
 }
 
-template <typename T, int DSEL, bool P2P = false, int NT = MXS_NT, bool SCHED = false, bool HUB = false>
+template <typename T, int DSEL, bool P2P = false, int NT = MXS_NT, bool SCHED = false, bool HUB = false, int VF = 0>
 __device__ __forceinline__ int sweep_block(const SweepArgs<T>& a) {
     int c = 0, blk = -1;
     if (SCHED || a.sched != nullptr) {
@@ -967,12 +1023,12 @@
         return ci.kind;
     }
     if (DSEL != 0) {
-        sweep_d<T, (DSEL != 0 ? DSEL : 2), P2P, NT, !SCHED>(a, ci, item);
+        sweep_d<T, (DSEL != 0 ? DSEL : 2), P2P, NT, !SCHED, VF>(a, ci, item);
     } else {
         switch (ci.D) {
-            case 2: sweep_d<T, 2, P2P, NT, !SCHED>(a, ci, item); break;
-            case 3: sweep_d<T, 3, P2P, NT, !SCHED>(a, ci, item); break;
-            case 4: sweep_d<T, 4, P2P, NT, !SCHED>(a, ci, item); break;
+            case 2: sweep_d<T, 2, P2P, NT, !SCHED, VF>(a, ci, item); break;
+            case 3: sweep_d<T, 3, P2P, NT, !SCHED, VF>(a, ci, item); break;
+            case 4: sweep_d<T, 4, P2P, NT, !SCHED, VF>(a, ci, item); break;
             default: break;
         }
     }
@@ -998,15 +1054,30 @@
     sweep_block<T, DSEL, false, NT, SCHED, true>(a);
 }
 
+template <typename T, int DSEL, int NT = MXS_NT, bool SCHED = false>
+__global__ void __launch_bounds__(BLOCK, SWEEP_MIN_WAVES) __attribute__((amdgpu_num_sgpr(SWEEP_SGPRS)))
+k_sweep_vf(SweepArgs<T> a) {
+    sweep_block<T, DSEL, false, NT, SCHED, false, VF_NARROW_TABLES>(a);
+}
+template <typename T, int NT = MXS_NT, bool SCHED = false>
+__global__ void __launch_bounds__(BLOCK, SWEEP_MIN_WAVES) __attribute__((amdgpu_num_sgpr(80)))
+k_sweep_vf_d2(SweepArgs<T> a) {
+    sweep_block<T, 2, false, NT, SCHED, false, VF_NARROW_TABLES>(a);
+}
+template <typename T, int DSEL>
+__global__ void __launch_bounds__(BLOCK, SWEEP_MIN_WAVES) k_sweep_vf_widened(SweepArgs<T> a) {
+    sweep_block<T, DSEL, false, MXS_NT, false, false, VF_ANY_TABLE>(a);
+}
+
 template <typename T, int DSEL>
 __global__ void __launch_bounds__(BLOCK, SWEEP_MIN_WAVES) k_sweep_p2p(SweepArgs<T> a) {
     sweep_block<T, DSEL, true, MXS_NT, false, true>(a);
 }
 
-template <typename T, int DSEL, bool HUB>
+template <typename T, int DSEL, bool HUB, int VF = 0>
 __device__ __forceinline__ void sweep_timeline(const SweepArgs<T>& a) {
     const int64_t t0 = (int64_t)wall_clock64();
-    const int kind = sweep_block<T, DSEL, false, MXS_NT, false, HUB>(a);
+    const int kind = sweep_block<T, DSEL, false, MXS_NT, false, HUB, VF>(a);
     __builtin_amdgcn_s_waitcnt(0);
     const int64_t t1 = (int64_t)wall_clock64();
     if (threadIdx.x == 0) {
@@ -1018,6 +1089,10 @@
 template <typename T, int DSEL>
 __global__ void __launch_bounds__(BLOCK, SWEEP_MIN_WAVES) k_sweep_timeline(SweepArgs<T> a) {
     sweep_timeline<T, DSEL, false>(a);
+}
+template <typename T, int DSEL, int VF>
+__global__ void __launch_bounds__(BLOCK, SWEEP_MIN_WAVES) k_sweep_timeline_vf(SweepArgs<T> a) {
+    sweep_timeline<T, DSEL, false, VF>(a);
 }
 template <typename T, int DSEL>
 __global__ void __launch_bounds__(BLOCK) k_sweep_timeline_hub(SweepArgs<T> a) {
diff --git a/pydcop_amd/csrc/layout.cpp b/pydcop_amd/csrc/layout.cpp
--- a/pydcop_amd/csrc/layout.cpp
+++ b/pydcop_amd/csrc/layout.cpp
@@ -39,6 +39,9 @@
     o.nary_multi = !(f & 33554432);
     o.small = !(f & 8388608);
     o.hub = !(f & 4194304);
+    o.vf = MXS_VF_DEFAULT != 0;
+    if (f & 134217728) o.vf = true;
+    if (f & (67108864 | 4 | 32 | 64 | 2048 | 131072)) o.vf = false;
     o.tile_bytes = -1;
     if (f & 131072) o.tile_bytes = MXS_TILE_BYTES;
     if (f & 262144) o.tile_bytes = 0;
@@ -119,6 +122,17 @@
     return "";
 }
 
+}
+
+void refresh_vf_classes(Layout& L) {
+    for (ClassInfo& ci : L.classes) {
+        if (ci.kind != K_V_PACK || !ci.vf) continue;
+        const ClassInfo& fc = L.classes[ci.vf_fclass];
+        ci.vf_tab_type = fc.tab_type;
+        ci.vf_count = fc.count;
+        ci.vf_tab_base = fc.tab_base;
+        ci.vf_ctab_base = fc.ctab_base;
+    }
 }
 
 int narrowest_tab_type(const double* v, int64_t n, int word) {
@@ -373,6 +387,30 @@
 
     L.factor_e2i.resize(nF);
     for (int fi = 0; fi < nF; ++fi) L.factor_e2i[L.factor_i2e[fi]] = fi;
+    bool vf_D[MAX_REG_D + 1] = {};
+    if (L.opt.vf && L.opt.compact_tables && !g.var_owned) {
+        auto vkind = [&](int v) { return vsort[v] / 4096 / 1024; };
+        bool any_hub = false;
+        for (int v = 0; v < nV; ++v) any_hub = any_hub || vkind(v) == K_V_HUB;
+        int n[MAX_REG_D + 1] = {}, type[MAX_REG_D + 1];
+        bool ok[MAX_REG_D + 1];
+        for (int D = 0; D <= MAX_REG_D; ++D) {
+            type[D] = TAB_I8;
+            ok[D] = !any_hub && L.half(D) == D;
+        }
+        for (int f = 0; f < nF; ++f) {
+            if (fkey[f].kind != K_F_BIN) continue;
+            const int D = fkey[f].D, e0 = g.factor_rowptr[f];
+            n[D] += 1;
+            if (!ok[D]) continue;
+            if (vkind(g.edge_var[e0]) != K_V_PACK || vkind(g.edge_var[e0 + 1]) != K_V_PACK) ok[D] = false;
+            type[D] = std::min(type[D], narrowest_tab_type(g.tables + g.table_off[f], g.table_off[f + 1] - g.table_off[f], L.opt.word));
+            if (type[D] == TAB_FULL) ok[D] = false;
+        }
+        for (int D = 2; D <= MAX_REG_D; ++D) vf_D[D] = ok[D] && n[D] > 0;
+    }
+    auto is_vf_key = [&](const FKey& k) { return k.kind == K_F_BIN && vf_D[k.D]; };
+    std::vector<int32_t> vf_class(MAX_REG_D + 1, -1);
     L.f_tab_base.assign(nF, 0);
     L.f_tab_stride.assign(nF, 1);
     L.f_ctab_off.assign(nF, -1);
@@ -390,6 +428,7 @@
     L.edge_gen_factor.assign(nE, -1);
     L.edge_fcim.assign(nE, 0);
     L.edge_vcim.assign(nE, 0);
+    int64_t f2v_end = 0;
     {
         int ei = 0;
         int64_t off = 0;
@@ -400,6 +439,7 @@
             while (fj < nF && fkey[L.factor_i2e[fj]] == key) ++fj;
             off = (off + align - 1) / align * align;
             const bool split = key.kind == K_F_BIN;
+            const bool in_lanes = is_vf_key(key);
             const int Hc = split ? L.half(key.D) : 0;
             const int64_t half_len = split ? ((int64_t)(fj - fi) * Hc + align - 1) / align * align : 0;
             for (int f2 = fi; f2 < fj; ++f2) {
@@ -413,7 +453,9 @@
                     L.edge_dom[ei] = D;
                     L.edge_half[ei] = H;
                     int64_t at = off;
-                    if (split) {
+                    if (in_lanes) {
+                        at = 0;
+                    } else if (split) {
                         at = off + (int64_t)(e - g.factor_rowptr[f]) * half_len + (int64_t)(f2 - fi) * Hc;
                     } else {
                         const int bytes = H * L.opt.word;
@@ -426,7 +468,7 @@
                     L.f2v_off[ei] = (int32_t)at;
                 }
             }
-            if (split) off += 2 * half_len;
+            if (split && !in_lanes) off += 2 * half_len;
             if (off > ((int64_t)1 << 31) - 8192) return "message buffer exceeds 2^31 elements";
             fi = fj;
         }
@@ -434,7 +476,7 @@
         off = (off + align - 1) / align * align;
         L.null_f2v = off;
         off += std::max(L.half(MAX_REG_D), L.half(MAX_PACK8_D));
-        L.f2v_elems = off;
+        f2v_end = off;
     }
 
     L.vrowptr.assign(nV + 1, 0);
@@ -544,7 +586,14 @@
             }
             for (int j = 0; j < n; ++j) L.f_class[fi + j] = cls;
             L.classes.push_back(ci);
-            sweep_class(cls, BLOCK, key.cut || second);
+            if (is_vf_key(key)) {
+                if (ci.tab_type == TAB_FULL) return "internal error: VF factor class without a narrow table type";
+                L.classes[cls].per_block = BLOCK;
+                vf_class[key.D] = cls;
+                L.n_vf_factors += n;
+            } else {
+                sweep_class(cls, BLOCK, key.cut || second);
+            }
         } else {
             const int gen_base = (int)L.fgen.size();
             for (int j = 0; j < n; ++j) {
@@ -603,6 +652,15 @@
 
     L.n_cv = nE;
     for (int k = 0; k < nE; ++k) L.vslot_cv[k] = k;
+    L.n_cf = nE;
+    L.edge_cf.resize(nE);
+    std::iota(L.edge_cf.begin(), L.edge_cf.end(), (int64_t)0);
+    std::vector<int32_t> edge_factor;
+    if (L.n_vf_factors > 0) {
+        edge_factor.resize(nE);
+        for (int fi = 0; fi < nF; ++fi)
+            for (int e = L.frowptr[fi]; e < L.frowptr[fi + 1]; ++e) edge_factor[e] = fi;
+    }
     int64_t voff = 0;
     for (int vi = 0; vi < nV;) {
         const int v0 = L.var_i2e[vi];
@@ -675,6 +733,14 @@
             ci.cv_base = L.n_cv;
             ci.v2f_base = voff;
             int64_t lanes = 0;
+            const int fcls = ci.kind == K_V_PACK ? vf_class[ci.D] : -1;
+            int64_t not_vf = 0;
+            if (fcls >= 0) {
+                const int64_t align = 32 / L.opt.word;
+                ci.vf_fclass = fcls;
+                ci.vf_f2v_base = (f2v_end + align - 1) / align * align;
+                ci.vf_cf_base = L.n_cf;
+            }
             for (int w = vi; w < vj;) {
                 const int deg = L.vrowptr[w + 1] - L.vrowptr[w];
                 int w2 = w;
@@ -688,12 +754,30 @@
                         const int var = lane / deg, k = lane % deg;
                         if (var < nv) {
                             const int ks = L.vrowptr[x + var] + k;
+                            const int ei = L.vslot_edge[ks];
+                            int32_t partner = -1, jp = 0;
+                            if (fcls >= 0 && L.f_class[edge_factor[ei]] == fcls) {
+                                const int fi = edge_factor[ei], pp = ei - L.frowptr[fi];
+                                partner = L.frowptr[fi] + (1 - pp);
+                                jp = ((fi - L.classes[fcls].first) << 1) | pp;
+                                const int64_t at = ci.vf_f2v_base + lanes * ci.H;
+                                if (at > ((int64_t)1 << 31) - 8192) return "message buffer exceeds 2^31 elements";
+                                L.f2v_off[ei] = (int32_t)at;
+                                L.vslot_f2v[ks] = (int32_t)at;
+                                L.edge_cf[ei] = ci.vf_cf_base + lanes;
+                            } else {
+                                not_vf += 1;
+                            }
+                            L.vf_partner.push_back(partner);
+                            L.vf_jp.push_back(jp);
                             L.vell.push_back(L.vslot_f2v[ks]);
                             L.vslot_cv[ks] = ci.cv_base + lanes;
                             L.vslot_v2f[ks] = (int32_t)(ci.v2f_base + lanes * ci.H);
                             if (ci.H > ci.D) L.edge_vcim[L.vslot_edge[ks]] = 1;
                         } else {
                             L.vell.push_back(-1);
+                            L.vf_partner.push_back(-1);
+                            L.vf_jp.push_back(0);
                         }
                         ++lanes;
                     }
@@ -703,6 +787,12 @@
             ci.count = (int32_t)lanes;
             L.n_cv += lanes;
             voff += lanes * ci.H;
+            if (fcls >= 0) {
+                ci.vf = not_vf == 0 ? 2 : 1;
+                L.n_cf += lanes;
+                f2v_end = ci.vf_f2v_base + lanes * ci.H;
+                if (f2v_end > ((int64_t)1 << 31) - 8192) return "message buffer exceeds 2^31 elements";
+            }
         } else {
             for (int w = vi; w < vj; ++w)
                 for (int k = L.vrowptr[w]; k < L.vrowptr[w + 1]; ++k) {
@@ -727,7 +817,11 @@
         vi = vj;
     }
     L.v2f_elems = voff;
+    L.f2v_elems = f2v_end;
     for (int k = 0; k < nE; ++k) L.v2f_off[L.vslot_edge[k]] = L.vslot_v2f[k];
+    for (int32_t& pe : L.vf_partner)
+        if (pe >= 0) pe = L.v2f_off[pe];
+    refresh_vf_classes(L);
     for (NaryDesc& d : L.ndesc)
         for (int i = 0; i < (d.arity & 255); ++i) d.v2f_off[i] = L.v2f_off[d.edge_base + i];
 
diff --git a/pydcop_amd/csrc/layout.h b/pydcop_amd/csrc/layout.h
--- a/pydcop_amd/csrc/layout.h
+++ b/pydcop_amd/csrc/layout.h
@@ -32,6 +32,9 @@
 #endif
 #ifndef MXS_SCHEDULE_DEFAULT
 #define MXS_SCHEDULE_DEFAULT 1
+#endif
+#ifndef MXS_VF_DEFAULT
+#define MXS_VF_DEFAULT 0
 #endif
 #ifndef MXS_TILE_BYTES
 #define MXS_TILE_BYTES (512 << 10)
@@ -228,6 +231,14 @@
     int64_t ctab_base;
     int32_t own_pos;
     int32_t uni_D;
+    int32_t vf;
+    int32_t vf_fclass;
+    int32_t vf_tab_type;
+    int32_t vf_count;
+    int64_t vf_tab_base;
+    int64_t vf_ctab_base;
+    int64_t vf_f2v_base;
+    int64_t vf_cf_base;
 };
 
 constexpr int NARY_DESC_ARITY = 6;
@@ -333,6 +344,7 @@
     bool bin2 = true;
     bool hub = true;
     bool half_cut = true;
+    bool vf = true;
     int64_t tile_bytes = -1;
 };
 
@@ -387,6 +399,11 @@
     std::vector<int64_t> vslot_cv;
     std::vector<int32_t> vell;
     std::vector<WaveMeta> vwave;
+    std::vector<int32_t> vf_partner;
+    std::vector<int32_t> vf_jp;
+    std::vector<int64_t> edge_cf;
+    int64_t n_cf = 0;
+    int32_t n_vf_factors = 0;
     int64_t n_cv = 0;
     int dsel = 0;
     std::vector<int32_t> vdom;
@@ -413,5 +430,6 @@
 void encode_tab_record(const double* v, int entries, int t, uint8_t* dst);
 void encode_tab_entry(double v, int t, int word, uint8_t* dst);
 LayoutOptions options_from_params(const mxs_params& p);
-
-}
+void refresh_vf_classes(Layout& L);
+
+}
diff --git a/pydcop_amd/engine.py b/pydcop_amd/engine.py
--- a/pydcop_amd/engine.py
+++ b/pydcop_amd/engine.py
@@ -27,7 +27,7 @@
     "mxs_peer_export", "mxs_peer_connect",
     "mxs_debug_timeline", "mxs_update_factor_table", "mxs_destroy", "mxs_last_error", "mxs_version",
     "mxs_build_kind", "mxs_set_state", "mxs_set_parent_table", "mxs_slice_factor",
-    "mxs_table_storage", "mxs_factor_order", "mxs_factor_kernels", "mxs_variable_kernels",
+    "mxs_table_storage", "mxs_factor_order", "mxs_factor_kernels", "mxs_variable_kernels", "mxs_vf_factors",
     "mxs_amaxsum_create", "mxs_amaxsum_reset", "mxs_amaxsum_run", "mxs_amaxsum_status",
     "mxs_amaxsum_generation_sizes", "mxs_amaxsum_get_assignment", "mxs_amaxsum_get_messages",
     "mxs_amaxsum_eval_cost", "mxs_amaxsum_update_factor_table", "mxs_amaxsum_destroy",
@@ -210,6 +210,7 @@
         "mxs_factor_order": ([vp, C.POINTER(i32)], C.c_int),
         "mxs_factor_kernels": ([vp, vp], C.c_int),
         "mxs_variable_kernels": ([vp, vp], C.c_int),
+        "mxs_vf_factors": ([vp, C.POINTER(i64)], C.c_int),
         "mxs_halo_setup": ([vp, vp, i64, vp, i64], C.c_int),
         "mxs_halo_buffers": ([vp, C.POINTER(vp), C.POINTER(i64), C.POINTER(vp), C.POINTER(i64)], C.c_int),
         "mxs_halo_bind": ([vp, vp, vp], C.c_int),
@@ -397,6 +398,11 @@
         self._check(self._lib.mxs_variable_kernels(self._h, n))
         return dict(zip(("packed", "packed8", "wide", "generic", "not_swept", "hub"), (int(x) for x in n)))
 
+    def vf_factors(self) -> int:
+        n = C.c_int64(0)
+        self._check(self._lib.mxs_vf_factors(self._h, C.byref(n)))
+        return int(n.value)
+
     def table_storage(self) -> dict:
         n = (C.c_int64 * 4)()
         b = C.c_int64(0)
```

Measured after the change: 57760 iterations/s, median of 5. +1.2%, better.
